# Mingrui-Yu/A-Simple-Stereo-SLAM-System-with-Deep-Loop-Closing

Hardware: AMD Instinct MI355X
Metric: stereo frames/sec (ORB+match+LCD+BA-build) @1241x376 (higher is better)
Workload: dtype u8/int32 (ORB, Hamming), f32 via f16x3 / bf16x6 split products on the matrix cores with f32 accumulate (CALC conv1 / conv2, DB scan), f64 (triangulation, BA)

## Files before the change

### a-simple-stereo-slam-system-with-deep-loop-closing_amd/api.py

```python
import ctypes as C
import os
import re

import numpy as np

_HERE = os.path.dirname(os.path.abspath(__file__))
LIB_PATH = os.path.join(_HERE, "libmyslam_hip.so")

OK, ERR_INVALID, ERR_HIP, ERR_CAPACITY, ERR_UNSUPPORTED = 0, -1, -2, -3, -4
LCD_DIM = 1064

KP_DTYPE = np.dtype([("x", "<f4"), ("y", "<f4"), ("size", "<f4"), ("angle", "<f4"),
                     ("response", "<f4"), ("octave", "<i4"), ("class_id", "<i4")])
assert KP_DTYPE.itemsize == 28


class MyslamError(RuntimeError):
    def __init__(self, where, code):
        names = {-1: "INVALID", -2: "HIP", -3: "CAPACITY", -4: "UNSUPPORTED"}
        super().__init__(f"{where} failed: {code} ({names.get(code, '?')})")
        self.code = code


HEADER_PATH = os.path.join(_HERE, "..", "include", "myslam_hip.h")
CALC_LAYER_DTYPE = np.dtype([("type", "<i4"), ("num_output", "<i4"), ("kernel", "<i4"), ("stride", "<i4"), ("pad", "<i4"),
                             ("local_size", "<i4"), ("alpha", "<f4"), ("beta", "<f4"), ("k", "<f4")])
assert CALC_LAYER_DTYPE.itemsize == 36
CALC_CONV, CALC_RELU, CALC_POOL_MAX, CALC_LRN = 1, 2, 3, 4
CAND_DTYPE = np.dtype([("best_id", "<u8"), ("max_score", "<f4"), ("cnt", "<i4")])
assert CAND_DTYPE.itemsize == 16
OWNED_DTYPE = np.dtype([("pre_best_id", "<u8"), ("pre_max_score", "<f4"), ("pre_cnt", "<i4"),
                        ("suf_best_id", "<u8"), ("suf_max_score", "<f4"), ("suf_cnt", "<i4")])
assert OWNED_DTYPE.itemsize == 32

_lib = None
_SCALARS = {"int": C.c_int, "float": C.c_float, "double": C.c_double, "size_t": C.c_size_t, "uint64_t": C.c_uint64, "long": C.c_long,
            "int32_t": C.c_int32, "uint8_t": C.c_uint8, "int64_t": C.c_int64}


def header_prototypes(path=HEADER_PATH):
    txt = open(path).read()
    txt = re.sub(r"/\*.*?\*/", " ", txt, flags=re.S)
    txt = re.sub(r"//[^\n]*", " ", txt)
    out = {}
    for m in re.finditer(r"\b(int|float|size_t|const char\s*\*)\s+(myslam_\w+)\s*\(([^()]*)\)\s*;", txt):
        ret, name, params = m.group(1), m.group(2), m.group(3).strip()
        types = []
        if params and params != "void":
            for prm in params.split(","):
                prm = prm.strip()
                if "*" in prm:
                    types.append("ptr")
                else:
                    toks = [t for t in prm.split() if t != "const"]
                    types.append(toks[0])
        out[name] = ("char*" if "char" in ret else ret, types)
    return out


def lib():
    global _lib
    if _lib is None:
        if not os.path.exists(LIB_PATH):
            raise RuntimeError(f"{LIB_PATH} is missing: run __graft_entry__.build() / build.py first (no CPU fallback)")
        L = C.CDLL(LIB_PATH)
        for name, (ret, types) in header_prototypes().items():
            fn = getattr(L, name)
            fn.restype = {"int": C.c_int, "float": C.c_float, "size_t": C.c_size_t, "char*": C.c_char_p}[ret]
            fn.argtypes = [C.c_void_p if t == "ptr" else _SCALARS[t] for t in types]
        _lib = L
    return _lib


def _check(code, where):
    if code != OK:
        raise MyslamError(where, code)


def _p(a):
    return a.ctypes.data_as(C.c_void_p) if a is not None else None


def device_count():
    return lib().myslam_hip_device_count()


def version():
    return lib().myslam_hip_version().decode()


def build_id():
    return version().rsplit(" ", 1)[-1]


def shader_clock_mhz(stream=0, spin_us=200.0):
    v = C.c_float()
    _check(lib().myslam_prof_shader_clock_mhz(stream, float(spin_us), C.byref(v)), "myslam_prof_shader_clock_mhz")
    return float(v.value)


def prof_enable(on=True):
    lib().myslam_prof_enable(1 if on else 0)


def prof_reset():
    lib().myslam_prof_reset()


def prof_read():
    L = lib()
    out = {}
    for i in range(L.myslam_prof_count()):
        name = C.c_char_p(); ms = C.c_double(); n = C.c_long()
        L.myslam_prof_get(i, C.byref(name), C.byref(ms), C.byref(n))
        out[name.value.decode()] = (ms.value, n.value)
    return out


class ORBextractor:

    def __init__(self, nfeatures=2000, scaleFactor=1.2, nlevels=8, iniThFAST=20, minThFAST=7, stream=None):
        self._h = C.c_void_p()
        _check(lib().myslam_orb_create(C.byref(self._h), int(nfeatures), C.c_float(scaleFactor), int(nlevels),
                                       int(iniThFAST), int(minThFAST)), "myslam_orb_create")
        self.nfeatures, self.nlevels = nfeatures, nlevels
        if stream is not None:
            self.set_stream(stream)

    def __del__(self):
        if getattr(self, "_h", None) and self._h.value and _lib is not None:
            _lib.myslam_orb_destroy(self._h)
            self._h = C.c_void_p()

    def set_stream(self, stream_ptr):
        _check(lib().myslam_orb_set_stream(self._h, C.c_void_p(stream_ptr)), "myslam_orb_set_stream")

    def set_fast_event(self, event_ptr):
        _check(lib().myslam_orb_set_fast_event(self._h, C.c_void_p(event_ptr or None)), "myslam_orb_set_fast_event")

    def set_fast_gate(self, event_ptr):
        _check(lib().myslam_orb_set_fast_gate(self._h, C.c_void_p(event_ptr or None)), "myslam_orb_set_fast_gate")

    OPT_FAST_MODE, OPT_INTERNAL_STREAM, OPT_STOP_AFTER, OPT_COPY_INPUT, OPT_BLUR_MFMA, OPT_SIDE_BLOCKS_PER_CU = 1, 2, 3, 4, 5, 6

    def set_option(self, option, value):
        _check(lib().myslam_orb_set_option(self._h, int(option), int(value)), "myslam_orb_set_option")

    def set_gauss_taps(self, q7=None):
        q = None if q7 is None else np.ascontiguousarray(q7, np.int32)
        _check(lib().myslam_orb_set_gauss_taps(self._h, _p(q) if q is not None else None), "myslam_orb_set_gauss_taps")

    def tables(self):
        n = self.nlevels
        sc = np.zeros(n, np.float32); isc = np.zeros(n, np.float32); npl = np.zeros(n, np.int32); um = np.zeros(16, np.int32)
        _check(lib().myslam_orb_get_tables(self._h, _p(sc), _p(isc), _p(npl), _p(um)), "myslam_orb_get_tables")
        return sc, isc, npl, um

    def max_keypoints(self, rows=None, cols=None):
        if rows is not None:
            return lib().myslam_orb_max_keypoints_for(self._h, int(rows), int(cols))
        return lib().myslam_orb_max_keypoints(self._h)

    @staticmethod
    def _img(img):
        img = np.ascontiguousarray(img, np.uint8)
        assert img.ndim == 2
        return img

    def DetectAndCompute(self, image, mask=None, cap=None):
        img = self._img(image)
        cap = cap or self.max_keypoints(*img.shape)
        kps = np.zeros(cap, KP_DTYPE); desc = np.zeros((cap, 32), np.uint8); n = C.c_int()
        m = self._img(mask) if mask is not None else None
        _check(lib().myslam_orb_detect_and_compute(self._h, _p(img), img.shape[0], img.shape[1], img.strides[0],
                                                   _p(m), m.strides[0] if m is not None else 0,
                                                   _p(kps), _p(desc), cap, C.byref(n)), "myslam_orb_detect_and_compute")
        return kps[:n.value].copy(), desc[:n.value].copy()

    def Detect(self, image, mask=None, cap=None):
        img = self._img(image)
        cap = cap or self.max_keypoints(*img.shape)
        kps = np.zeros(cap, KP_DTYPE); n = C.c_int()
        m = self._img(mask) if mask is not None else None
        _check(lib().myslam_orb_detect(self._h, _p(img), img.shape[0], img.shape[1], img.strides[0],
                                       _p(m), m.strides[0] if m is not None else 0, _p(kps), cap, C.byref(n)),
               "myslam_orb_detect")
        return kps[:n.value].copy()

    def ScreenAndComputeKPsParams(self, image, keypoints):
        img = self._img(image)
        kin = np.ascontiguousarray(keypoints, KP_DTYPE).copy()
        kout = np.zeros(max(len(kin), 1), KP_DTYPE); n = C.c_int()
        _check(lib().myslam_orb_screen_and_compute_params(self._h, _p(img), img.shape[0], img.shape[1], img.strides[0],
                                                          _p(kin), len(kin), _p(kout), len(kout), C.byref(n)),
               "myslam_orb_screen_and_compute_params")
        return kout[:n.value].copy(), kin

    def CalcDescriptors(self, image, keypoints):
        img = self._img(image)
        k = np.ascontiguousarray(keypoints, KP_DTYPE)
        desc = np.zeros((len(k), 32), np.uint8)
        _check(lib().myslam_orb_calc_descriptors(self._h, _p(img), img.shape[0], img.shape[1], img.strides[0],
                                                 _p(k), len(k), _p(desc)), "myslam_orb_calc_descriptors")
        return desc

    def detect_and_compute_batch(self, d_imgs, batch, rows, cols, step, img_stride, d_kps, d_desc, d_counts, d_status, cap,
                                 d_masks=0):
        _check(lib().myslam_orb_detect_and_compute_batch(self._h, C.c_void_p(d_imgs), batch, rows, cols, step,
                                                         C.c_size_t(img_stride), C.c_void_p(d_masks or None),
                                                         C.c_void_p(d_kps), C.c_void_p(d_desc), C.c_void_p(d_counts),
                                                         C.c_void_p(d_status or None), cap),
               "myslam_orb_detect_and_compute_batch")

    def detect_batch(self, d_imgs, batch, rows, cols, step, img_stride, d_kps, d_counts, d_status, cap, d_masks=0):
        _check(lib().myslam_orb_detect_batch(self._h, C.c_void_p(d_imgs), batch, rows, cols, step, C.c_size_t(img_stride),
                                             C.c_void_p(d_masks or None), C.c_void_p(d_kps), C.c_void_p(d_counts),
                                             C.c_void_p(d_status or None), cap), "myslam_orb_detect_batch")

    def process_keyframes_batch(self, d_imgs, batch, rows, cols, step, img_stride, d_feat_xy, d_n_feat, feat_cap, d_pyr_kps, d_desc, d_counts,
                                d_status, cap):
        _check(lib().myslam_orb_process_keyframes_batch(self._h, C.c_void_p(d_imgs), int(batch), int(rows), int(cols), int(step),
                                                        C.c_size_t(img_stride), C.c_void_p(d_feat_xy), C.c_void_p(d_n_feat), int(feat_cap),
                                                        C.c_void_p(d_pyr_kps), C.c_void_p(d_desc), C.c_void_p(d_counts), C.c_void_p(d_status),
                                                        int(cap)), "myslam_orb_process_keyframes_batch")

    def debug_pyramid(self, image, level, blurred=False):
        img = self._img(image)
        w = C.c_int(); h = C.c_int()
        _check(lib().myslam_orb_debug_pyramid(self._h, _p(img), img.shape[0], img.shape[1], img.strides[0], level,
                                              1 if blurred else 0, None, 0, C.byref(w), C.byref(h)), "debug_pyramid(size)")
        out = np.zeros((h.value, w.value), np.uint8)
        _check(lib().myslam_orb_debug_pyramid(self._h, _p(img), img.shape[0], img.shape[1], img.strides[0], level,
                                              1 if blurred else 0, _p(out), out.strides[0], C.byref(w), C.byref(h)),
               "debug_pyramid")
        return out

    def debug_candidates(self, image, level, mask=None):
        img = self._img(image)
        cap = 65536
        xs = np.zeros(cap, np.int32); ys = np.zeros(cap, np.int32); sc = np.zeros(cap, np.int32); n = C.c_int()
        m = self._img(mask) if mask is not None else None
        _check(lib().myslam_orb_debug_candidates(self._h, _p(img), img.shape[0], img.shape[1], img.strides[0],
                                                 _p(m), m.strides[0] if m is not None else 0, level,
                                                 _p(xs), _p(ys), _p(sc), cap, C.byref(n)), "debug_candidates")
        return xs[:n.value].copy(), ys[:n.value].copy(), sc[:n.value].copy()

    def fast_statistics(self, level):
        out = np.zeros(4, np.uint32)
        _check(lib().myslam_orb_debug_readback(self._h, 6, 0, level, _p(out), out.nbytes, 0), "debug_readback")
        return int(out[0]), int(out[1]), int(out[2])


def hamming_match(query, train):
    q = np.ascontiguousarray(query, np.uint8).reshape(-1, 32); t = np.ascontiguousarray(train, np.uint8).reshape(-1, 32)
    idx = np.zeros(len(q), np.int32); dist = np.zeros(len(q), np.int32)
    _check(lib().myslam_hamming_match(_p(q), len(q), _p(t), len(t), _p(idx), _p(dist)), "myslam_hamming_match")
    return idx, dist


def hamming_match_batch(d_q, d_nq, d_t, d_nt, batch, cap, d_idx, d_dist, stream=0):
    _check(lib().myslam_hamming_match_batch(C.c_void_p(d_q), C.c_void_p(d_nq), C.c_void_p(d_t), C.c_void_p(d_nt), batch, cap,
                                            C.c_void_p(d_idx), C.c_void_p(d_dist), C.c_void_p(stream or None)),
           "myslam_hamming_match_batch")


def hamming_filter(dist):
    d = np.ascontiguousarray(dist, np.int32)
    keep = np.zeros(len(d), np.uint8); mn = C.c_int()
    _check(lib().myslam_hamming_filter(_p(d), len(d), _p(keep), C.byref(mn)), "myslam_hamming_filter")
    return keep.astype(bool), mn.value


def expand_pyramid_keypoints(feats, nlevels=8):
    f = np.ascontiguousarray(feats, KP_DTYPE)
    out = np.zeros(len(f) * nlevels, KP_DTYPE)
    _check(lib().myslam_expand_pyramid_keypoints(_p(f), len(f), nlevels, _p(out)), "myslam_expand_pyramid_keypoints")
    return out


def match_feature_pairs(train_idx, dist, loop_pyr_kps, cur_pyr_kps):
    ti = np.ascontiguousarray(train_idx, np.int32); d = np.ascontiguousarray(dist, np.int32)
    lk = np.ascontiguousarray(loop_pyr_kps, KP_DTYPE); ck = np.ascontiguousarray(cur_pyr_kps, KP_DTYPE)
    assert len(ti) == len(d) == len(lk)
    pairs = np.zeros((max(len(ti), 1), 2), np.int32); n = C.c_int()
    _check(lib().myslam_match_feature_pairs(_p(ti), _p(d), len(ti), _p(lk), _p(ck), len(ck), _p(pairs), C.byref(n)), "myslam_match_feature_pairs")
    return pairs[:n.value].copy()


LOOP_MATCH_OK, LOOP_MATCH_FEW_PAIRS, LOOP_MATCH_FEW_POINTS = 0, 1, 2


def loop_match_batch(d_loop_desc, d_n_loop, d_cur_desc, d_n_cur, d_loop_pyr, d_cur_pyr, batch, cap, d_cur_feat_xy, d_loop_feat_landmark, feat_cap,
                     d_landmark_pos, landmark_stride, landmark_cap, min_matches, out_cap, d_train_idx, d_dist, d_pairs, d_n_pairs, d_valid_pairs,
                     d_pts3d, d_pts2d, d_counts, d_status, stream=0):
    ptrs = [C.c_void_p(x) for x in (d_loop_desc, d_n_loop, d_cur_desc, d_n_cur, d_loop_pyr, d_cur_pyr)]
    outs = [C.c_void_p(x) for x in (d_train_idx, d_dist, d_pairs, d_n_pairs, d_valid_pairs, d_pts3d, d_pts2d, d_counts, d_status)]
    _check(lib().myslam_loop_match_batch(*ptrs, int(batch), int(cap), C.c_void_p(d_cur_feat_xy), C.c_void_p(d_loop_feat_landmark), int(feat_cap),
                                         C.c_void_p(d_landmark_pos), int(landmark_stride), int(landmark_cap), int(min_matches), int(out_cap), *outs,
                                         C.c_void_p(stream or None)), "myslam_loop_match_batch")


def triangulate_stereo(xl, yl, xr, yr, fx, fy, cx, cy, baseline):
    xl, yl, xr, yr = [np.ascontiguousarray(a, np.float32) for a in (xl, yl, xr, yr)]
    n = len(xl)
    xyz = np.zeros((n, 3)); ok = np.zeros(n, np.uint8)
    _check(lib().myslam_triangulate_stereo(_p(xl), _p(yl), _p(xr), _p(yr), n, C.c_double(fx), C.c_double(fy), C.c_double(cx),
                                           C.c_double(cy), C.c_double(baseline), _p(xyz), _p(ok)), "myslam_triangulate_stereo")
    return xyz, ok.astype(bool)


def triangulate_stereo_batch(d_kl, d_kr, d_match, d_nl, batch, cap, K, baseline, d_xyz, d_ok, stream=0):
    _check(lib().myslam_triangulate_stereo_batch(C.c_void_p(d_kl), C.c_void_p(d_kr), C.c_void_p(d_match), C.c_void_p(d_nl),
                                                 batch, cap, C.c_double(K[0]), C.c_double(K[1]), C.c_double(K[2]),
                                                 C.c_double(K[3]), C.c_double(baseline), C.c_void_p(d_xyz), C.c_void_p(d_ok),
                                                 C.c_void_p(stream or None)), "myslam_triangulate_stereo_batch")


def hamming_match_triangulate_batch(d_q, d_nq, d_t, d_nt, d_kl, d_kr, batch, cap, K, baseline, d_idx, d_dist, d_xyz, d_ok, stream=0):
    _check(lib().myslam_hamming_match_triangulate_batch(C.c_void_p(d_q), C.c_void_p(d_nq), C.c_void_p(d_t), C.c_void_p(d_nt), C.c_void_p(d_kl),
                                                        C.c_void_p(d_kr), batch, cap, C.c_double(K[0]), C.c_double(K[1]), C.c_double(K[2]),
                                                        C.c_double(K[3]), C.c_double(baseline), C.c_void_p(d_idx), C.c_void_p(d_dist),
                                                        C.c_void_p(d_xyz), C.c_void_p(d_ok), C.c_void_p(stream or None)),
           "myslam_hamming_match_triangulate_batch")


def calc_default_layers():
    n = lib().myslam_lcd_default_layers(None, 0)
    L = np.zeros(n, CALC_LAYER_DTYPE)
    assert lib().myslam_lcd_default_layers(_p(L), n) == n
    return L


def calc_parse_caffe(prototxt_path, caffemodel_path):
    nl = C.c_int(); nw = C.c_size_t()
    _check(lib().myslam_calc_parse_caffe(prototxt_path.encode(), caffemodel_path.encode(), None, 0, C.byref(nl), None, 0, C.byref(nw)),
           "myslam_calc_parse_caffe")
    L = np.zeros(nl.value, CALC_LAYER_DTYPE); w = np.zeros(nw.value, np.float32)
    _check(lib().myslam_calc_parse_caffe(prototxt_path.encode(), caffemodel_path.encode(), _p(L), len(L), C.byref(nl), _p(w), w.size, C.byref(nw)),
           "myslam_calc_parse_caffe")
    return L, w


class DeepLCD:
    OPT_GENERIC_KERNELS = 1
    OPT_CONV2_BF16X6 = 2
    OPT_SKIP_KERNELS = 3

    def __init__(self, weights=None, stream=None, layers=None, caffe=None, path=None):
        self._h = C.c_void_p()
        if caffe is not None:
            _check(lib().myslam_lcd_create_from_caffe(C.byref(self._h), caffe[0].encode(), caffe[1].encode()), "myslam_lcd_create_from_caffe")
        elif path is not None:
            _check(lib().myslam_lcd_create_from_file(C.byref(self._h), path.encode()), "myslam_lcd_create_from_file")
        else:
            w = np.ascontiguousarray(weights, np.float32).ravel()
            if layers is not None:
                L = np.ascontiguousarray(layers, CALC_LAYER_DTYPE)
                _check(lib().myslam_lcd_create_from_layers(C.byref(self._h), _p(L), len(L), _p(w), w.size), "myslam_lcd_create_from_layers")
            else:
                _check(lib().myslam_lcd_create(C.byref(self._h), _p(w), w.size), "myslam_lcd_create")
        if stream is not None:
            _check(lib().myslam_lcd_set_stream(self._h, C.c_void_p(stream)), "myslam_lcd_set_stream")

    @classmethod
    def from_caffe(cls, prototxt_path="calc_model/deploy.prototxt", caffemodel_path="calc_model/calc.caffemodel", stream=None):
        return cls(caffe=(prototxt_path, caffemodel_path), stream=stream)

    def set_option(self, option, value):
        _check(lib().myslam_lcd_set_option(self._h, int(option), int(value)), "myslam_lcd_set_option")

    def uses_fused_kernels(self):
        return lib().myslam_lcd_uses_fused_kernels(self._h) == 1

    def conv2_products(self):
        return lib().myslam_lcd_conv2_products(self._h)

    def __del__(self):
        if getattr(self, "_h", None) and self._h.value and _lib is not None:
            _lib.myslam_lcd_destroy(self._h)
            self._h = C.c_void_p()

    def calcDescrOriginalImg(self, image, blur_in_place=True):
        img = np.ascontiguousarray(image, np.uint8).copy()
        d = np.zeros(LCD_DIM, np.float32)
        _check(lib().myslam_lcd_calc_descr_original_img(self._h, _p(img), img.shape[0], img.shape[1], img.strides[0],
                                                        1 if blur_in_place else 0, _p(d)), "myslam_lcd_calc_descr_original_img")
        return d, img

    def calcDescr(self, im160x120):
        img = np.ascontiguousarray(im160x120, np.uint8)
        assert img.shape == (120, 160)
        d = np.zeros(LCD_DIM, np.float32)
        _check(lib().myslam_lcd_calc_descr(self._h, _p(img), img.strides[0], _p(d)), "myslam_lcd_calc_descr")
        return d

    @staticmethod
    def score(d1, d2):
        a = np.ascontiguousarray(d1, np.float32); b = np.ascontiguousarray(d2, np.float32)
        return float(lib().myslam_lcd_score(_p(a), _p(b)))

    def describe_batch(self, d_imgs, batch, rows, cols, step, img_stride, d_out, blur_in_place=False):
        _check(lib().myslam_lcd_describe_batch(self._h, C.c_void_p(d_imgs), batch, rows, cols, step, C.c_size_t(img_stride),
                                               1 if blur_in_place else 0, C.c_void_p(d_out)), "myslam_lcd_describe_batch")
# ... 845 lines not shown
```

### a-simple-stereo-slam-system-with-deep-loop-closing_amd/csrc/orb_engine.hip

```cpp
#include <math.h>
#include <stdlib.h>
#include <string.h>

#include <vector>

#include "common.h"
#include "orb_launch.h"
#include "orb_plan.h"
#include "resize_tab.h"

namespace myslam_hip {

static inline int cv_round(float v) { return (int)lrintf(v); }
static inline size_t align_up(size_t v, size_t a) { return (v + a - 1) / a * a; }

void gauss_q8(int kind, int q[7]) {
    if (kind == 1) { const int t[7] = {8, 28, 56, 72, 56, 28, 8}; memcpy(q, t, sizeof(t)); return; }
    double g[7], sum = 0;
    for (int i = 0; i < 7; i++) { double x = i - 3; g[i] = exp(-(x * x) / 8.0); sum += g[i]; }
    for (int i = 0; i < 7; i++) q[i] = (int)lrint(g[i] / sum * 256.0);
}

}

using namespace myslam_hip;

struct myslam_orb {
    int nfeatures, nlevels, iniTh, minTh;
    float scaleFactor;
    std::vector<float> scale, invScale;
    std::vector<int> nPerLevel;
    int umax[16];
    hipStream_t stream = nullptr;
    hipStream_t aux = nullptr;
    hipEvent_t evFork = nullptr, evJoin = nullptr;
    hipEvent_t evUserFast = nullptr;
    hipEvent_t evUserGate = nullptr;

    int rows = 0, cols = 0;
    OrbPlan full{}, det{};

    int batchCap = 0;
    Buf<uint8_t> d_pyr, d_blur, d_mask;
    Buf<uint32_t> d_cand;
    Buf<uint32_t> d_sort;
    Buf<int32_t> d_candCount, d_selCount, d_status;
    Buf<uint32_t> d_sel;
    Buf<uint16_t> d_order;
    Buf<uint32_t> d_octTab;
    Buf<uint32_t> d_stripTab;
    Buf<uint32_t> d_resizeTab;
    size_t resizeColOff[MAXL] = {0}, resizeRowOff[MAXL] = {0}; bool resizeLvOk[MAXL] = {false};
    Buf<uint32_t> d_fastStat; int fastFlip = 0;
    int optFastMode = -1;
    int optInternalStream = 1;
    int optCopyInput = 0;
    int optStopAfter = 0;
    int tapsSet = 0, taps[7] = {0};
    int optSideBlocksPerCu = 0;
    int optBlurMfma = 0;
    Buf<uint4> d_blurTab; bool blurTabValid = false; size_t blurOffI = 0, blurOffH[MAXL] = {0}, blurOffV[MAXL] = {0}; bool blurLvOk[MAXL] = {false}; int blurVconst = 0;
    int ensure_blur_tables();

    struct HostGraph {
        static constexpr int kStayEager = -1000000;
        hipGraphExec_t exec = nullptr; hipGraph_t graph = nullptr; uint64_t gen = 0; int rows = 0, cols = 0, step = 0, dcap = 0, calls = 0; bool mask = false;
        void reset(bool stayEager = false) {
            if (exec) (void)hipGraphExecDestroy(exec);
            if (graph) (void)hipGraphDestroy(graph);
            if (stayEager) { exec = nullptr; graph = nullptr; calls = kStayEager; }
            else *this = HostGraph();
        }
        bool matches(uint64_t g, int r, int c, int st, int dc, bool m) const { return gen == g && rows == r && cols == c && step == st && dcap == dc && mask == m; }
        void rekey(uint64_t g, int r, int c, int st, int dc, bool m) { reset(); gen = g; rows = r; cols = c; step = st; dcap = dc; mask = m; }
    };
    HostGraph hostGraph[2][2];
    uint64_t gen = 1;
    ZeroArgs clr{};
    ZeroArgs take_clear() { const ZeroArgs z = clr; clr = ZeroArgs{}; return z; }
    hipStream_t hostStream = nullptr;
    PinBuf<uint8_t> h_pin;
    int ensure_pin(size_t bytes);
    void drop_host_graphs();
    Buf<uint8_t> d_stageImg, d_stageMask;
    int stageCap = 0;
    Buf<uint8_t> d_stageOut; size_t stageDescOff = 0;
    int32_t* stage_counts() const { return reinterpret_cast<int32_t*>(d_stageOut.get()); }
    myslam_keypoint* stage_kps() const { return reinterpret_cast<myslam_keypoint*>(d_stageOut + 256); }
    uint8_t* stage_desc() const { return d_stageOut + stageDescOff; }
    Buf<myslam_keypoint> d_stageKps2; Buf<uint8_t> d_stageKeep;

    int make_tables();
    void level_size(int l, int r, int c, int& w, int& h) const {
        w = cv_round((float)c * invScale[l]); h = cv_round((float)r * invScale[l]);
    }
    int make_plan(int r, int c);
    int ensure(int batch, int r, int c, bool needMask);
    int ensure_stage(size_t imgBytes, size_t maskBytes, int cap);
    int ensure_fast_stat();
    Buf<myslam_keypoint> d_pkfRows; Buf<uint8_t> d_pkfKeep;
    int ensure_pkf(size_t nrows);
    int process_keyframes(const uint8_t* d_imgs, int batch, int r, int c, int step, size_t stride, const float* d_feat_xy, const int32_t* d_n_feat,
                          int feat_cap, myslam_keypoint* d_pyr_kps, uint8_t* d_desc, int32_t* d_counts, int32_t* d_stat, int cap);
    void set_in_place(const uint8_t* p, size_t stride, int pitch, int n0) {
        full.ext0 = det.ext0 = p; full.ext0Stride = det.ext0Stride = stride; full.ext0Pitch = det.ext0Pitch = pitch; full.ext0N = det.ext0N = n0;
    }
    int stage_pyramid(const uint8_t* img, int r, int c, int step, const uint8_t* mask, int ncap);
    int build_pyramids(const uint8_t* d_imgs, int batch, int step, size_t stride, const uint8_t* d_masks, int nlev);
    ResizeArgs level_resize_args(uint8_t* base, int l) const;
    BlurArgs level_blur_args(int l) const;
    int blur_levels(int batch, int nlev, hipStream_t s);
    void fill_blur_args(BlurArgs* lv, int nlev) const;
    int run_fast(const OrbPlan& P, const uint8_t* maskPyr, int batch);
    int run_batch(const uint8_t* d_imgs, int batch, int r, int c, int step, size_t stride, const uint8_t* d_masks,
                  myslam_keypoint* d_kps, uint8_t* d_desc, int32_t* d_counts, int32_t* d_stat, int cap, bool detectOnly);
    void free_all();
};

int myslam_orb::make_tables() {
    scale.assign(nlevels, 1.f); invScale.assign(nlevels, 1.f); nPerLevel.assign(nlevels, 0);
    for (int i = 1; i < nlevels; i++) scale[i] = scale[i - 1] * scaleFactor;
    for (int i = 0; i < nlevels; i++) invScale[i] = 1.0f / scale[i];
    float factor = 1.0f / scaleFactor;
    float nDesired = nfeatures * (1 - factor) / (1 - (float)pow((double)factor, (double)nlevels));
    int sum = 0;
    for (int l = 0; l < nlevels - 1; l++) { nPerLevel[l] = cv_round(nDesired); sum += nPerLevel[l]; nDesired *= factor; }
    nPerLevel[nlevels - 1] = std::max(nfeatures - sum, 0);
    int v, v0, vmax = (int)floor(HALF_PATCH * sqrtf(2.f) / 2 + 1), vmin = (int)ceil(HALF_PATCH * sqrtf(2.f) / 2);
    const double hp2 = HALF_PATCH * HALF_PATCH;
    for (v = 0; v < 16; v++) umax[v] = 0;
    for (v = 0; v <= vmax; ++v) umax[v] = (int)lrint(sqrt(hp2 - v * v));
    for (v = HALF_PATCH, v0 = 0; v >= vmin; --v) { while (umax[v0] == umax[v0 + 1]) ++v0; umax[v] = v0; ++v0; }
    const int expect[16] = {15, 15, 15, 15, 14, 14, 14, 13, 13, 12, 11, 10, 9, 8, 6, 3};
    for (v = 0; v < 16; v++) if (umax[v] != expect[v]) return MYSLAM_ERR_INVALID;
    return MYSLAM_OK;
}

static int ceil_log2(int v) { int b = 0; while ((1 << b) < v) b++; return b; }

static int level_nini(int w, int h) {
    const int bx = w - EDGE_THRESHOLD + 3 - MIN_BORDER, by = h - EDGE_THRESHOLD + 3 - MIN_BORDER;
    return bx > 0 && by > 0 ? (int)roundf((float)bx / (float)by) : 0;
}
static int node_cap(int N, int nIni, int& cap) {
    cap = (std::max(N + 4, 4 * nIni + 4) + 3) & ~3;
    return cap > 4092 ? MYSLAM_ERR_UNSUPPORTED : MYSLAM_OK;
}

int myslam_orb::make_plan(int r, int c) {
    OrbPlan P{};
    P.nlevels = nlevels; P.rows = r; P.cols = c; P.iniTh = iniTh; P.minTh = minTh;
    size_t imgOff = 0, keyOff = 0; int cellBase = 0, outBase = 0, stripBase = 0;
    for (int l = 0; l < nlevels; l++) {
        LevelGeom& g = P.lv[l];
        level_size(l, r, c, g.w, g.h);
        if (g.w < 1 || g.h < 1) return MYSLAM_ERR_UNSUPPORTED;
        g.pitch = (int)align_up(g.w, 64);
        g.maxBX = g.w - EDGE_THRESHOLD + 3; g.maxBY = g.h - EDGE_THRESHOLD + 3;
        const float width = (float)(g.maxBX - MIN_BORDER), height = (float)(g.maxBY - MIN_BORDER);
        const float W = 30;
        g.nCols = (int)(width / W); g.nRows = (int)(height / W);
        if (g.nCols < 1 || g.nRows < 1) return MYSLAM_ERR_UNSUPPORTED;
        g.wCell = (int)ceilf(width / g.nCols); g.hCell = (int)ceilf(height / g.nRows);
        if (g.wCell > MAX_CELL || g.hCell > MAX_CELL) return MYSLAM_ERR_UNSUPPORTED;
        if (g.maxBX + 3 > 4095 + MIN_BORDER || g.maxBY + 3 > 4095 + MIN_BORDER) return MYSLAM_ERR_UNSUPPORTED;
        g.cellBase = cellBase; cellBase += g.nCols * g.nRows;
        g.stripBase = stripBase; stripBase += g.nRows * ((g.nCols + 3) / 4);
        g.N = nPerLevel[l];
        g.nIni = level_nini(g.w, g.h);
        if (g.nIni < 1 || g.nIni > 64) return MYSLAM_ERR_UNSUPPORTED;
        g.hX = (float)(g.maxBX - MIN_BORDER) / g.nIni;
        const int rootW = (int)ceilf(g.hX) + 2, H = g.maxBY - MIN_BORDER;
        g.ndepth = std::min(MAX_DEPTH, ceil_log2(std::max(rootW, H)) + 2);
        g.sortDepth = 0;
        while (g.sortDepth + 1 <= g.ndepth && (g.nIni << (2 * (g.sortDepth + 1))) <= 1024) g.sortDepth++;
        g.keyCap = (int)std::min<size_t>(262143, std::max<size_t>(256, (size_t)((g.w + 1) / 2) * ((g.h + 1) / 2)));
        if (node_cap(g.N, g.nIni, g.nodeCap)) return MYSLAM_ERR_UNSUPPORTED;
        g.outBase = outBase; outBase += g.nodeCap;
        g.scale = scale[l];
        g.scaledPatch = (float)(int)(PATCH_SIZE * scale[l]);
        g.imgOff = imgOff; imgOff += align_up((size_t)g.pitch * align_up((size_t)g.h, 8), 256);
        g.keyOff = keyOff; keyOff += g.keyCap;
    }
    for (int l = 0; l < MAXL; l++) P.stripBaseOf[l] = l < P.nlevels ? P.lv[l].stripBase : INT32_MAX;
    P.ncells = cellBase; P.nstrips = stripBase; P.totalKeyCap = (int)keyOff; P.totalOut = outBase; P.pyrBytes = imgOff;
    {
        std::vector<uint32_t> tab;
        for (int l = 0; l < nlevels; l++) {
            LevelGeom& g = P.lv[l];
            g.tabX = g.maxBX - MIN_BORDER + 8; g.tabY = g.maxBY - MIN_BORDER + 8; g.tabOff = (int)tab.size();
            tab.resize(tab.size() + 2 * (size_t)(g.tabX + g.tabY), 0u);
            uint32_t* xcode = tab.data() + g.tabOff; uint32_t* ycode = xcode + g.tabX;
            uint32_t* xcell = ycode + g.tabY; uint32_t* ycell = xcell + g.tabX;
            for (int px = 0; px < g.tabX; px++) {
                int r = (int)((float)px / g.hX);
                r = std::min(std::max(r, 0), g.nIni - 1);
                int UL = (int)(g.hX * (float)r), UR = (int)(g.hX * (float)(r + 1));
                uint32_t code = (uint32_t)r << ROOT_SHIFT;
                for (int k = 1; k <= g.ndepth; k++) {
                    const int mid = UL + ((UR - UL + 1) >> 1);
                    const uint32_t d = px >= mid;
                    code |= d << (ROOT_SHIFT - 2 * k);
                    if (d) UL = mid; else UR = mid;
                }
                xcode[px] = code;
                xcell[px] = (uint32_t)(std::max(px - 3, 0) / g.wCell);
            }
            for (int py = 0; py < g.tabY; py++) {
                int UL = 0, BR = g.maxBY - MIN_BORDER;
                uint32_t code = 0;
                for (int k = 1; k <= g.ndepth; k++) {
                    const int mid = UL + ((BR - UL + 1) >> 1);
                    const uint32_t d = py >= mid;
                    code |= (d << 1) << (ROOT_SHIFT - 2 * k);
                    if (d) UL = mid; else BR = mid;
                }
                ycode[py] = code;
                ycell[py] = (uint32_t)((std::max(py - 3, 0) / g.hCell) * g.nCols);
            }
        }
        int rc = d_octTab.renew(tab.size());
        if (rc) return rc;
        if ((rc = upload_table(d_octTab, tab.data(), tab.size() * sizeof(uint32_t)))) return rc;
    }
    {
        std::vector<uint32_t> st((size_t)P.nstrips * 8, 0u);
        for (int l = 0; l < nlevels; l++) {
            const LevelGeom& g = P.lv[l];
            const int spr = (g.nCols + 3) / 4;
            for (int strip = 0; strip < g.nRows * spr; strip++) {
                uint32_t* e = st.data() + (size_t)(g.stripBase + strip) * 8;
                const int ci = strip / spr, cj0 = (strip - ci * spr) * 4;
                const int iniY = MIN_BORDER + ci * g.hCell;
                int ncell = 0, pairs = 0; uint32_t wcs = 0; int hr = 0;
                if (iniY < g.maxBY - 3) {
                    hr = std::min(iniY + g.hCell + 6, g.maxBY) - iniY;
                    const int hc = hr - 6;
                    if (hc > 0)
                        for (int c = 0; c < 4; c++) {
                            const int cj = cj0 + c, iniX = MIN_BORDER + cj * g.wCell;
                            int wc = 0;
                            if (cj < g.nCols && iniX < g.maxBX - 6) wc = std::max(0, std::min(iniX + g.wCell + 6, g.maxBX) - iniX - 6);
                            if (wc > 0) ncell = c + 1;
                            wcs |= (uint32_t)wc << (8 * c);
                            pairs += ((wc + 1) >> 1) * hc;
                        }
                }
                if (ncell == 0) wcs = 0;
                e[0] = (uint32_t)l | ((uint32_t)ci << 8) | ((uint32_t)cj0 << 16) | ((uint32_t)ncell << 24);
                e[1] = (uint32_t)iniY | ((uint32_t)hr << 16);
                e[2] = (uint32_t)(MIN_BORDER + cj0 * g.wCell) | ((uint32_t)g.wCell << 16);
                e[3] = wcs; e[4] = (uint32_t)g.pitch; e[5] = (uint32_t)pairs;
                e[6] = (uint32_t)(g.imgOff & 0xffffffffu); e[7] = (uint32_t)(g.imgOff >> 32);
            }
        }
        int rc = d_stripTab.renew(st.size());
        if (rc) return rc;
        if ((rc = upload_table(d_stripTab, st.data(), st.size() * sizeof(uint32_t)))) return rc;
        P.stripTab = d_stripTab;
    }
    full = P;
    {
        std::vector<uint32_t> rt;
        std::vector<ResizeColRec> cr; std::vector<ResizeRowRec> rr;
        for (int l = 1; l < nlevels; l++) {
            const ResizeArgs a = level_resize_args(nullptr, l);
            resizeLvOk[l] = resize_uses_strips(a);
            if (!resizeLvOk[l]) continue;
            resize_col_records(a.sw, a.dw, a.scale_x, (a.dw + 255) / 256 * 64, cr);
            resize_row_records(a.sh, a.dh, a.scale_y, rr);
            resizeColOff[l] = rt.size();
            rt.insert(rt.end(), reinterpret_cast<const uint32_t*>(cr.data()), reinterpret_cast<const uint32_t*>(cr.data() + cr.size()));
            resizeRowOff[l] = rt.size();
            rt.insert(rt.end(), reinterpret_cast<const uint32_t*>(rr.data()), reinterpret_cast<const uint32_t*>(rr.data() + rr.size()));
            rt.resize((rt.size() + 7) & ~(size_t)7, 0u);
        }
        int rc = d_resizeTab.renew(rt.size());
        if (rc) return rc;
        if (!rt.empty() && (rc = upload_table(d_resizeTab, rt.data(), rt.size() * sizeof(uint32_t)))) return rc;
    }
    det = P;
    det.nlevels = 1;
    det.ncells = P.lv[0].nCols * P.lv[0].nRows;
    det.nstrips = P.lv[0].nRows * ((P.lv[0].nCols + 3) / 4);
    det.lv[0].N = nfeatures;
    if (node_cap(nfeatures, P.lv[0].nIni, det.lv[0].nodeCap)) return MYSLAM_ERR_UNSUPPORTED;
    det.lv[0].outBase = 0;
    det.totalOut = det.lv[0].nodeCap;
    rows = r; cols = c;
    return MYSLAM_OK;
}

int myslam_orb::ensure(int batch, int r, int c, bool needMask) {
    if (r != rows || c != cols) {
        MYSLAM_HIP_CHECK(hipStreamSynchronize(stream));
        int rc = make_plan(r, c);
        if (rc) { rows = cols = 0; return rc; }
        batchCap = 0; gen++; blurTabValid = false;
    }
    const int detOut = det.totalOut;
    const size_t selPer = (size_t)std::max(full.totalOut, detOut);
    if (batch > batchCap) {
        MYSLAM_HIP_CHECK(hipStreamSynchronize(stream));
        gen++;
        d_mask.release();
        int rc = regrow(batchCap, batch, [&]() -> int {
            int rc;
            if ((rc = d_pyr.renew((size_t)batch * full.pyrBytes + 64))) return rc;
            if ((rc = d_blur.renew((size_t)batch * full.pyrBytes + 4096))) return rc;
            if ((rc = d_cand.renew((size_t)batch * full.totalKeyCap))) return rc;
            if ((rc = d_sort.renew((size_t)batch * full.totalKeyCap * 2))) return rc;
            if ((rc = d_candCount.renew((size_t)batch * MAXL))) return rc;
            if ((rc = d_selCount.renew((size_t)batch * MAXL))) return rc;
            if ((rc = d_status.renew((size_t)batch))) return rc;
            if ((rc = d_sel.renew((size_t)batch * selPer))) return rc;
            return d_order.renew((size_t)batch * selPer);
        });
        if (rc) return rc;
    }
    if (needMask && !d_mask) return d_mask.renew((size_t)batchCap * full.pyrBytes + 64);
    return MYSLAM_OK;
}

int myslam_orb::build_pyramids(const uint8_t* d_imgs, int batch, int step, size_t stride, const uint8_t* d_masks, int nlev) {
    const OrbPlan& P = full;
    for (int pass = 0; pass < (d_masks ? 2 : 1); pass++) {
        uint8_t* base = pass ? d_mask : d_pyr;
        const uint8_t* src = pass ? d_masks : d_imgs;
        const int n0 = pass ? 0 : P.ext0N;
        int l = 1;
        const int nhead = std::min(pyr_head_levels(), nlev - 1);
        if (nhead >= 1 && batch > n0 && resize_is_little(level_resize_args(base, 1), batch)) {
            ScopedProf sp(P_RESIZE, stream);
            ResizeArgs grp[3];
            for (int j = 0; j < nhead; j++) grp[j] = level_resize_args(base, 1 + j);
            grp[0].src = src; grp[0].spitch = step; grp[0].sstride = stride;
            launch_pyr_head(grp, nhead, P.rows, P.cols, base + P.lv[0].imgOff, P.lv[0].pitch, P.pyrBytes, n0, batch, take_clear(), stream);
            l = 1 + nhead;
        } else if (batch > n0) {
            launch_ingest(src + (size_t)n0 * stride, P.rows, P.cols, step, stride, base + (size_t)n0 * P.pyrBytes + P.lv[0].imgOff, P.lv[0].pitch,
                          P.pyrBytes, batch - n0, take_clear(), stream);
        }
        for (; l < nlev;) {
            ScopedProf sp(P_RESIZE, stream);
            ResizeArgs a = level_resize_args(base, l);
            if (l == 1 && n0 > 0) { a.src0 = d_imgs; a.spitch0 = step; a.sstride0 = stride; a.n0 = n0; }
            ResizeArgs grp[4]; int ng = 0;
            const int gmax = resize_chain_max();
            if (gmax > 1 && resize_is_little(a, batch)) {
                static const double kEvals[4] = {1, 5, 21, 85};
                double evals = (double)batch * a.dw * a.dh;
                grp[ng++] = a;
                while (ng < gmax && l + ng < nlev) {
                    const ResizeArgs nx = level_resize_args(base, l + ng);
                    evals += (double)batch * nx.dw * nx.dh * kEvals[ng];
                    if (!resize_is_little(nx, batch) || evals > 6e6) break;
                    grp[ng++] = nx;
                }
            }
            if (ng > 1) { launch_resize_chain(grp, ng, batch, stream); l += ng; }
            else { launch_resize(a, batch, stream); l++; }
        }
    }
    return MYSLAM_OK;
}
ResizeArgs myslam_orb::level_resize_args(uint8_t* base, int l) const {
    const OrbPlan& P = full;
    ResizeArgs a;
    a.src = base + P.lv[l - 1].imgOff; a.sw = P.lv[l - 1].w; a.sh = P.lv[l - 1].h; a.spitch = P.lv[l - 1].pitch; a.sstride = P.pyrBytes;
    a.src0 = nullptr; a.spitch0 = 0; a.n0 = 0; a.sstride0 = 0;
    a.dst = base + P.lv[l].imgOff; a.dw = P.lv[l].w; a.dh = P.lv[l].h; a.dpitch = P.lv[l].pitch; a.dstride = P.pyrBytes;
    a.scale_x = 1. / ((double)a.dw / a.sw); a.scale_y = 1. / ((double)a.dh / a.sh);
    if (d_resizeTab && resizeLvOk[l]) { a.colTab = d_resizeTab + resizeColOff[l]; a.rowTab = d_resizeTab + resizeRowOff[l]; }
    return a;
}
int myslam_orb::ensure_blur_tables() {
    if (blurTabValid) return MYSLAM_OK;
    std::vector<uint4> tab;
    int q[7];
    if (tapsSet) memcpy(q, taps, sizeof(q)); else gauss_q8(0, q);
    int sum = 0;
    for (int t = 0; t < 7; t++) sum += q[t];
    blurVconst = sum * 128 * sum + 32768;
    blur_mfma_ident(tab, blurOffI);
    for (int l = 0; l < full.nlevels; l++) blurLvOk[l] = blur_mfma_tables(full.lv[l].w, full.lv[l].h, q, tab, blurOffH[l], blurOffV[l]);
    MYSLAM_HIP_CHECK(hipStreamSynchronize(stream));
    int rc = d_blurTab.renew(tab.size());
    if (rc) return rc;
    if ((rc = upload_table(d_blurTab, tab.data(), tab.size() * sizeof(uint4)))) return rc;
    blurTabValid = true; gen++;
    return MYSLAM_OK;
}

BlurArgs myslam_orb::level_blur_args(int l) const {
    const OrbPlan& P = full;
    BlurArgs a;
    a.src = d_pyr + P.lv[l].imgOff; a.dst = d_blur + P.lv[l].imgOff;
    a.w = P.lv[l].w; a.h = P.lv[l].h; a.spitch = a.dpitch = P.lv[l].pitch; a.sstride = a.dstride = P.pyrBytes;
    a.src0 = nullptr; a.spitch0 = 0; a.n0 = 0; a.sstride0 = 0;
    a.dtiled = 1;
    if (tapsSet) memcpy(a.q, taps, sizeof(taps)); else gauss_q8(0, a.q);
    if (optBlurMfma && blurTabValid && blurLvOk[l]) { a.tabH = d_blurTab + blurOffH[l]; a.tabV = d_blurTab + blurOffV[l]; a.ident = d_blurTab + blurOffI; a.vconst = blurVconst; }
    return a;
}
void myslam_orb::fill_blur_args(BlurArgs* lv, int nlev) const {
    const OrbPlan& P = full;
    for (int l = 0; l < nlev; l++) {
        lv[l] = level_blur_args(l);
        if (l == 0 && P.ext0N > 0) { lv[l].src0 = P.ext0; lv[l].spitch0 = P.ext0Pitch; lv[l].sstride0 = P.ext0Stride; lv[l].n0 = P.ext0N; }
    }
}
int myslam_orb::blur_levels(int batch, int nlev, hipStream_t stream) {
    BlurArgs lv[MAXL];
    fill_blur_args(lv, nlev);
    ScopedProf sp(P_BLUR, stream);
    launch_blur_levels(lv, nlev, batch, stream);
    return MYSLAM_OK;
}

int myslam_orb::run_batch(const uint8_t* d_imgs, int batch, int r, int c, int step, size_t stride, const uint8_t* d_masks,
                          myslam_keypoint* d_kps, uint8_t* d_desc, int32_t* d_counts, int32_t* d_stat, int cap, bool detectOnly) {
    if (!d_imgs || batch <= 0 || r <= 0 || c <= 0 || step < c || cap <= 0 || !d_kps || !d_counts) return MYSLAM_ERR_INVALID;
    if (!detectOnly && !d_desc) return MYSLAM_ERR_INVALID;
    int rc = ensure(batch, r, c, d_masks != nullptr);
    if (rc) return rc;
    if (optBlurMfma && !detectOnly && (rc = ensure_blur_tables())) return rc;
    const OrbPlan& P = detectOnly ? det : full;
    int32_t* stat = d_stat ? d_stat : d_status;
    if ((rc = ensure_fast_stat())) return rc;
    clr = {{reinterpret_cast<uint32_t*>(d_candCount.get()), reinterpret_cast<uint32_t*>(d_selCount.get()), reinterpret_cast<uint32_t*>(stat), d_fastStat + (size_t)fastFlip * MAXL * 4},
           {batch * MAXL, batch * MAXL, batch, MAXL * 4}};
    const int stop = optStopAfter;
    {
        int n0 = 0;
        if (!optCopyInput && stop == 0 && batch > 1 && full.nlevels >= 1 && stride >= (size_t)r * (size_t)step) {
            bool ok = blur_uses_strips(level_blur_args(0));
            if (full.nlevels > 1) ok = ok && resize_uses_strips(level_resize_args(d_pyr, 1));
            if (ok) n0 = batch - 1;
        }
        set_in_place(d_imgs, stride, step, n0);
    }
    if (stop == 1) {
        launch_ingest(d_imgs, full.rows, full.cols, step, stride, d_pyr + full.lv[0].imgOff, full.lv[0].pitch, full.pyrBytes, batch, take_clear(), stream);
        return MYSLAM_OK;
    }
    if ((rc = build_pyramids(d_imgs, batch, step, stride, d_masks, P.nlevels))) return rc;
    if (stop == 2) return MYSLAM_OK;
    hipStreamCaptureStatus capst = hipStreamCaptureStatusNone;
    if (stream && hipStreamIsCapturing(stream, &capst) != hipSuccess) { (void)hipGetLastError(); capst = hipStreamCaptureStatusNone; }
    const int aux_mode = capst == hipStreamCaptureStatusActive ? 0 : optInternalStream;
    const bool fork = aux_mode > 0 && !detectOnly && stop == 0;
    if (fork && !aux) {
        MYSLAM_HIP_CHECK(hipStreamCreateWithFlags(&aux, hipStreamNonBlocking));
        MYSLAM_HIP_CHECK(hipEventCreateWithFlags(&evFork, hipEventDisableTiming));
        MYSLAM_HIP_CHECK(hipEventCreateWithFlags(&evJoin, hipEventDisableTiming));
    }
    auto fork_blur = [&]() -> int {
        MYSLAM_HIP_CHECK(hipEventRecord(evFork, stream));
        MYSLAM_HIP_CHECK(hipStreamWaitEvent(aux, evFork, 0));
        int rc2 = blur_levels(batch, P.nlevels, aux);
        if (rc2) return rc2;
        MYSLAM_HIP_CHECK(hipEventRecord(evJoin, aux));
        return MYSLAM_OK;
    };
    if (fork && aux_mode == 2 && (rc = fork_blur())) return rc;
    if (evUserGate) MYSLAM_HIP_CHECK(hipStreamWaitEvent(stream, evUserGate, 0));
    if ((rc = run_fast(P, d_masks ? d_mask : nullptr, batch))) return rc;
    if (evUserFast) MYSLAM_HIP_CHECK(hipEventRecord(evUserFast, stream));
    if (fork && aux_mode != 2 && (rc = fork_blur())) return rc;
    bool blurred = false;
    {
        ScopedProf sp(P_OCTREE, stream);
        BlurArgs blv[MAXL];
        const bool tryBlur = !fork && !detectOnly && stop == 0 && !optBlurMfma;
        if (tryBlur) fill_blur_args(blv, P.nlevels);
        blurred = launch_octree(P, d_cand, d_candCount, d_sort, d_octTab, d_sel, d_selCount, stat, batch,
                                describe_uses_tile_order(d_order != nullptr, detectOnly ? 1 : 0, batch) ? d_order : nullptr, stream,
                                tryBlur ? blv : nullptr, tryBlur ? P.nlevels : 0);
    }
    if (stop == 3) return MYSLAM_OK;
    if (fork) MYSLAM_HIP_CHECK(hipStreamWaitEvent(stream, evJoin, 0));
    else if (!detectOnly && !blurred && (rc = blur_levels(batch, P.nlevels, stream))) return rc;
    if (stop == 4) return MYSLAM_OK;
    {
        ScopedProf sp(P_DESC, stream);
        launch_describe(P, d_pyr, d_blur, full.pyrBytes, d_sel, d_selCount, d_kps, d_desc, d_counts, stat, cap,
                        detectOnly ? 1 : 0, batch, d_order, true, optSideBlocksPerCu, stream);
    }
    MYSLAM_HIP_CHECK(hipGetLastError());
    return MYSLAM_OK;
}

int myslam_orb::run_fast(const OrbPlan& P, const uint8_t* maskPyr, int batch) {
    uint32_t* cur = d_fastStat + (size_t)fastFlip * MAXL * 4;
    const uint32_t* prev = d_fastStat + (size_t)(fastFlip ^ 1) * MAXL * 4;
    fastFlip ^= 1;
    ScopedProf sp(P_FAST, stream);
    launch_fast(P, d_pyr, full.pyrBytes, maskPyr, d_cand, d_candCount, prev, cur, optFastMode, batch, stream);
    return MYSLAM_OK;
}

int myslam_orb::ensure_pin(size_t bytes) {
    if (bytes <= h_pin.size()) return MYSLAM_OK;
    gen++;
    return h_pin.renew((bytes + (bytes >> 2) + 4095) & ~(size_t)4095);
}

void myslam_orb::drop_host_graphs() {
    for (auto& row : hostGraph)
        for (auto& g : row) g.reset();
}

int myslam_orb::ensure_fast_stat() {
    if (d_fastStat) return MYSLAM_OK;
    int rc = d_fastStat.renew(2 * MAXL * 4);
    if (rc) return rc;
    MYSLAM_HIP_CHECK(hipMemsetAsync(d_fastStat, 0, sizeof(uint32_t) * 2 * MAXL * 4, stream));
    return MYSLAM_OK;
}

int myslam_orb::ensure_pkf(size_t nrows) {
    if (nrows <= std::min(d_pkfRows.size(), d_pkfKeep.size())) return MYSLAM_OK;
    MYSLAM_HIP_CHECK(hipStreamSynchronize(stream));
    gen++; drop_host_graphs();
    int rc;
    if ((rc = d_pkfRows.renew(nrows))) return rc;
    return d_pkfKeep.renew(nrows);
}

int myslam_orb::process_keyframes(const uint8_t* d_imgs, int batch, int r, int c, int step, size_t stride, const float* d_feat_xy,
                                  const int32_t* d_n_feat, int feat_cap, myslam_keypoint* d_pyr_kps, uint8_t* d_desc, int32_t* d_counts,
                                  int32_t* d_stat, int cap) {
    if (!d_imgs || !d_feat_xy || !d_n_feat || !d_pyr_kps || !d_desc || !d_counts || !d_stat) return MYSLAM_ERR_INVALID;
    if (batch <= 0 || r <= 0 || c <= 0 || step < c || feat_cap <= 0 || cap <= 0) return MYSLAM_ERR_INVALID;
    if (batch > 65535 || (size_t)feat_cap * nlevels > ((size_t)1 << 24) || cap > (1 << 24)) return MYSLAM_ERR_CAPACITY;
    int rc = ensure(batch, r, c, false);
    if (rc) return rc;
    if (optBlurMfma && (rc = ensure_blur_tables())) return rc;
    const int rowCap = feat_cap * nlevels;
    if ((rc = ensure_pkf((size_t)batch * rowCap))) return rc;
    clr = {{reinterpret_cast<uint32_t*>(d_counts), reinterpret_cast<uint32_t*>(d_stat), nullptr, nullptr}, {batch, batch, 0, 0}};
    set_in_place(nullptr, 0, 0, 0);
    rc = build_pyramids(d_imgs, batch, step, stride, nullptr, nlevels);
    clr = ZeroArgs{};
    if (rc) return rc;
    if ((rc = blur_levels(batch, nlevels, stream))) return rc;
    {
        ScopedProf sp(P_SCREEN, stream);
        launch_process_keyframes(full, PkfArgs{d_pyr, d_blur, full.pyrBytes, d_feat_xy, d_n_feat, feat_cap, d_pkfRows, d_pkfKeep, rowCap,
                                               d_pyr_kps, d_desc, d_counts, d_stat, cap}, batch, stream);
    }
    MYSLAM_HIP_CHECK(hipGetLastError());
    return MYSLAM_OK;
}

int myslam_orb::stage_pyramid(const uint8_t* img, int r, int c, int step, const uint8_t* mask, int ncap) {
    const size_t bytes = (size_t)r * step;
    int rc = ensure(1, r, c, mask != nullptr);
    if (rc) return rc;
    if ((rc = ensure_stage(bytes, mask ? bytes : 0, ncap))) return rc;
    MYSLAM_HIP_CHECK(hipMemcpyAsync(d_stageImg, img, bytes, hipMemcpyHostToDevice, stream));
    if (mask) MYSLAM_HIP_CHECK(hipMemcpyAsync(d_stageMask, mask, bytes, hipMemcpyHostToDevice, stream));
    set_in_place(nullptr, 0, 0, 0);
    return build_pyramids(d_stageImg, 1, step, bytes, mask ? d_stageMask : nullptr, nlevels);
}

int myslam_orb::ensure_stage(size_t imgBytes, size_t maskBytes, int cap) {
    int rc;
    if (imgBytes > d_stageImg.size()) { gen++; if ((rc = d_stageImg.renew(imgBytes))) return rc; }
    if (maskBytes > d_stageMask.size()) { gen++; if ((rc = d_stageMask.renew(maskBytes))) return rc; }
    if (cap > stageCap) {
        gen++;
        stageDescOff = 256 + (((size_t)cap * sizeof(myslam_keypoint) + 255) & ~(size_t)255);
        return regrow(stageCap, cap, [&]() -> int {
            int rc;
            if ((rc = d_stageOut.renew(stageDescOff + (size_t)cap * 32))) return rc;
            if ((rc = d_stageKps2.renew((size_t)cap))) return rc;
            return d_stageKeep.renew((size_t)cap);
        });
    }
    return MYSLAM_OK;
}

void myslam_orb::free_all() {
    if (aux) { (void)hipStreamSynchronize(aux); (void)hipStreamDestroy(aux); (void)hipEventDestroy(evFork); (void)hipEventDestroy(evJoin); aux = nullptr; }
    drop_host_graphs();
    if (hostStream) { (void)hipStreamSynchronize(hostStream); (void)hipStreamDestroy(hostStream); hostStream = nullptr; }
}

extern "C" {

int myslam_orb_create(myslam_orb** out, int nfeatures, float scale_factor, int nlevels, int ini_th_fast, int min_th_fast) {
    if (!out || nfeatures < 1 || nlevels < 1 || nlevels > MAXL || !(scale_factor > 1.0f) || ini_th_fast < 0 ||
        min_th_fast < 1 || min_th_fast > ini_th_fast || ini_th_fast > 255 || scale_factor > 2.5f)
        return MYSLAM_ERR_INVALID;
    if (need_device()) return MYSLAM_ERR_HIP;
    myslam_orb* h = new myslam_orb();
    h->nfeatures = nfeatures; h->scaleFactor = scale_factor; h->nlevels = nlevels; h->iniTh = ini_th_fast; h->minTh = min_th_fast;
    int rc = h->make_tables();
    if (rc) { delete h; return rc; }
    *out = h;
    return MYSLAM_OK;
}

int myslam_orb_destroy(myslam_orb* h) {
    if (!h) return MYSLAM_ERR_INVALID;
    (void)hipStreamSynchronize(h->stream);
    h->free_all();
    delete h;
    return MYSLAM_OK;
}

int myslam_orb_set_stream(myslam_orb* h, void* s) {
    if (!h) return MYSLAM_ERR_INVALID;
    (void)hipStreamSynchronize(h->stream);
    h->stream = (hipStream_t)s; h->gen++;
    return MYSLAM_OK;
}

int myslam_orb_set_fast_event(myslam_orb* h, void* ev) {
    if (!h) return MYSLAM_ERR_INVALID;
    h->evUserFast = (hipEvent_t)ev; h->gen++;
    return MYSLAM_OK;
}

int myslam_orb_set_fast_gate(myslam_orb* h, void* ev) {
    if (!h) return MYSLAM_ERR_INVALID;
    h->evUserGate = (hipEvent_t)ev; h->gen++;
    return MYSLAM_OK;
}

int myslam_orb_set_option(myslam_orb* h, int option, int value) {
    if (!h) return MYSLAM_ERR_INVALID;
    h->gen++;
    switch (option) {
        case MYSLAM_ORB_OPT_FAST_MODE: if (value < -1 || value > 1) return MYSLAM_ERR_INVALID; h->optFastMode = value; return MYSLAM_OK;
        case MYSLAM_ORB_OPT_INTERNAL_STREAM: if (value < 0 || value > 2) return MYSLAM_ERR_INVALID; h->optInternalStream = value; return MYSLAM_OK;
        case MYSLAM_ORB_OPT_COPY_INPUT: if (value < 0 || value > 1) return MYSLAM_ERR_INVALID; h->optCopyInput = value; return MYSLAM_OK;
        case MYSLAM_ORB_OPT_STOP_AFTER: if (value < 0 || value > 4) return MYSLAM_ERR_INVALID; h->optStopAfter = value; return MYSLAM_OK;
        case MYSLAM_ORB_OPT_BLUR_MFMA: if (value < 0 || value > 1) return MYSLAM_ERR_INVALID; h->optBlurMfma = value; return MYSLAM_OK;
        case MYSLAM_ORB_OPT_SIDE_BLOCKS_PER_CU: if (value < 0 || value > 64) return MYSLAM_ERR_INVALID; h->optSideBlocksPerCu = value; return MYSLAM_OK;
    }
    return MYSLAM_ERR_INVALID;
}

int myslam_orb_set_gauss_taps(myslam_orb* h, const int32_t* q7) {
    if (!h) return MYSLAM_ERR_INVALID;
    h->blurTabValid = false;
    if (!q7) { h->tapsSet = 0; h->gen++; return MYSLAM_OK; }
    int sum = 0;
    for (int i = 0; i < 7; i++) { if (q7[i] < 0 || q7[i] > 255) return MYSLAM_ERR_INVALID; sum += q7[i]; }
    if (sum < 1 || sum > 257) return MYSLAM_ERR_INVALID;
    for (int i = 0; i < 7; i++) h->taps[i] = q7[i];
    h->tapsSet = 1; h->gen++;
    return MYSLAM_OK;
}

int myslam_orb_get_tables(const myslam_orb* h, float* scale, float* inv_scale, int* fpl, int* umax16) {
    if (!h) return MYSLAM_ERR_INVALID;
    for (int i = 0; i < h->nlevels; i++) {
        if (scale) scale[i] = h->scale[i];
        if (inv_scale) inv_scale[i] = h->invScale[i];
        if (fpl) fpl[i] = h->nPerLevel[i];
    }
    if (umax16) for (int i = 0; i < 16; i++) umax16[i] = h->umax[i];
    return MYSLAM_OK;
}

int myslam_orb_max_keypoints(const myslam_orb* h) {
    if (!h) return MYSLAM_ERR_INVALID;
    int s = 0;
    for (int l = 0; l < h->nlevels; l++) s += std::max(h->nPerLevel[l] + 3, 32);
    return std::max(s, std::max(h->nfeatures + 3, 32));
}

int myslam_orb_max_keypoints_for(const myslam_orb* h, int rows, int cols) {
    if (!h || rows < 1 || cols < 1) return MYSLAM_ERR_INVALID;
    int s = 0, first = 0;
    for (int l = 0; l < h->nlevels; l++) {
        int w, hh;
        h->level_size(l, rows, cols, w, hh);
        const int nIni = std::max(1, level_nini(w, hh));
        s += std::max(h->nPerLevel[l] + 3, 4 * nIni);
        if (l == 0) first = std::max(h->nfeatures + 3, 4 * nIni);
    }
    return std::max(std::max(s, first), 32);
}

int myslam_orb_detect_and_compute_batch(myslam_orb* h, const uint8_t* d_imgs, int batch, int rows, int cols, int step,
                                        size_t img_stride, const uint8_t* d_masks, myslam_keypoint* d_kps, uint8_t* d_desc,
                                        int32_t* d_counts, int32_t* d_status, int cap) {
    if (!h) return MYSLAM_ERR_INVALID;
    return h->run_batch(d_imgs, batch, rows, cols, step, img_stride, d_masks, d_kps, d_desc, d_counts, d_status, cap, false);
}

int myslam_orb_detect_batch(myslam_orb* h, const uint8_t* d_imgs, int batch, int rows, int cols, int step, size_t img_stride,
                            const uint8_t* d_masks, myslam_keypoint* d_kps, int32_t* d_counts, int32_t* d_status, int cap) {
    if (!h) return MYSLAM_ERR_INVALID;
    return h->run_batch(d_imgs, batch, rows, cols, step, img_stride, d_masks, d_kps, nullptr, d_counts, d_status, cap, true);
}

int myslam_orb_process_keyframes_batch(myslam_orb* h, const uint8_t* d_imgs, int batch, int rows, int cols, int step, size_t img_stride,
                                       const float* d_feat_xy, const int32_t* d_n_feat, int feat_cap, myslam_keypoint* d_pyr_kps,
                                       uint8_t* d_desc, int32_t* d_counts, int32_t* d_status, int cap) {
    if (!h) return MYSLAM_ERR_INVALID;
    return h->process_keyframes(d_imgs, batch, rows, cols, step, img_stride, d_feat_xy, d_n_feat, feat_cap, d_pyr_kps, d_desc, d_counts,
                                d_status, cap);
}

static int host_extract(myslam_orb* h, const uint8_t* img, int rows, int cols, int step, const uint8_t* mask, int mask_step,
                        myslam_keypoint* kps, uint8_t* desc, int cap, int* n, bool detectOnly) {
    if (!h || !n) return MYSLAM_ERR_INVALID;
    *n = 0;
    if (!img || rows <= 0 || cols <= 0) return MYSLAM_OK;
    if (step < cols || cap <= 0 || !kps || (!detectOnly && !desc)) return MYSLAM_ERR_INVALID;
    if (mask && mask_step < cols) return MYSLAM_ERR_INVALID;
    int rc = h->ensure(1, rows, cols, mask != nullptr);
    if (rc) return rc;
    if (mask && mask_step != step) return MYSLAM_ERR_INVALID;
    const int dcap = std::max(cap, std::max(h->full.totalOut, h->det.totalOut));
    const size_t imgBytes = (size_t)rows * step, maskBytes = mask ? imgBytes : 0;
    if ((rc = h->ensure_stage(imgBytes, maskBytes, dcap))) return rc;
    if (h->optBlurMfma && !detectOnly && (rc = h->ensure_blur_tables())) return rc;
    const size_t oOut = (imgBytes + maskBytes + 255) & ~(size_t)255, oCnt = oOut, oKps = oOut + 256, oDesc = oOut + h->stageDescOff;
    const size_t outBytes = detectOnly ? 256 + sizeof(myslam_keypoint) * (size_t)dcap : h->stageDescOff + (size_t)32 * dcap;
    if ((rc = h->ensure_pin(oOut + h->d_stageOut.size()))) return rc;
    hipStream_t caller = h->stream;
    if (!caller) {
        if (!h->hostStream) { MYSLAM_HIP_CHECK(hipStreamCreateWithFlags(&h->hostStream, hipStreamNonBlocking)); h->gen++; }
        MYSLAM_HIP_CHECK(hipStreamSynchronize(nullptr));
    }
    hipStream_t hs = caller ? caller : h->hostStream;
    struct Swap { myslam_orb* h; hipStream_t keep; ~Swap() { h->stream = keep; } } swap{h, caller};
    h->stream = hs;
    memcpy(h->h_pin, img, imgBytes);
    if (mask) memcpy(h->h_pin + imgBytes, mask, maskBytes);
    auto enqueue = [&]() -> int {
        MYSLAM_HIP_CHECK(hipMemcpyAsync(h->d_stageImg, h->h_pin, imgBytes, hipMemcpyHostToDevice, hs));
        if (mask) MYSLAM_HIP_CHECK(hipMemcpyAsync(h->d_stageMask, h->h_pin + imgBytes, maskBytes, hipMemcpyHostToDevice, hs));
        int r2 = h->run_batch(h->d_stageImg, 1, rows, cols, step, imgBytes, mask ? h->d_stageMask : nullptr,
                              h->stage_kps(), h->stage_desc(), h->stage_counts(), h->stage_counts() + 1, dcap, detectOnly);
        if (r2) return r2;
        MYSLAM_HIP_CHECK(hipMemcpyAsync(h->h_pin + oOut, h->d_stageOut, outBytes, hipMemcpyDeviceToHost, hs));
        return MYSLAM_OK;
    };
    const bool graphable = !prof_is_on() && !h->evUserGate && !h->evUserFast && h->optStopAfter == 0;
    myslam_orb::HostGraph& G = h->hostGraph[detectOnly ? 1 : 0][h->fastFlip & 1];
    if (!G.matches(h->gen, rows, cols, step, dcap, mask != nullptr)) G.rekey(h->gen, rows, cols, step, dcap, mask != nullptr);
    bool done = false;
    if (graphable && G.exec) {
        if (hipGraphLaunch(G.exec, hs) == hipSuccess) { h->fastFlip ^= 1; done = true; }
        else { (void)hipGetLastError(); G.reset(true); }
    } else if (graphable && G.calls >= 1) {
        const int flip0 = h->fastFlip;
        if (hipStreamBeginCapture(hs, hipStreamCaptureModeThreadLocal) == hipSuccess) {
            const int r2 = enqueue();
            const hipError_t e = hipStreamEndCapture(hs, &G.graph);
            if (r2 == MYSLAM_OK && e == hipSuccess && G.graph && hipGraphInstantiate(&G.exec, G.graph, nullptr, nullptr, 0) == hipSuccess &&
                hipGraphLaunch(G.exec, hs) == hipSuccess) {
                done = true;
            } else {
                (void)hipGetLastError(); G.reset(true); h->fastFlip = flip0;
            }
        } else {
            (void)hipGetLastError(); G.reset(true);
        }
    }
    if (!done && (rc = enqueue())) return rc;
    G.calls++;
    MYSLAM_HIP_CHECK(hipStreamSynchronize(hs));
    int32_t res[2];
    memcpy(res, h->h_pin + oCnt, sizeof(res));
    if (res[1] != 0) return res[1];
    if (res[0] > cap) { *n = res[0]; return MYSLAM_ERR_CAPACITY; }
    memcpy(kps, h->h_pin + oKps, sizeof(myslam_keypoint) * (size_t)res[0]);
    if (!detectOnly) memcpy(desc, h->h_pin + oDesc, (size_t)32 * res[0]);
    *n = res[0];
    return MYSLAM_OK;
}

int myslam_orb_detect_and_compute(myslam_orb* h, const uint8_t* img, int rows, int cols, int step, const uint8_t* mask,
                                  int mask_step, myslam_keypoint* kps, uint8_t* desc, int cap, int* n) {
    return host_extract(h, img, rows, cols, step, mask, mask_step, kps, desc, cap, n, false);
}

int myslam_orb_detect(myslam_orb* h, const uint8_t* img, int rows, int cols, int step, const uint8_t* mask, int mask_step,
                      myslam_keypoint* kps, int cap, int* n) {
    return host_extract(h, img, rows, cols, step, mask, mask_step, kps, nullptr, cap, n, true);
}

int myslam_orb_screen_and_compute_params(myslam_orb* h, const uint8_t* img, int rows, int cols, int step,
                                         myslam_keypoint* kps_in, int n_in, myslam_keypoint* kps_out, int cap, int* n_out) {
    if (!h || !n_out) return MYSLAM_ERR_INVALID;
    *n_out = 0;
    if (!img || rows <= 0 || cols <= 0 || n_in <= 0) return MYSLAM_OK;
    if (!kps_in || !kps_out || step < cols) return MYSLAM_ERR_INVALID;
    for (int i = 0; i < n_in; i++) if (kps_in[i].octave < 0 || kps_in[i].octave >= h->nlevels) return MYSLAM_ERR_INVALID;
    int rc = h->stage_pyramid(img, rows, cols, step, nullptr, n_in);
    if (rc) return rc;
    MYSLAM_HIP_CHECK(hipMemcpyAsync(h->stage_kps(), kps_in, sizeof(myslam_keypoint) * n_in, hipMemcpyHostToDevice, h->stream));
    {
        ScopedProf sp(P_SCREEN, h->stream);
        launch_screen(h->full, h->d_pyr, h->stage_kps(), n_in, h->d_stageKps2, h->d_stageKeep, h->stream);
    }
    std::vector<myslam_keypoint> tmp(n_in);
    std::vector<uint8_t> keep(n_in);
    MYSLAM_HIP_CHECK(hipMemcpyAsync(kps_in, h->stage_kps(), sizeof(myslam_keypoint) * n_in, hipMemcpyDeviceToHost, h->stream));
    MYSLAM_HIP_CHECK(hipMemcpyAsync(tmp.data(), h->d_stageKps2, sizeof(myslam_keypoint) * n_in, hipMemcpyDeviceToHost, h->stream));
    MYSLAM_HIP_CHECK(hipMemcpyAsync(keep.data(), h->d_stageKeep, n_in, hipMemcpyDeviceToHost, h->stream));
    MYSLAM_HIP_CHECK(hipStreamSynchronize(h->stream));
    int m = 0;
    for (int i = 0; i < n_in; i++)
        if (keep[i]) { if (m >= cap) return MYSLAM_ERR_CAPACITY; kps_out[m++] = tmp[i]; }
    *n_out = m;
    return MYSLAM_OK;
}

int myslam_orb_calc_descriptors(myslam_orb* h, const uint8_t* img, int rows, int cols, int step, const myslam_keypoint* kps,
                                int n, uint8_t* desc) {
    if (!h) return MYSLAM_ERR_INVALID;
    if (!img || rows <= 0 || cols <= 0 || n <= 0) return MYSLAM_OK;
    if (!kps || !desc || step < cols) return MYSLAM_ERR_INVALID;
    for (int i = 0; i < n; i++) if (kps[i].octave < 0 || kps[i].octave >= h->nlevels) return MYSLAM_ERR_INVALID;
    int rc = h->stage_pyramid(img, rows, cols, step, nullptr, n);
    if (rc) return rc;
    if ((rc = h->blur_levels(1, h->nlevels, h->stream))) return rc;
    MYSLAM_HIP_CHECK(hipMemcpyAsync(h->stage_kps(), kps, sizeof(myslam_keypoint) * n, hipMemcpyHostToDevice, h->stream));
    {
        ScopedProf sp(P_DESC, h->stream);
        launch_calc_desc(h->full, h->d_blur, h->stage_kps(), n, h->stage_desc(), h->stream);
    }
    MYSLAM_HIP_CHECK(hipMemcpyAsync(desc, h->stage_desc(), (size_t)32 * n, hipMemcpyDeviceToHost, h->stream));
    MYSLAM_HIP_CHECK(hipStreamSynchronize(h->stream));
    return MYSLAM_OK;
}

static int download_tiled_plane(const uint8_t* d_plane, const LevelGeom& g, uint8_t* out, int out_step, hipStream_t stream) {
    std::vector<uint8_t> tmp((size_t)g.pitch * align_up((size_t)g.h, 8));
    MYSLAM_HIP_CHECK(hipMemcpyAsync(tmp.data(), d_plane, tmp.size(), hipMemcpyDeviceToHost, stream));
    MYSLAM_HIP_CHECK(hipStreamSynchronize(stream));
    for (int y = 0; y < g.h; y++)
        for (int x = 0; x < g.w; x++) out[(size_t)y * out_step + x] = tmp[tiled_off(x, y, g.pitch)];
    return MYSLAM_OK;
}

int myslam_orb_debug_pyramid(myslam_orb* h, const uint8_t* img, int rows, int cols, int step, int level, int blurred,
                             uint8_t* out, int out_step, int* w, int* hgt) {
    if (!h || !img || level < 0 || level >= h->nlevels) return MYSLAM_ERR_INVALID;
    int rc = h->stage_pyramid(img, rows, cols, step, nullptr, 16);
    if (rc) return rc;
    if (blurred && (rc = h->blur_levels(1, h->nlevels, h->stream))) return rc;
    const LevelGeom& g = h->full.lv[level];
    if (w) *w = g.w;
    if (hgt) *hgt = g.h;
    if (out) {
        if (out_step < g.w) return MYSLAM_ERR_INVALID;
        if (blurred) return download_tiled_plane(h->d_blur + g.imgOff, g, out, out_step, h->stream);
        MYSLAM_HIP_CHECK(hipMemcpy2DAsync(out, out_step, h->d_pyr + g.imgOff, g.pitch, g.w, g.h, hipMemcpyDeviceToHost, h->stream));
    }
    MYSLAM_HIP_CHECK(hipStreamSynchronize(h->stream));
    return MYSLAM_OK;
}

int myslam_orb_debug_candidates(myslam_orb* h, const uint8_t* img, int rows, int cols, int step, const uint8_t* mask,
                                int mask_step, int level, int32_t* xs, int32_t* ys, int32_t* scores, int cap, int* n) {
    if (!h || !img || !n || level < 0 || level >= h->nlevels) return MYSLAM_ERR_INVALID;
    if (mask && mask_step != step) return MYSLAM_ERR_INVALID;
    int rc = h->stage_pyramid(img, rows, cols, step, mask, 16);
    if (rc) return rc;
    if ((rc = h->ensure_fast_stat())) return rc;
    launch_zero_u32(ZeroArgs{{reinterpret_cast<uint32_t*>(h->d_candCount.get()), h->d_fastStat + (size_t)h->fastFlip * MAXL * 4}, {MAXL, MAXL * 4}}, h->stream);
    if ((rc = h->run_fast(h->full, mask ? h->d_mask : nullptr, 1))) return rc;
    int32_t counts[MAXL];
    MYSLAM_HIP_CHECK(hipMemcpyAsync(counts, h->d_candCount, sizeof(counts), hipMemcpyDeviceToHost, h->stream));
    MYSLAM_HIP_CHECK(hipStreamSynchronize(h->stream));
    const LevelGeom& g = h->full.lv[level];
    *n = counts[level];
    if (counts[level] > g.keyCap || counts[level] > cap) return MYSLAM_ERR_CAPACITY;
    Buf<int32_t> d_tmp;
    const int m = counts[level];
    if (m > 0) {
        if ((rc = d_tmp.renew((size_t)3 * m))) return rc;
        launch_unpack_cands(h->d_cand + g.keyOff, m, d_tmp, d_tmp + m, d_tmp + 2 * m, h->stream);
        MYSLAM_HIP_CHECK(hipMemcpyAsync(xs, d_tmp, 4 * m, hipMemcpyDeviceToHost, h->stream));
        MYSLAM_HIP_CHECK(hipMemcpyAsync(ys, d_tmp + m, 4 * m, hipMemcpyDeviceToHost, h->stream));
        MYSLAM_HIP_CHECK(hipMemcpyAsync(scores, d_tmp + 2 * m, 4 * m, hipMemcpyDeviceToHost, h->stream));
        MYSLAM_HIP_CHECK(hipStreamSynchronize(h->stream));
    }
    return MYSLAM_OK;
}

int myslam_orb_debug_readback(myslam_orb* h, int what, int b, int level, void* out, size_t cap_bytes, int detect_plan) {
    if (!h || !out || h->rows == 0 || b < 0 || b >= h->batchCap || level < 0 || level >= h->nlevels) return MYSLAM_ERR_INVALID;
    MYSLAM_HIP_CHECK(hipStreamSynchronize(h->stream));
    const OrbPlan& P = detect_plan ? h->det : h->full;
    const LevelGeom& g = P.lv[level];
    switch (what) {
        case 0: case 1: {
            if (cap_bytes < (size_t)g.w * g.h) return MYSLAM_ERR_CAPACITY;
            const uint8_t* base = (what ? h->d_blur : h->d_pyr) + (size_t)b * h->full.pyrBytes + g.imgOff;
            if (what) return download_tiled_plane(base, g, static_cast<uint8_t*>(out), g.w, h->stream);
            MYSLAM_HIP_CHECK(hipMemcpy2D(out, g.w, base, g.pitch, g.w, g.h, hipMemcpyDeviceToHost));
            return MYSLAM_OK;
        }
        case 2: case 4: {
            if (cap_bytes < 4) return MYSLAM_ERR_CAPACITY;
            MYSLAM_HIP_CHECK(hipMemcpy(out, (what == 2 ? h->d_candCount : h->d_selCount) + b * MAXL + level, 4, hipMemcpyDeviceToHost));
            return MYSLAM_OK;
        }
        case 3: {
            if (cap_bytes < (size_t)g.keyCap * 4) return MYSLAM_ERR_CAPACITY;
            MYSLAM_HIP_CHECK(hipMemcpy(out, h->d_cand + (size_t)b * P.totalKeyCap + g.keyOff, (size_t)g.keyCap * 4, hipMemcpyDeviceToHost));
            return MYSLAM_OK;
        }
        case 6: {
            if (cap_bytes < 16) return MYSLAM_ERR_CAPACITY;
            if (!h->d_fastStat) return MYSLAM_ERR_INVALID;
            MYSLAM_HIP_CHECK(hipMemcpy(out, h->d_fastStat + ((size_t)(h->fastFlip ^ 1) * MAXL + level) * 4, 16, hipMemcpyDeviceToHost));
            return MYSLAM_OK;
        }
        case 5: {
            if (cap_bytes < (size_t)g.nodeCap * 4) return MYSLAM_ERR_CAPACITY;
            MYSLAM_HIP_CHECK(hipMemcpy(out, h->d_sel + (size_t)b * P.totalOut + g.outBase, (size_t)g.nodeCap * 4, hipMemcpyDeviceToHost));
            return MYSLAM_OK;
        }
    }
    return MYSLAM_ERR_INVALID;
}

}
```

### a-simple-stereo-slam-system-with-deep-loop-closing_amd/csrc/orb_kernels.hip

```cpp
#include <stdio.h>
#include <stdlib.h>

#include <type_traits>

#include "common.h"
#include "orb_launch.h"
#include "orb_plan.h"

namespace myslam_hip {

typedef unsigned short u16x2 __attribute__((ext_vector_type(2)));

#ifdef MYSLAM_BLOCK_TRACE
__device__ unsigned long long* g_bt_buf = nullptr;
__device__ unsigned int g_bt_cap = 0, g_bt_n = 0;
struct BlockTrace {
    unsigned long long t0 = 0, marks = 0, aux = 0; int kid; unsigned hw = 0; bool on = false;
    __device__ __forceinline__ void mark(int i) {
        if (on) marks |= ((__builtin_amdgcn_s_memrealtime() - t0) & 0xffffull) << (16 * i);
    }
    __device__ __forceinline__ BlockTrace(int kid_) : kid(kid_) {
        if (threadIdx.x != 0 || g_bt_buf == nullptr) return;
        const unsigned xcc = __builtin_amdgcn_s_getreg((3 << 11) | 20) & 0xf;
        if (xcc != 0) return;
        hw = __builtin_amdgcn_s_getreg((31 << 11) | 4);
        if (((hw >> 13) & 7) != 0) return;
        on = true; t0 = __builtin_amdgcn_s_memrealtime();
    }
    __device__ __forceinline__ ~BlockTrace() {
        if (!on) return;
        const unsigned long long dt = __builtin_amdgcn_s_memrealtime() - t0;
        const unsigned i = atomicAdd(&g_bt_n, 1u);
        if (i < g_bt_cap) {
            g_bt_buf[4 * i] = t0; g_bt_buf[4 * i + 2] = marks; g_bt_buf[4 * i + 3] = aux;
            g_bt_buf[4 * i + 1] = (dt & 0xffffffull) | ((unsigned long long)(kid & 0xf) << 24) | ((unsigned long long)((hw >> 8) & 0xff) << 32) |
                                  ((unsigned long long)(blockIdx.x & 0xffffff) << 40);
        }
    }
};
#define MYSLAM_BT(kid) BlockTrace bt_(kid)
#define MYSLAM_BT_MARK(i) bt_.mark(i)
#define MYSLAM_BT_AUX(v) bt_.aux = (v)
#define MYSLAM_BT_PARAM , BlockTrace* btp_
#define MYSLAM_BT_ARG , &bt_
#define MYSLAM_BT_MARKP(i) btp_->mark(i)
#else
#define MYSLAM_BT(kid) ((void)0)
#define MYSLAM_BT_MARK(i) ((void)0)
#define MYSLAM_BT_AUX(v) ((void)0)
#define MYSLAM_BT_PARAM
#define MYSLAM_BT_ARG
#define MYSLAM_BT_MARKP(i) ((void)0)
#endif

__constant__ int8_t c_pattern[1024] = {
#include "orb_pattern.inc"
};

__constant__ int c_umax[16] = {15, 15, 15, 15, 14, 14, 14, 13, 13, 12, 11, 10, 9, 8, 6, 3};

__device__ __forceinline__ void resize_coord(int d, double scale, int ssize, bool is_x, int& s, int& c0, int& c1) {
    float f = (float)__dsub_rn(__dmul_rn((double)d + 0.5, scale), 0.5);
    int si = (int)floorf(f);
    f = __fsub_rn(f, (float)si);
    if (is_x) {
        if (si < 0) { f = 0.f; si = 0; }
        if (si >= ssize - 1) { f = 0.f; si = ssize - 1; }
    }
    s = si;
    c0 = __float2int_rn(__fmul_rn(__fsub_rn(1.f, f), 2048.f));
    c1 = __float2int_rn(__fmul_rn(f, 2048.f));
}

__global__ __launch_bounds__(256) void k_resize(ResizeArgs a) {
    const int b = blockIdx.z;
    const int dy = blockIdx.y * 4 + (threadIdx.x >> 6);
    const int dx4 = (blockIdx.x * 64 + (threadIdx.x & 63)) * 4;
    if (dy >= a.dh || dx4 >= a.dw) return;
    int sy, b0, b1;
    resize_coord(dy, a.scale_y, a.sh, false, sy, b0, b1);
    const int sy0 = min(max(sy, 0), a.sh - 1), sy1 = min(max(sy + 1, 0), a.sh - 1);
    const uint8_t* S0 = a.src + (size_t)b * a.sstride + (size_t)sy0 * a.spitch;
    const uint8_t* S1 = a.src + (size_t)b * a.sstride + (size_t)sy1 * a.spitch;
    int sx[4], a0[4], a1[4];
#pragma unroll
    for (int k = 0; k < 4; k++) resize_coord(min(dx4 + k, a.dw - 1), a.scale_x, a.sw, true, sx[k], a0[k], a1[k]);
    const int xal = sx[0] & ~3;
    uint32_t w0[4], w1[4];
#pragma unroll
    for (int j = 0; j < 4; j++) {
        const int xo = xal + 4 * j;
        const bool ok = xo + 4 <= a.spitch;
        w0[j] = ok ? *reinterpret_cast<const uint32_t*>(S0 + xo) : 0u;
        w1[j] = ok ? *reinterpret_cast<const uint32_t*>(S1 + xo) : 0u;
    }
    uint32_t packed = 0;
#pragma unroll
    for (int k = 0; k < 4; k++) {
        const int o = sx[k] - xal;
        const int q = o >> 2;
        const uint32_t lo0 = (q == 0) ? w0[0] : (q == 1) ? w0[1] : (q == 2) ? w0[2] : w0[3];
        const uint32_t hi0 = (q == 0) ? w0[1] : (q == 1) ? w0[2] : (q == 2) ? w0[3] : 0u;
        const uint32_t lo1 = (q == 0) ? w1[0] : (q == 1) ? w1[1] : (q == 2) ? w1[2] : w1[3];
        const uint32_t hi1 = (q == 0) ? w1[1] : (q == 1) ? w1[2] : (q == 2) ? w1[3] : 0u;
        const uint32_t v0 = __builtin_amdgcn_alignbyte(hi0, lo0, (uint32_t)(o & 3));
        const uint32_t v1 = __builtin_amdgcn_alignbyte(hi1, lo1, (uint32_t)(o & 3));
        const int r0 = (int)(v0 & 0xff) * a0[k] + (int)((v0 >> 8) & 0xff) * a1[k];
        const int r1 = (int)(v1 & 0xff) * a0[k] + (int)((v1 >> 8) & 0xff) * a1[k];
        int v = (((b0 * (r0 >> 4)) >> 16) + ((b1 * (r1 >> 4)) >> 16) + 2) >> 2;
        v = min(max(v, 0), 255);
        packed |= (uint32_t)v << (8 * k);
    }
    *reinterpret_cast<uint32_t*>(a.dst + (size_t)b * a.dstride + (size_t)dy * a.dpitch + dx4) = packed;
}

constexpr int RC_MAX = 4;
struct ResizeChain {
    const uint8_t* src; int sw, sh, spitch; size_t sstride;
    int n;
    uint8_t* dst[RC_MAX]; int dw[RC_MAX], dh[RC_MAX], dpitch[RC_MAX]; size_t dstride;
    double scale_x[RC_MAX], scale_y[RC_MAX];
    int blk0[RC_MAX + 1];
};

template <int J>
__device__ __forceinline__ int rc_pix(const ResizeChain& c, const uint8_t* S, int x, int y) {
    if constexpr (J == 0) {
        return S[(size_t)y * c.spitch + x];
    } else {
        const int sw = J == 1 ? c.sw : c.dw[J - 2], sh = J == 1 ? c.sh : c.dh[J - 2];
        int sx, a0, a1, sy, b0, b1;
        resize_coord(x, c.scale_x[J - 1], sw, true, sx, a0, a1);
        resize_coord(y, c.scale_y[J - 1], sh, false, sy, b0, b1);
        const int sy0 = min(max(sy, 0), sh - 1), sy1 = min(max(sy + 1, 0), sh - 1);
        const int sx1 = min(sx + 1, sw - 1);
        const int r0 = rc_pix<J - 1>(c, S, sx, sy0) * a0 + rc_pix<J - 1>(c, S, sx1, sy0) * a1;
        const int r1 = rc_pix<J - 1>(c, S, sx, sy1) * a0 + rc_pix<J - 1>(c, S, sx1, sy1) * a1;
        const int v = (((b0 * (r0 >> 4)) >> 16) + ((b1 * (r1 >> 4)) >> 16) + 2) >> 2;
        return min(max(v, 0), 255);
    }
}

__host__ __device__ constexpr int rc_px(int J) { return J >= 4 ? 1 : 4; }

template <int J>
__device__ __forceinline__ void rc_store(const ResizeChain& c, const uint8_t* S, uint8_t* D, int item) {
    const int dw = c.dw[J - 1], dh = c.dh[J - 1], gpr = (dw + 3) >> 2;
    if constexpr (rc_px(J) == 4) {
        const int dy = item / gpr, dx4 = (item - dy * gpr) * 4;
        if (dy >= dh) return;
        uint32_t packed = 0;
#pragma unroll
        for (int k = 0; k < 4; k++) packed |= (uint32_t)rc_pix<J>(c, S, min(dx4 + k, dw - 1), dy) << (8 * k);
        *reinterpret_cast<uint32_t*>(D + (size_t)dy * c.dpitch[J - 1] + dx4) = packed;
    } else {
        const int dy = item / (4 * gpr), dx = item - dy * 4 * gpr;
        if (dy >= dh) return;
        D[(size_t)dy * c.dpitch[J - 1] + dx] = (uint8_t)rc_pix<J>(c, S, min(dx, dw - 1), dy);
    }
}

__device__ __forceinline__ void rc_block(const ResizeChain& c, int blk, int b) {
    const uint8_t* S = c.src + (size_t)b * c.sstride;
    if (blk < c.blk0[1]) rc_store<1>(c, S, c.dst[0] + (size_t)b * c.dstride, blk * 256 + (int)threadIdx.x);
    else if (blk < c.blk0[2]) rc_store<2>(c, S, c.dst[1] + (size_t)b * c.dstride, (blk - c.blk0[1]) * 256 + (int)threadIdx.x);
    else if (blk < c.blk0[3]) rc_store<3>(c, S, c.dst[2] + (size_t)b * c.dstride, (blk - c.blk0[2]) * 256 + (int)threadIdx.x);
    else rc_store<4>(c, S, c.dst[3] + (size_t)b * c.dstride, (blk - c.blk0[3]) * 256 + (int)threadIdx.x);
}

__global__ __launch_bounds__(256) void k_resize_chain(ResizeChain c) { rc_block(c, blockIdx.x, blockIdx.y); }

#ifndef MYSLAM_RS_BAND
#define MYSLAM_RS_BAND 64
#endif
#ifndef MYSLAM_RS_PF
#define MYSLAM_RS_PF 4
#endif
constexpr int RS_BAND = MYSLAM_RS_BAND;
constexpr int RS_PF = MYSLAM_RS_PF;

typedef uint32_t rs_u32x3 __attribute__((ext_vector_type(3)));
typedef uint32_t rs_u32x2 __attribute__((ext_vector_type(2)));

template <bool EXT>
__device__ __forceinline__ void resize_strip_walk(const ResizeArgs& a, const uint8_t* src, int spitch, uint8_t* dst, int lane, int strip, int dy0, int dy1) {
    typedef const uint32_t __attribute__((address_space(4))) * ConstU32;
    typedef const uint8_t __attribute__((address_space(1))) * GlobalU8;
    typedef std::conditional_t<EXT, rs_u32x2, rs_u32x3> Raw;
    typedef Raw __attribute__((aligned(EXT ? 1 : 4))) RawMem;
    const int dx4 = strip * 256 + 4 * lane;
    const uint4* crec = reinterpret_cast<const uint4*>(a.colTab) + 2 * (size_t)(strip * 64 + lane);
    const uint4 c0 = crec[0], c1 = crec[1];
    const uint32_t sel[4] = {0x0c010c00u, c0.y, c0.z, c0.w}, aw[4] = {c1.x, c1.y, c1.z, c1.w};
    const uint32_t xoff = EXT ? c0.x : (c0.x & ~3u), bsh = c0.x & 3u;
    const ConstU32 rt = (ConstU32)((uintptr_t)a.rowTab);
    const int r0 = (int)rt[4 * dy0];
    const int rlast = min((int)rt[4 * (dy1 - 1)] + 1, a.sh - 1);
    auto load_row = [&](int r) -> Raw {
        uintptr_t rp = (uintptr_t)src + (size_t)min(r, rlast) * (size_t)spitch;
        uint32_t xo = xoff;
        asm("" : "+s"(rp));
        asm volatile("" : "+v"(xo));
        return *reinterpret_cast<const RawMem __attribute__((address_space(1)))*>((GlobalU8)rp + xo);
    };
    auto hrow = [&](const Raw& w, uint32_t* h) {
// ... 1046 lines not shown
        int nquad = 0;
        const int hc4 = (hc + 3) >> 2, per_cell4 = ngr * hc4;
        const int nitems4 = BITMAP ? 32 * hc4 : ncell * per_cell4;
        int c, gi, cy4;
        int ec = 0, ecy = 0, egi = 0;
        if constexpr (BITMAP) {
            gi = tid & 7; c = (tid >> 3) & 3; cy4 = tid >> 5;
        } else {
            const float inv_ngr = 1.0f / (float)ngr;
            const int q = tid;
            c = (int)(((float)q + 0.5f) * (1.0f / (float)per_cell4));
            int rem = q - c * per_cell4;
            if (rem < 0) { c--; rem += per_cell4; } else if (rem >= per_cell4) { c++; rem -= per_cell4; }
            cy4 = (int)(((float)rem + 0.5f) * inv_ngr);
            gi = rem - cy4 * ngr;
            if (gi < 0) { cy4--; gi += ngr; } else if (gi >= ngr) { cy4++; gi -= ngr; }
            ec = T / per_cell4; const int erem = T - ec * per_cell4; ecy = erem / ngr; egi = erem - ecy * ngr;
        }
        const int wc_lane = BITMAP ? wc_of(c) : 0;
        const int zini = P.iniTh - zoff;
        for (int q0 = 0; q0 < nitems4; q0 += T) {
            const int q = q0 + (unsigned)tid;
            uint32_t zm[4] = {0u, 0u, 0u, 0u};
            u16x2 zacc = {0, 0};
            if (BITMAP ? (cy4 < hc4 && 4 * gi < wc_lane) : (q < nitems4 && 4 * gi < wc_of(c))) {
                uint32_t m[6][3];
#pragma unroll
                for (int j = 0; j < 6; j++) {
                    const uint32_t* rp = reinterpret_cast<const uint32_t*>(&s_score[c][(4 * cy4 + j) * SP + 4 * gi]);
                    m[j][0] = rp[0]; m[j][1] = rp[1]; m[j][2] = rp[2];
                }
                if (sampled)
                    nquad += __popcll(__ballot(m[1][1] != 0)) + __popcll(__ballot(m[2][1] != 0)) + __popcll(__ballot(m[3][1] != 0)) + __popcll(__ballot(m[4][1] != 0));
                if ((m[1][1] | m[2][1] | m[3][1] | m[4][1]) != 0) {
                    const NmsRowH Rt = nms_row_h(m[0][0], m[0][1], m[0][2]), Rb = nms_row_h(m[5][0], m[5][1], m[5][2]);
                    NmsRow R[4];
#pragma unroll
                    for (int j = 0; j < 4; j++) R[j] = nms_row(m[j + 1][0], m[j + 1][1], m[j + 1][2]);
                    zm[0] = nms_strict4(Rt, R[0], R[1], zacc);
                    zm[1] = nms_strict4(R[0], R[1], R[2], zacc);
                    zm[2] = nms_strict4(R[1], R[2], R[3], zacc);
                    zm[3] = nms_strict4(R[2], R[3], Rb, zacc);
                }
            }
            const unsigned long long b0 = __ballot(zm[0] != 0), b1 = __ballot(zm[1] != 0), b2 = __ballot(zm[2] != 0), b3 = __ballot(zm[3] != 0);
            const int total = (int)(__popcll(b0) + __popcll(b1) + __popcll(b2) + __popcll(b3));
            if (total != 0) {
                int base = 0;
                if (lane == 0) base = atomicAdd(&s_nlist, total);
                base = __builtin_amdgcn_readfirstlane(base);
                const int code = (c << 10) | (cy4 << 6) | gi;
                int pos = rank_below(b0, rank_below(b1, rank_below(b2, rank_below(b3, base))));
#pragma unroll
                for (int j = 0; j < 4; j++)
                    if (zm[j] != 0) {
                        s_recz[pos] = zm[j]; s_pairs[pos] = (uint16_t)(code | (j << 4));
                        pos++;
                    }
                if (max((int)zacc.x, (int)zacc.y) >= zini) s_ini[c] = 1;
            }
            if constexpr (BITMAP) cy4 += T / 32;
            else {
                gi += egi; cy4 += ecy; c += ec;
                if (gi >= ngr) { gi -= ngr; cy4++; }
                if (cy4 >= hc4) { cy4 -= hc4; c++; }
            }
        }
        if (lane == 0 && nquad) atomicAdd(&s_ncorner, nquad);
#if MYSLAM_FAST_PHASE == 5
        return;
#endif
    }
    __syncthreads();
    MYSLAM_BT_MARK(2);
    if constexpr (NS > 1) asm volatile("s_waitcnt vmcnt(0)" ::: "memory");
    if ((unsigned)tid == 0 && sampled) {
        atomicAdd(&ctl.cur[level * 4], (uint32_t)(dense ? s_ncorner : min(s_npair, NPAIR)));
        atomicAdd(&ctl.cur[level * 4 + 1], (uint32_t)pairs_total);
        ctl.cur[level * 4 + 2] = dense ? 1u : 0u;
    }
    const uint8_t* mimg = maskPyr ? maskPyr + (size_t)b * pyrStride + g.imgOff : nullptr;
    uint32_t* out = cand + (size_t)b * P.totalKeyCap + g.keyOff;
    if (dense) {
        const int nrec = min(s_nlist, NLIST);
        for (int i0 = 0; i0 < nrec; i0 += T) {
            if (i0 + (int)((unsigned)tid & ~63u) >= nrec) continue;
            const int i = i0 + (unsigned)tid;
            uint32_t z = 0;
            int px0 = 0, py = 0, ini = 0;
            if (i < nrec) {
                const int code = s_pairs[i], c = code >> 10;
                z = s_recz[i];
                px0 = 4 * (code & 15) + 3 + (cj0 + c) * g.wCell;
                py = ((code >> 4) & 63) + 3 + ci * g.hCell;
                ini = s_ini[c];
            }
            uint32_t kp[2];
            unsigned long long bm[2];
            bool passk[2];
#pragma unroll
            for (int k = 0; k < 2; k++) {
                const uint32_t h = k ? z >> 16 : z & 0xffffu;
                const uint32_t second = h >> 8;
                const int sc = (int)(second ? second : h) + zoff;
                const int px = px0 + 2 * k + (second ? 1 : 0);
                bool pass = h != 0 && !(ini && sc < P.iniTh);
                if (pass && mimg) pass = mimg[(size_t)py * g.pitch + px] != 0;
                kp[k] = ((uint32_t)py << 20) | ((uint32_t)px << 8) | (uint32_t)sc;
                bm[k] = __ballot(pass); passk[k] = pass;
            }
            const int total = (int)(__popcll(bm[0]) + __popcll(bm[1]));
            if (total == 0) continue;
            int gbase = 0;
            if (lane == 0) gbase = atomicAdd(&candCount[b * MAXL + level], total);
            gbase = __builtin_amdgcn_readfirstlane(gbase);
            int dst = rank_below(bm[0], rank_below(bm[1], gbase));
            if (passk[0]) {
                if (dst < g.keyCap) out[dst] = kp[0];
                dst++;
            }
            if (passk[1]) {
                if (dst < g.keyCap) out[dst] = kp[1];
            }
        }
    } else {
    const int nl = min(s_nlist, NLIST);
    for (int i0 = 0; i0 < nl; i0 += T) {
        const int i = i0 + (unsigned)tid;
        bool pass = false;
        uint32_t kp = 0;
        if (i < nl) {
            const uint32_t e = s_list[i];
            const int sc = (int)(e & 0xff) + zoff;
            kp = (e & 0xffffff00u) | (uint32_t)sc;
            pass = !(s_ini[s_listc[i]] && sc < P.iniTh);
            if (pass && mimg) pass = mimg[(size_t)(e >> 20) * g.pitch + ((e >> 8) & 0xfff)] != 0;
        }
        const unsigned long long bm = __ballot(pass);
        if (bm == 0) continue;
        int gbase = 0;
        if (lane == 0) gbase = atomicAdd(&candCount[b * MAXL + level], __popcll(bm));
        gbase = __builtin_amdgcn_readfirstlane(gbase);
        if (pass) {
            const int dst = gbase + __popcll(bm & ((1ull << lane) - 1ull));
            if (dst < g.keyCap) out[dst] = kp;
        }
    }
    }
    rec = rec_next; par ^= (NS > 1 ? 1 : 0);
  }
}

constexpr int OT_MAXB = 1024;

__device__ __forceinline__ uint64_t wave_incl_scan64(uint64_t v) {
#define MYSLAM_SCAN64_STEP(CTRL, ROWS)                                                                                   \
    {                                                                                                                    \
        const uint32_t l2 = (uint32_t)__builtin_amdgcn_update_dpp(0, (int)(uint32_t)v, CTRL, ROWS, 0xf, false);          \
        const uint32_t h2 = (uint32_t)__builtin_amdgcn_update_dpp(0, (int)(uint32_t)(v >> 32), CTRL, ROWS, 0xf, false);  \
        v += ((uint64_t)h2 << 32) | l2;                                                                                  \
    }
    MYSLAM_SCAN64_STEP(0x111, 0xf)
    MYSLAM_SCAN64_STEP(0x112, 0xf)
    MYSLAM_SCAN64_STEP(0x114, 0xf)
    MYSLAM_SCAN64_STEP(0x118, 0xf)
    MYSLAM_SCAN64_STEP(0x142, 0xa)
    MYSLAM_SCAN64_STEP(0x143, 0xc)
#undef MYSLAM_SCAN64_STEP
    return v;
}

template <int OT>
__device__ __forceinline__ uint64_t block_excl_scan64(uint64_t v, uint64_t* s_w, uint64_t& total) {
    const int lane = threadIdx.x & 63, wid = threadIdx.x >> 6;
    const uint64_t incl = wave_incl_scan64(v);
    __syncthreads();
    if (lane == 63) s_w[wid] = incl;
    __syncthreads();
    uint64_t base = 0, tot = 0;
#pragma unroll
    for (int w = 0; w < OT / 64; w++) { const uint64_t x = s_w[w]; if (w < wid) base += x; tot += x; }
    total = tot;
    return base + incl - v;
}

__device__ __forceinline__ uint32_t oct_code(int px, int py, const LevelGeom& g) {
    int r = (int)__fdiv_rn((float)px, g.hX);
    r = min(max(r, 0), g.nIni - 1);
    int ULx = (int)__fmul_rn(g.hX, (float)r), URx = (int)__fmul_rn(g.hX, (float)(r + 1));
    int ULy = 0, BRy = g.maxBY - MIN_BORDER;
    uint32_t code = (uint32_t)r << ROOT_SHIFT;
    for (int k = 1; k <= g.ndepth; k++) {
        const int midX = ULx + ((URx - ULx + 1) >> 1);
        const int midY = ULy + ((BRy - ULy + 1) >> 1);
        const uint32_t dx = px >= midX, dy = py >= midY;
        code |= (dx | (dy << 1)) << (ROOT_SHIFT - 2 * k);
        if (dx) ULx = midX; else URx = midX;
        if (dy) ULy = midY; else BRy = midY;
    }
    return code;
}

__device__ __noinline__ void partition4(uint32_t* __restrict__ S, uint32_t* __restrict__ Cd, int lo, int hi, int sh, int& b1, int& b2, int& b3) {
    int c0 = 0, c1 = 0, c2 = 0;
    for (int i = lo; i < hi; i++) {
        const int d = (int)((Cd[i] >> sh) & 3);
        c0 += (d == 0); c1 += (d == 1); c2 += (d == 2);
    }
    b1 = lo + c0; b2 = b1 + c1; b3 = b2 + c2;
    int p0 = lo, p1 = b1, p2 = b2, p3 = b3;
    auto take = [&](int d) -> int { int r; if (d == 0) r = p0++; else if (d == 1) r = p1++; else if (d == 2) r = p2++; else r = p3++; return r; };
    const int ends[4] = {b1, b2, b3, hi};
#pragma unroll
    for (int k = 0; k < 3; k++) {
        int i = (k == 0) ? p0 : (k == 1) ? p1 : p2;
        while (i < ends[k]) {
            uint32_t v = S[i], cv = Cd[i];
            int d = (int)((cv >> sh) & 3);
            while (d != k) {
                const int j = take(d);
                const uint32_t w = S[j], cw = Cd[j];
                S[j] = v; Cd[j] = cv; v = w; cv = cw;
                d = (int)((cv >> sh) & 3);
            }
            S[i] = v; Cd[i] = cv;
            i++;
            if (k == 0) p0 = i; else if (k == 1) p1 = i; else p2 = i;
        }
    }
}

struct OctLds {
    uint32_t *lo0, *lo1, *hi0, *hi1;
    uint16_t *pfx0, *pfx1;
    uint8_t *dep0, *dep1;
    uint32_t *nb1, *nb2, *nb3;
    uint32_t *ckey0, *ckey1;
    uint16_t *cpos0, *cpos1;
    uint16_t* ord;
    uint16_t *kinc, *binc;
    uint8_t* kk;
    uint8_t* mark;
    uint32_t* offs;
    __device__ __forceinline__ uint32_t* lo(int i) const { return i ? lo1 : lo0; }
    __device__ __forceinline__ uint32_t* hi(int i) const { return i ? hi1 : hi0; }
    __device__ __forceinline__ uint16_t* pfx(int i) const { return i ? pfx1 : pfx0; }
    __device__ __forceinline__ uint8_t* dep(int i) const { return i ? dep1 : dep0; }
    __device__ __forceinline__ uint32_t* ckey(int i) const { return i ? ckey1 : ckey0; }
    __device__ __forceinline__ uint16_t* cpos(int i) const { return i ? cpos1 : cpos0; }
};

__device__ __forceinline__ void child_bounds(const OctLds& L, uint32_t* __restrict__ S, uint32_t* __restrict__ Cd, int D, int lo, int hi, int d, int pfx,
                                             int& b1, int& b2, int& b3) {
    if (d < D) {
        const int sb = 2 * (D - d - 1);
        const int base = pfx << 2;
        b1 = L.offs[(base + 1) << sb]; b2 = L.offs[(base + 2) << sb]; b3 = L.offs[(base + 3) << sb];
    } else {
        partition4(S, Cd, lo, hi, ROOT_SHIFT - 2 * (d + 1), b1, b2, b3);
    }
}

__device__ __forceinline__ uint32_t half_row_max_u32(uint32_t v) {
    v = max(v, (uint32_t)__builtin_amdgcn_update_dpp(0, (int)v, 0x141, 0xf, 0xf, false));
    v = max(v, (uint32_t)__builtin_amdgcn_update_dpp(0, (int)v, 0xb1, 0xf, 0xf, false));
    v = max(v, (uint32_t)__builtin_amdgcn_update_dpp(0, (int)v, 0x4e, 0xf, 0xf, false));
    return v;
}

__device__ __forceinline__ int sel_order_bin(uint32_t pay, int ts) {
    const int tx = (int)((pay >> 8) & 0xfff) >> ts, ty = (int)(pay >> 20) >> ts;
    int z = 0;
#pragma unroll
    for (int k = 0; k < 4; k++) z |= (((tx >> k) & 1) << (2 * k)) | (((ty >> k) & 1) << (2 * k + 1));
    return ((tx >> 4) << 8) | z;
}

constexpr int OCT_WIDE_BELOW = 64;
constexpr int OCT_FL = 4;
template <int OT>
__global__ __launch_bounds__(OT) void k_octree(OrbPlan P, const uint32_t* __restrict__ cand,
                                               const int32_t* __restrict__ candCount, uint32_t* __restrict__ sortbuf,
                                               const uint32_t* __restrict__ octTab,
                                               uint32_t* __restrict__ selOut, int32_t* __restrict__ selCount,
                                               int32_t* __restrict__ status, int NCmax, uint16_t* __restrict__ order, BlurMulti BM) {
    MYSLAM_SIDE_PRIO();
    MYSLAM_BT(2);
    extern __shared__ __attribute__((aligned(16))) uint8_t smem[];
    const int t = threadIdx.x;
    if constexpr (OT == 512) {
        if ((int)blockIdx.y >= P.nlevels) {
            const int wv = __builtin_amdgcn_readfirstlane(t >> 6);
            blur7_strip_wave(BM, ((int)blockIdx.y - P.nlevels) * 8 + wv, blockIdx.x, smem + wv * (16 * B3_TS));
            return;
        }
    }
    const int level = blockIdx.y, b = blockIdx.x;
    const LevelGeom& g = P.lv[level];
    const int NC = NCmax;

    uint64_t* s_w = reinterpret_cast<uint64_t*>(smem);
    int* s_i = reinterpret_cast<int*>(smem + 128);
    uint8_t* pcur = smem + 192;
    uint32_t* s_cursor = reinterpret_cast<uint32_t*>(pcur); pcur += 4 * OT_MAXB;
    OctLds L;
    L.offs = reinterpret_cast<uint32_t*>(pcur); pcur += 4 * (OT_MAXB + 2);
    uint32_t* const s_tab = reinterpret_cast<uint32_t*>(pcur);
    L.lo0 = reinterpret_cast<uint32_t*>(pcur); pcur += 4 * NC;
    L.lo1 = reinterpret_cast<uint32_t*>(pcur); pcur += 4 * NC;
    L.hi0 = reinterpret_cast<uint32_t*>(pcur); pcur += 4 * NC;
    L.hi1 = reinterpret_cast<uint32_t*>(pcur); pcur += 4 * NC;
    L.nb1 = reinterpret_cast<uint32_t*>(pcur); pcur += 4 * NC;
    L.nb2 = reinterpret_cast<uint32_t*>(pcur); pcur += 4 * NC;
    L.nb3 = reinterpret_cast<uint32_t*>(pcur); pcur += 4 * NC;
    L.ckey0 = reinterpret_cast<uint32_t*>(pcur); pcur += 4 * NC;
    L.ckey1 = reinterpret_cast<uint32_t*>(pcur); pcur += 4 * NC;
    L.pfx0 = reinterpret_cast<uint16_t*>(pcur); pcur += 2 * NC;
    L.pfx1 = reinterpret_cast<uint16_t*>(pcur); pcur += 2 * NC;
    L.cpos0 = reinterpret_cast<uint16_t*>(pcur); pcur += 2 * NC;
    L.cpos1 = reinterpret_cast<uint16_t*>(pcur); pcur += 2 * NC;
    L.ord = reinterpret_cast<uint16_t*>(pcur); pcur += 2 * NC;
    L.kinc = reinterpret_cast<uint16_t*>(pcur); pcur += 2 * NC;
    L.binc = reinterpret_cast<uint16_t*>(pcur); pcur += 2 * NC;
    L.dep0 = pcur; pcur += NC;
    L.dep1 = pcur; pcur += NC;
    L.kk = pcur; pcur += NC;
    L.mark = pcur; pcur += NC;

    const int cnt = candCount[b * MAXL + level];
    int32_t* myCount = selCount + b * MAXL + level;
    if (cnt > g.keyCap) {
        if (t == 0) { *myCount = 0; status[b] = MYSLAM_ERR_CAPACITY; }
        return;
    }
    const int n = cnt;
    if (n == 0) { if (t == 0) *myCount = 0; return; }

    const uint32_t* keys = cand + (size_t)b * P.totalKeyCap + g.keyOff;
    uint32_t* S = sortbuf + ((size_t)b * P.totalKeyCap + g.keyOff) * 2;
    uint32_t* Cd = S + g.keyCap;
    const int D = g.sortDepth;
    const int NB = g.nIni << (2 * D);
    const int bsh = ROOT_SHIFT - 2 * D;

    const uint32_t* xcode = octTab + g.tabOff; const uint32_t* ycode = xcode + g.tabX;
    const uint32_t* xcell = ycode + g.tabY; const uint32_t* ycell = xcell + g.tabX;
    const int ntab = 2 * (g.tabX + g.tabY);
    const bool tabLds = (size_t)ntab * 4 <= (size_t)54 * NC;
    for (int i = t; i < NB; i += OT) s_cursor[i] = 0;
    if (tabLds) for (int i = t; i < ntab; i += OT) s_tab[i] = xcode[i];
    __syncthreads();
    const bool rankkey = g.nCols * g.nRows <= 1024;
    const float inv_ncols = 1.0f / (float)g.nCols;
    auto passes = [&](auto in_lds) __attribute__((always_inline)) {
        constexpr bool LDS = decltype(in_lds)::value;
        const int oyc = g.tabX, oxl = g.tabX + g.tabY, oyl = 2 * g.tabX + g.tabY;
        auto XC = [&](uint32_t i) -> uint32_t { if constexpr (LDS) return s_tab[i]; else return xcode[i]; };
        auto YC = [&](uint32_t i) -> uint32_t { if constexpr (LDS) return s_tab[oyc + i]; else return ycode[i]; };
        auto XL = [&](uint32_t i) -> uint32_t { if constexpr (LDS) return s_tab[oxl + i]; else return xcell[i]; };
        auto YL = [&](uint32_t i) -> uint32_t { if constexpr (LDS) return s_tab[oyl + i]; else return ycell[i]; };
        for (int i0 = t; i0 < n; i0 += OCT_FL * OT) {
            uint32_t pay[OCT_FL], cx[OCT_FL], cy[OCT_FL];
#pragma unroll
            for (int u = 0; u < OCT_FL; u++) pay[u] = (i0 + u * OT < n) ? keys[i0 + u * OT] : 0u;
#pragma unroll
            for (int u = 0; u < OCT_FL; u++) { cx[u] = XC((pay[u] >> 8) & 0xfff); cy[u] = YC(pay[u] >> 20); }
#pragma unroll
            for (int u = 0; u < OCT_FL; u++)
                if (i0 + u * OT < n) atomicAdd(&s_cursor[(cx[u] | cy[u]) >> bsh], 1u);
        }
        __syncthreads();
        {
            const int c = (NB + OT - 1) / OT;
            const int beg = min(NB, t * c), end = min(NB, beg + c);
            uint64_t sum = 0;
            for (int i = beg; i < end; i++) sum += s_cursor[i];
            uint64_t total;
            uint64_t run = block_excl_scan64<OT>(sum, s_w, total);
            for (int i = beg; i < end; i++) {
                const uint32_t h = s_cursor[i];
                L.offs[i] = (uint32_t)run;
                s_cursor[i] = (uint32_t)run;
                run += h;
            }
            if (t == 0) L.offs[NB] = (uint32_t)n;
        }
        __syncthreads();
        for (int i0 = t; i0 < n; i0 += OCT_FL * OT) {
            uint32_t pay[OCT_FL], cx[OCT_FL], cy[OCT_FL], qx[OCT_FL], qy[OCT_FL];
#pragma unroll
            for (int u = 0; u < OCT_FL; u++) pay[u] = (i0 + u * OT < n) ? keys[i0 + u * OT] : 0u;
#pragma unroll
            for (int u = 0; u < OCT_FL; u++) {
                const uint32_t px = (pay[u] >> 8) & 0xfff, py = pay[u] >> 20;
                cx[u] = XC(px); cy[u] = YC(py);
                qx[u] = rankkey ? XL(px) : 0u; qy[u] = rankkey ? YL(py) : 0u;
            }
#pragma unroll
            for (int u = 0; u < OCT_FL; u++) {
                if (i0 + u * OT >= n) continue;
                uint32_t low = pay[u];
                if (rankkey) {
                    const int px = (int)((pay[u] >> 8) & 0xfff), py = (int)(pay[u] >> 20);
                    const int ci = (int)(((float)qy[u] + 0.5f) * inv_ncols);
                    const uint32_t pxc = (uint32_t)(px - 3 - (int)qx[u] * g.wCell), pyc = (uint32_t)(py - 3 - ci * g.hCell);
                    low = ((pay[u] & 0xffu) << 22) | (0x3fffffu - (((qy[u] + qx[u]) << 12) | (pyc << 6) | pxc));
                }
                const uint32_t code = cx[u] | cy[u];
                const uint32_t pos = atomicAdd(&s_cursor[code >> bsh], 1u);
                S[pos] = low; Cd[pos] = code;
            }
        }
        __syncthreads();
    };
    if (tabLds) passes(std::true_type{}); else passes(std::false_type{});

    MYSLAM_BT_MARK(0);
    MYSLAM_BT_AUX((unsigned long long)level | ((unsigned long long)n << 8));
    if (t == 0) {
        int m = 0;
        for (int r = 0; r < g.nIni; r++) {
            const int lo = L.offs[r << (2 * D)], hi = L.offs[(r + 1) << (2 * D)];
            if (hi > lo) { L.lo0[m] = (uint32_t)lo; L.hi0[m] = (uint32_t)hi; L.dep0[m] = 0; L.pfx0[m] = (uint16_t)r; m++; }
        }
        s_i[0] = m; s_i[1] = 0;
    }
    __syncthreads();

    int cur = 0, ccur = 0, mode = 0;
    const int N = g.N;
    for (int round = 0; round < 96; round++) {
        const int m = s_i[0];
        const int prevSize = m;
        int newM;
        if (mode == 0) {
            const int c = (m + OT - 1) / OT;
            const int beg = min(m, t * c), end = min(m, beg + c);
            uint64_t packed = 0;
            for (int p = beg; p < end; p++) {
                const int lo = (int)L.lo(cur)[p], hi = (int)L.hi(cur)[p], d = L.dep(cur)[p];
                int k = 0;
                if (hi - lo > 1 && d < g.ndepth) {
                    int b1, b2, b3;
                    child_bounds(L, S, Cd, D, lo, hi, d, L.pfx(cur)[p], b1, b2, b3);
                    L.nb1[p] = (uint32_t)b1; L.nb2[p] = (uint32_t)b2; L.nb3[p] = (uint32_t)b3;
                    const int c0 = b1 - lo, c1 = b2 - b1, c2 = b3 - b2, c3 = hi - b3;
                    k = (c0 > 0) + (c1 > 0) + (c2 > 0) + (c3 > 0);
                    const int big = (c0 > 1) + (c1 > 1) + (c2 > 1) + (c3 > 1);
                    packed += (uint64_t)k | ((uint64_t)big << 42);
                } else {
                    packed += 1ull << 21;
                }
                L.kk[p] = (uint8_t)k;
            }
            uint64_t total;
            uint64_t run = block_excl_scan64<OT>(packed, s_w, total);
            const int Ktot = (int)(total & 0x1fffff), Ntot = (int)((total >> 21) & 0x1fffff), Btot = (int)(total >> 42);
            const int nxt = cur ^ 1, cnxt = ccur ^ 1;
            for (int p = beg; p < end; p++) {
                const int lo = (int)L.lo(cur)[p], hi = (int)L.hi(cur)[p], d = L.dep(cur)[p];
                const int pf = L.pfx(cur)[p];
                const int k = L.kk[p];
                if (k) {
                    const int bnd[5] = {lo, (int)L.nb1[p], (int)L.nb2[p], (int)L.nb3[p], hi};
                    const int rk = (int)(run & 0x1fffff);
                    int pos = Ktot - (rk + k);
                    int cidx = (int)(run >> 42);
                    int childPos[4];
#pragma unroll
                    for (int q = 3; q >= 0; q--) {
                        childPos[q] = pos;
                        if (bnd[q + 1] > bnd[q]) {
                            L.lo(nxt)[pos] = (uint32_t)bnd[q]; L.hi(nxt)[pos] = (uint32_t)bnd[q + 1];
                            L.dep(nxt)[pos] = (uint8_t)(d + 1);
                            L.pfx(nxt)[pos] = (uint16_t)((pf << 2) | q);
                            pos++;
                        }
                    }
#pragma unroll
                    for (int q = 0; q < 4; q++) {
                        const int sz = bnd[q + 1] - bnd[q];
                        if (sz > 1) {
                            L.ckey(cnxt)[cidx] = ((uint32_t)sz << 14) | (uint32_t)cidx;
                            L.cpos(cnxt)[cidx] = (uint16_t)childPos[q];
                            cidx++;
                        }
                    }
                    const int big = cidx - (int)(run >> 42);
                    run += (uint64_t)k | ((uint64_t)big << 42);
                } else {
                    const int rn = (int)((run >> 21) & 0x1fffff);
                    L.lo(nxt)[Ktot + rn] = (uint32_t)lo; L.hi(nxt)[Ktot + rn] = (uint32_t)hi;
                    L.dep(nxt)[Ktot + rn] = (uint8_t)d;
                    L.pfx(nxt)[Ktot + rn] = (uint16_t)pf;
                    run += 1ull << 21;
                }
            }
            newM = Ktot + Ntot;
            __syncthreads();
            if (t == 0) { s_i[0] = newM; s_i[1] = Btot; }
            cur = nxt; ccur = cnxt;
            __syncthreads();
            if (newM >= N || newM == prevSize) break;
            if (newM + 3 * Btot > N) mode = 1;
        } else {
            const int nc = s_i[1];
            if (nc == 0) break;
            for (int ci = t; ci < nc; ci += OT) {
                const uint32_t key = L.ckey(ccur)[ci];
                int rank = 0;
                for (int cj = 0; cj < nc; cj++) rank += (L.ckey(ccur)[cj] > key);
                L.ord[rank] = (uint16_t)ci;
            }
            for (int p = t; p < m; p += OT) L.mark[p] = 0;
            if (t == 0) s_i[2] = nc - 1;
            __syncthreads();
            const int c = (nc + OT - 1) / OT;
            const int beg = min(nc, t * c), end = min(nc, beg + c);
            uint64_t packed = 0;
            for (int j = beg; j < end; j++) {
                const int p = L.cpos(ccur)[L.ord[j]];
                const int lo = (int)L.lo(cur)[p], hi = (int)L.hi(cur)[p], d = L.dep(cur)[p];
                int k = 1, big = 1, b1 = hi, b2 = hi, b3 = hi;
                if (d < g.ndepth) {
                    child_bounds(L, S, Cd, D, lo, hi, d, L.pfx(cur)[p], b1, b2, b3);
                    const int c0 = b1 - lo, c1 = b2 - b1, c2 = b3 - b2, c3 = hi - b3;
                    k = (c0 > 0) + (c1 > 0) + (c2 > 0) + (c3 > 0);
                    big = (c0 > 1) + (c1 > 1) + (c2 > 1) + (c3 > 1);
                }
                L.nb1[j] = (uint32_t)b1; L.nb2[j] = (uint32_t)b2; L.nb3[j] = (uint32_t)b3;
                L.kk[j] = (uint8_t)(k | (big << 4));
                packed += (uint64_t)k | ((uint64_t)big << 32);
            }
            uint64_t total;
            uint64_t run = block_excl_scan64<OT>(packed, s_w, total);
            for (int j = beg; j < end; j++) {
                const int k = L.kk[j] & 15, big = L.kk[j] >> 4;
                run += (uint64_t)k | ((uint64_t)big << 32);
                const int kincl = (int)(run & 0xffffffffu);
                L.kinc[j] = (uint16_t)kincl;
                L.binc[j] = (uint16_t)(run >> 32);
                if (m + kincl - (j + 1) >= N) atomicMin(&s_i[2], j);
            }
            __syncthreads();
            const int ncmt = min(s_i[2] + 1, nc);
            const int Kc = L.kinc[ncmt - 1];
            const int nxt = cur ^ 1, cnxt = ccur ^ 1;
            for (int j = t; j < ncmt; j += OT) L.mark[L.cpos(ccur)[L.ord[j]]] = 1;
            __syncthreads();
            for (int j = t; j < ncmt; j += OT) {
                const int p = L.cpos(ccur)[L.ord[j]];
                const int lo = (int)L.lo(cur)[p], hi = (int)L.hi(cur)[p], d = L.dep(cur)[p];
                const int pf = L.pfx(cur)[p];
                const int big = L.kk[j] >> 4;
                const int bnd[5] = {lo, (int)L.nb1[j], (int)L.nb2[j], (int)L.nb3[j], hi};
                int pos = Kc - L.kinc[j];
                int childPos[4];
                if (d < g.ndepth) {
#pragma unroll
                    for (int q = 3; q >= 0; q--) {
                        childPos[q] = pos;
                        if (bnd[q + 1] > bnd[q]) {
                            L.lo(nxt)[pos] = (uint32_t)bnd[q]; L.hi(nxt)[pos] = (uint32_t)bnd[q + 1];
                            L.dep(nxt)[pos] = (uint8_t)(d + 1);
                            L.pfx(nxt)[pos] = (uint16_t)((pf << 2) | q);
                            pos++;
                        }
                    }
                    int cidx = L.binc[j] - big;
#pragma unroll
                    for (int q = 0; q < 4; q++) {
                        const int sz = bnd[q + 1] - bnd[q];
                        if (sz > 1) {
                            L.ckey(cnxt)[cidx] = ((uint32_t)sz << 14) | (uint32_t)cidx;
                            L.cpos(cnxt)[cidx] = (uint16_t)childPos[q];
                            cidx++;
                        }
                    }
                } else {
                    L.lo(nxt)[pos] = (uint32_t)lo; L.hi(nxt)[pos] = (uint32_t)hi; L.dep(nxt)[pos] = (uint8_t)d; L.pfx(nxt)[pos] = (uint16_t)pf;
                    const int cidx = L.binc[j] - 1;
                    L.ckey(cnxt)[cidx] = ((uint32_t)(hi - lo) << 14) | (uint32_t)cidx;
                    L.cpos(cnxt)[cidx] = (uint16_t)pos;
                }
            }
            {
                const int c2 = (m + OT - 1) / OT;
                const int pb = min(m, t * c2), pe = min(m, pb + c2);
                uint64_t un = 0;
                for (int p = pb; p < pe; p++) un += (L.mark[p] == 0);
                uint64_t tot2;
                uint64_t ex = block_excl_scan64<OT>(un, s_w, tot2);
                for (int p = pb; p < pe; p++) {
                    if (L.mark[p] == 0) {
                        L.lo(nxt)[Kc + (int)ex] = L.lo(cur)[p]; L.hi(nxt)[Kc + (int)ex] = L.hi(cur)[p];
                        L.dep(nxt)[Kc + (int)ex] = L.dep(cur)[p];
                        L.pfx(nxt)[Kc + (int)ex] = L.pfx(cur)[p];
                        ex++;
                    }
                }
            }
            newM = Kc + (m - ncmt);
            const int newNc = L.binc[ncmt - 1];
            __syncthreads();
            if (t == 0) { s_i[0] = newM; s_i[1] = newNc; }
            cur = nxt; ccur = cnxt;
            __syncthreads();
            if (newM >= N || newM == prevSize) break;
        }
    }

    MYSLAM_BT_MARK(1);
    const int m = s_i[0];
    uint32_t* out = selOut + (size_t)b * P.totalOut + g.outBase;
    {
        const int GLN = rankkey ? 8 : 16;
        const int sub = t & (GLN - 1);
        const int mm = min(m, g.nodeCap);
        const int ngrp = OT / GLN;
        for (int p0 = t / GLN; p0 < ((mm + ngrp - 1) / ngrp) * ngrp; p0 += ngrp) {
            const bool live = p0 < mm;
            const int lo = live ? (int)L.lo(cur)[p0] : 0, hi = live ? (int)L.hi(cur)[p0] : 0;
            if (rankkey) {
                uint32_t bk = 0;
#pragma unroll 4
                for (int i = lo + 4 * sub; i < hi; i += 32) {
                    uint4 k4;
                    __builtin_memcpy(&k4, S + i, 16);
                    const int left = hi - i;
                    bk = max(bk, k4.x);
                    bk = max(bk, left > 1 ? k4.y : 0u);
                    bk = max(bk, left > 2 ? k4.z : 0u);
                    bk = max(bk, left > 3 ? k4.w : 0u);
                }
                bk = half_row_max_u32(bk);
                if (live && sub == 0) {
                    const uint32_t rank = 0x3fffffu - (bk & 0x3fffffu), cell = rank >> 12;
                    const int ci = (int)(((float)cell + 0.5f) * inv_ncols), cj = (int)cell - ci * g.nCols;
                    const uint32_t px = (rank & 63u) + 3u + (uint32_t)(cj * g.wCell), py = ((rank >> 6) & 63u) + 3u + (uint32_t)(ci * g.hCell);
                    out[p0] = (py << 20) | (px << 8) | (bk >> 22);
                }
                continue;
            }
            uint32_t best = 0;
#pragma unroll 2
            for (int i = lo + sub; i < hi; i += 16) best = max(best, S[i] & 0xffu);
#pragma unroll
            for (int o = 1; o < 16; o <<= 1) best = max(best, (uint32_t)__shfl_xor((int)best, o, 64));
            uint64_t bo = ~0ull;
            for (int i = lo + sub; i < hi; i += 16) {
                const uint32_t pay = S[i];
                if ((pay & 0xffu) != best) continue;
                const uint32_t px = (pay >> 8) & 0xfff, py = pay >> 20;
                bo = min(bo, ((uint64_t)(ycell[py] + xcell[px]) << 24) | ((uint64_t)py << 12) | (uint64_t)px);
            }
#pragma unroll
            for (int o = 1; o < 16; o <<= 1) bo = min(bo, (uint64_t)__shfl_xor((unsigned long long)bo, o, 64));
            if (live && sub == 0) out[p0] = ((uint32_t)((bo >> 12) & 0xfff) << 20) | ((uint32_t)(bo & 0xfff) << 8) | best;
        }
    }
    if (t == 0) *myCount = min(m, g.nodeCap);
    MYSLAM_BT_MARK(2);
    if (order) {
        __threadfence_block();
        __syncthreads();
        int* s_hist = reinterpret_cast<int*>(s_cursor);
        int* s_ws = reinterpret_cast<int*>(s_w);
        const int n = min(m, g.nodeCap);
        int ts = 4;
        while ((g.w >> ts) >= 64 || (g.h >> ts) >= 16) ts++;
        uint16_t* ord = order + (size_t)b * P.totalOut + g.outBase;
        for (int i = t; i < 1024; i += OT) s_hist[i] = 0;
        __syncthreads();
        for (int i = t; i < n; i += OT) atomicAdd(&s_hist[sel_order_bin(__hip_atomic_load(&out[i], __ATOMIC_RELAXED, __HIP_MEMORY_SCOPE_AGENT), ts)], 1);
        __syncthreads();
        int base = 0, v0 = 0, v1 = 0, v2 = 0, v = 0, incl = 0;
        if (t < 256) {
            v0 = s_hist[4 * t]; v1 = s_hist[4 * t + 1]; v2 = s_hist[4 * t + 2];
            v = v0 + v1 + v2 + s_hist[4 * t + 3];
            incl = v;
#pragma unroll
            for (int o = 1; o < 64; o <<= 1) { const int nb = __shfl_up(incl, o, 64); if ((t & 63) >= o) incl += nb; }
            if ((t & 63) == 63) s_ws[t >> 6] = incl;
        }
        __syncthreads();
        if (t < 256) {
            base = incl - v;
            for (int w = 0; w < (t >> 6); w++) base += s_ws[w];
            s_hist[4 * t] = base; s_hist[4 * t + 1] = base + v0; s_hist[4 * t + 2] = base + v0 + v1; s_hist[4 * t + 3] = base + v0 + v1 + v2;
        }
        __syncthreads();
        for (int i = t; i < n; i += OT) ord[atomicAdd(&s_hist[sel_order_bin(__hip_atomic_load(&out[i], __ATOMIC_RELAXED, __HIP_MEMORY_SCOPE_AGENT), ts)], 1)] = (uint16_t)i;
    }
}

__device__ __forceinline__ float fast_atan2_deg(float y, float x) {
    const float p1 = 0.9997878412794807f * (float)(180 / 3.14159265358979323846);
    const float p3 = -0.3258083974640975f * (float)(180 / 3.14159265358979323846);
    const float p5 = 0.1555786518463281f * (float)(180 / 3.14159265358979323846);
    const float p7 = -0.04432655554792128f * (float)(180 / 3.14159265358979323846);
    const float eps = (float)2.2204460492503131e-16;
    const float ax = fabsf(x), ay = fabsf(y);
    float a, c, c2;
    if (ax >= ay) {
        c = __fdiv_rn(ay, __fadd_rn(ax, eps));
        c2 = __fmul_rn(c, c);
        a = __fmul_rn(__fadd_rn(__fmul_rn(__fadd_rn(__fmul_rn(__fadd_rn(__fmul_rn(p7, c2), p5), c2), p3), c2), p1), c);
    } else {
        c = __fdiv_rn(ax, __fadd_rn(ay, eps));
        c2 = __fmul_rn(c, c);
        a = __fsub_rn(90.f, __fmul_rn(__fadd_rn(__fmul_rn(__fadd_rn(__fmul_rn(__fadd_rn(__fmul_rn(p7, c2), p5), c2), p3), c2), p1), c));
    }
    if (x < 0) a = __fsub_rn(180.f, a);
    if (y < 0) a = __fsub_rn(360.f, a);
    return a;
}

__device__ __forceinline__ void det_sincos(float rad, float& s_out, float& c_out) {
    const double x = (double)rad;
    const double kd = rint(__dmul_rn(x, 0.6366197723675814));
    const int k = (int)kd;
    const double y = __dsub_rn(__dsub_rn(x, __dmul_rn(kd, 1.5707963267948966)), __dmul_rn(kd, 6.123233995736766e-17));
    const double y2 = __dmul_rn(y, y);
    double ps = -7.647163731819816e-13;
    ps = __dadd_rn(__dmul_rn(ps, y2), 1.6059043836821613e-10);
    ps = __dadd_rn(__dmul_rn(ps, y2), -2.505210838544172e-08);
    ps = __dadd_rn(__dmul_rn(ps, y2), 2.7557319223985893e-06);
    ps = __dadd_rn(__dmul_rn(ps, y2), -0.0001984126984126984);
    ps = __dadd_rn(__dmul_rn(ps, y2), 0.008333333333333333);
    ps = __dadd_rn(__dmul_rn(ps, y2), -0.16666666666666666);
    const double sn = __dadd_rn(y, __dmul_rn(y, __dmul_rn(y2, ps)));
    double pc = 4.779477332387385e-14;
    pc = __dadd_rn(__dmul_rn(pc, y2), -1.1470745597729725e-11);
    pc = __dadd_rn(__dmul_rn(pc, y2), 2.08767569878681e-09);
    pc = __dadd_rn(__dmul_rn(pc, y2), -2.755731922398589e-07);
    pc = __dadd_rn(__dmul_rn(pc, y2), 2.48015873015873e-05);
    pc = __dadd_rn(__dmul_rn(pc, y2), -0.001388888888888889);
    pc = __dadd_rn(__dmul_rn(pc, y2), 0.041666666666666664);
    pc = __dadd_rn(__dmul_rn(pc, y2), -0.5);
    const double cs = __dadd_rn(1.0, __dmul_rn(y2, pc));
    double s, c;
    switch (k & 3) {
        case 0: s = sn; c = cs; break;
        case 1: s = cs; c = -sn; break;
        case 2: s = -sn; c = -cs; break;
        default: s = -cs; c = sn; break;
    }
    s_out = (float)s;
    c_out = (float)c;
}

__device__ __forceinline__ float wave_ic_angle(const uint8_t* __restrict__ img, int pitch, int x, int y) {
    const int lane = threadIdx.x & 63;
    int m10 = 0, m01 = 0;
    const int r = lane >> 1;
    if (r < 31) {
        const int v = r - 15;
        const int d = c_umax[v < 0 ? -v : v];
        const uint8_t* row = img + (size_t)(y + v) * pitch + x;
        const int u0 = (lane & 1) ? 1 : -d, u1 = (lane & 1) ? d : 0;
        int sI = 0;
        for (int u = u0; u <= u1; u++) { const int I = row[u]; m10 += u * I; sI += I; }
        m01 = v * sI;
    }
    m10 = wave_reduce_sum(m10);
    m01 = wave_reduce_sum(m01);
    return fast_atan2_deg((float)m01, (float)m10);
}

template <bool TILED = false>
__device__ __forceinline__ uint32_t wave_brief(const uint8_t* __restrict__ img, int pitch, int x, int y, float angle_deg) {
    const int lane = threadIdx.x & 63;
    const float factorPI = (float)(3.14159265358979323846 / 180.f);
    const float ang = __fmul_rn(angle_deg, factorPI);
    float a, b;
    det_sincos(ang, b, a);
    const uint8_t* center = img + (size_t)y * pitch + x;
    uint32_t nib = 0;
#pragma unroll
    for (int j = 0; j < 4; j++) {
        const int8_t* pp = &c_pattern[(lane * 4 + j) * 4];
        const float x0 = (float)pp[0], y0 = (float)pp[1], x1 = (float)pp[2], y1 = (float)pp[3];
        const int r0 = __float2int_rn(__fadd_rn(__fmul_rn(x0, b), __fmul_rn(y0, a)));
        const int c0 = __float2int_rn(__fsub_rn(__fmul_rn(x0, a), __fmul_rn(y0, b)));
        const int r1 = __float2int_rn(__fadd_rn(__fmul_rn(x1, b), __fmul_rn(y1, a)));
        const int c1 = __float2int_rn(__fsub_rn(__fmul_rn(x1, a), __fmul_rn(y1, b)));
        const int t0 = TILED ? img[tiled_off(x + c0, y + r0, pitch)] : center[r0 * pitch + c0];
        const int t1 = TILED ? img[tiled_off(x + c1, y + r1, pitch)] : center[r1 * pitch + c1];
        nib |= (uint32_t)(t0 < t1) << j;
    }
    uint32_t byte = nib | (__shfl_down(nib, 1, 64) << 4);
    uint32_t w = byte | (__shfl_down(byte, 2, 64) << 8);
    w |= (__shfl_down(byte, 4, 64) << 16) | (__shfl_down(byte, 6, 64) << 24);
    return w;
}

constexpr int DB_R = 18, DB_ROWS = 2 * DB_R + 1, DB_P = 64;
constexpr int DB_N = DB_ROWS * 4;
constexpr int DB_IT = 3;


template <int CTRL, int ROW_MASK>
__device__ __forceinline__ int dpp_add_i32(int v) { return v + __builtin_amdgcn_update_dpp(0, v, CTRL, ROW_MASK, 0xf, false); }
__device__ __forceinline__ int wave_sum_lane63_i32(int v) {
    v = dpp_add_i32<0xB1, 0xf>(v); v = dpp_add_i32<0x4E, 0xf>(v); v = dpp_add_i32<0x141, 0xf>(v); v = dpp_add_i32<0x140, 0xf>(v);
    v = dpp_add_i32<0x142, 0xa>(v); v = dpp_add_i32<0x143, 0xc>(v);
    return v;
}

constexpr int KD_KPB = 64;
#ifndef MYSLAM_KD_GLDS
#define MYSLAM_KD_GLDS 2
#endif

__global__ __launch_bounds__(256) void k_sel_order(OrbPlan P, const uint32_t* __restrict__ selOut, const int32_t* __restrict__ selCount,
                                                   uint16_t* __restrict__ order, int batch) {
    constexpr int NB = 1024;
    __shared__ int s_hist[NB], s_wsum[4];
    const int level = blockIdx.x, b = blockIdx.y, t = threadIdx.x;
    const LevelGeom& g = P.lv[level];
    const int n = min(selCount[b * MAXL + level], g.nodeCap);
    int ts = 4;
    while ((g.w >> ts) >= 64 || (g.h >> ts) >= 16) ts++;
    const uint32_t* sel = selOut + (size_t)b * P.totalOut + g.outBase;
    uint16_t* out = order + (size_t)b * P.totalOut + g.outBase;
    for (int i = t; i < NB; i += 256) s_hist[i] = 0;
    __syncthreads();
    auto bin_of = [&](uint32_t pay) -> int { return sel_order_bin(pay, ts); };
    for (int i = t; i < n; i += 256) atomicAdd(&s_hist[bin_of(sel[i])], 1);
    __syncthreads();
    {
        const int v0 = s_hist[4 * t], v1 = s_hist[4 * t + 1], v2 = s_hist[4 * t + 2], v3 = s_hist[4 * t + 3];
        const int v = v0 + v1 + v2 + v3;
        int incl = v;
#pragma unroll
        for (int o = 1; o < 64; o <<= 1) { const int nb = __shfl_up(incl, o, 64); if ((t & 63) >= o) incl += nb; }
        if ((t & 63) == 63) s_wsum[t >> 6] = incl;
        __syncthreads();
        int base = incl - v;
        for (int w = 0; w < (t >> 6); w++) base += s_wsum[w];
        s_hist[4 * t] = base; s_hist[4 * t + 1] = base + v0; s_hist[4 * t + 2] = base + v0 + v1; s_hist[4 * t + 3] = base + v0 + v1 + v2;
    }
    __syncthreads();
    for (int i = t; i < n; i += 256) out[atomicAdd(&s_hist[bin_of(sel[i])], 1)] = (uint16_t)i;
}
// ... 277 lines not shown
}

__device__ __forceinline__ bool is_fast_corner(const uint8_t* __restrict__ img, int pitch, int x, int y, int th) {
    constexpr int RX[16] = {0, 1, 2, 3, 3, 3, 2, 1, 0, -1, -2, -3, -3, -3, -2, -1};
    constexpr int RY[16] = {3, 3, 2, 1, 0, -1, -2, -3, -3, -3, -2, -1, 0, 1, 2, 3};
    th = min(max(th, 0), 255);
    const uint8_t* p = img + (size_t)y * pitch + x;
    const int v = p[0];
    unsigned dm = 0, bm = 0;
#pragma unroll
    for (int k = 0; k < 16; k++) {
        const int pv = p[RX[k] + RY[k] * pitch];
        dm |= (unsigned)(pv < v - th) << k;
        bm |= (unsigned)(pv > v + th) << k;
    }
    auto run9 = [](unsigned m) {
        unsigned x = m | (m << 16);
        unsigned r = x & (x >> 1);
        r &= r >> 2;
        r &= r >> 4;
        r &= x >> 8;
        return (r & 0xffffu) != 0;
    };
    return run9(dm) || run9(bm);
}

__global__ __launch_bounds__(256) void k_screen(OrbPlan P, const uint8_t* __restrict__ pyr, myslam_keypoint* __restrict__ kin,
                                                int n, myslam_keypoint* __restrict__ kout, uint8_t* __restrict__ keep) {
    const int i = blockIdx.x * 4 + (threadIdx.x >> 6);
    const int lane = threadIdx.x & 63;
    if (i >= n) return;
    myslam_keypoint k = kin[i];
    const int level = k.octave;
    if (level < 0 || level >= P.nlevels) { if (lane == 0) keep[i] = 0; return; }
    const LevelGeom& g = P.lv[level];
    const float scale = g.scale;
    k.x = __fdiv_rn(k.x, scale); k.y = __fdiv_rn(k.y, scale);
    bool ok = (__fsub_rn(k.y, (float)EDGE_THRESHOLD) >= 0 && __fadd_rn(k.y, (float)EDGE_THRESHOLD) < (float)g.h &&
               __fsub_rn(k.x, (float)EDGE_THRESHOLD) >= 0 && __fadd_rn(k.x, (float)EDGE_THRESHOLD) < (float)g.w);
    const uint8_t* img = pyr + g.imgOff;
    int px = 0, py = 0;
    if (ok) {
        px = __float2int_rn(k.x); py = __float2int_rn(k.y);
        ok = is_fast_corner(img, g.pitch, px, py, P.minTh);
    }
    if (ok) {
        k.angle = wave_ic_angle(img, g.pitch, px, py);
        k.size = __fmul_rn((float)PATCH_SIZE, scale);
    }
    k.x = __fmul_rn(k.x, scale); k.y = __fmul_rn(k.y, scale);
    if (lane == 0) { kin[i] = k; kout[i] = k; keep[i] = ok ? 1 : 0; }
}

__global__ __launch_bounds__(256) void k_calc_desc(OrbPlan P, const uint8_t* __restrict__ blur, const myslam_keypoint* __restrict__ kps,
                                                   int n, uint8_t* __restrict__ desc) {
    const int i = blockIdx.x * 4 + (threadIdx.x >> 6);
    const int lane = threadIdx.x & 63;
    if (i >= n) return;
    const myslam_keypoint k = kps[i];
    const int level = min(max(k.octave, 0), P.nlevels - 1);
    const LevelGeom& g = P.lv[level];
    const int px = __float2int_rn(__fdiv_rn(k.x, g.scale)), py = __float2int_rn(__fdiv_rn(k.y, g.scale));
    const uint32_t w = wave_brief<true>(blur + g.imgOff, g.pitch, px, py, k.angle);
    if ((lane & 7) == 0) reinterpret_cast<uint32_t*>(desc + (size_t)i * 32)[lane >> 3] = w;
}

__device__ __forceinline__ int pkf_count(const PkfArgs& a, int b) { return min(max(a.nFeat[b], 0), a.featCap); }

__global__ __launch_bounds__(256) void k_pkf_screen(OrbPlan P, PkfArgs a) {
    const int b = blockIdx.y, r = blockIdx.x * 4 + (threadIdx.x >> 6);
    const int lane = threadIdx.x & 63;
    const int n = pkf_count(a, b);
    if (r >= n * P.nlevels) return;
    const int i = r / P.nlevels, level = r - i * P.nlevels;
    const LevelGeom& g = P.lv[level];
    const float scale = g.scale;
    const float* xy = a.featXy + ((size_t)b * a.featCap + i) * 2;
    myslam_keypoint k;
    k.x = __fdiv_rn(xy[0], scale); k.y = __fdiv_rn(xy[1], scale);
    bool ok = (__fsub_rn(k.y, (float)EDGE_THRESHOLD) >= 0 && __fadd_rn(k.y, (float)EDGE_THRESHOLD) < (float)g.h &&
               __fsub_rn(k.x, (float)EDGE_THRESHOLD) >= 0 && __fadd_rn(k.x, (float)EDGE_THRESHOLD) < (float)g.w);
    const uint8_t* img = a.pyr + (size_t)b * a.pyrStride + g.imgOff;
    int px = 0, py = 0;
    if (ok) {
        px = __float2int_rn(k.x); py = __float2int_rn(k.y);
        ok = is_fast_corner(img, g.pitch, px, py, P.minTh);
    }
    const size_t row = (size_t)b * a.rowCap + r;
    if (ok) {
        k.angle = wave_ic_angle(img, g.pitch, px, py);
        k.size = __fmul_rn((float)PATCH_SIZE, scale);
        k.x = __fmul_rn(k.x, scale); k.y = __fmul_rn(k.y, scale);
        k.response = -1.f; k.octave = level; k.class_id = i;
        if (lane == 0) a.rows[row] = k;
    }
    if (lane == 0) a.keep[row] = ok ? 1 : 0;
}

__global__ __launch_bounds__(256) void k_pkf_compact(OrbPlan P, PkfArgs a) {
    __shared__ int s_w[4];
    const int b = blockIdx.x, t = threadIdx.x, lane = t & 63, wv = t >> 6;
    const int total = pkf_count(a, b) * P.nlevels;
    const uint8_t* keep = a.keep + (size_t)b * a.rowCap;
    const myslam_keypoint* rows = a.rows + (size_t)b * a.rowCap;
    int mine = 0;
    for (int r = t; r < total; r += 256) mine += keep[r];
    mine = wave_reduce_sum(mine);
    if (lane == 0) s_w[wv] = mine;
    __syncthreads();
    const int kept = s_w[0] + s_w[1] + s_w[2] + s_w[3];
    if (kept > a.cap) {
        if (t == 0) { a.counts[b] = 0; a.status[b] = MYSLAM_ERR_CAPACITY; }
        return;
    }
    myslam_keypoint* out = a.outKps + (size_t)b * a.cap;
    int done = 0;
    for (int base = 0; base < total; base += 256) {
        const int r = base + t;
        const bool f = r < total && keep[r] != 0;
        const unsigned long long m = __ballot(f);
        __syncthreads();
        if (lane == 0) s_w[wv] = __popcll(m);
        __syncthreads();
        int before = 0, sum = 0;
#pragma unroll
        for (int k = 0; k < 4; k++) { const int c = s_w[k]; if (k < wv) before += c; sum += c; }
        if (f) out[done + before + __popcll(m & ((1ull << lane) - 1ull))] = rows[r];
        done += sum;
    }
    if (t == 0) { a.counts[b] = kept; a.status[b] = MYSLAM_OK; }
}

__global__ __launch_bounds__(256) void k_pkf_describe(OrbPlan P, PkfArgs a) {
    const int b = blockIdx.y, slot = blockIdx.x * 4 + (threadIdx.x >> 6);
    const int lane = threadIdx.x & 63;
    if (slot >= min(a.counts[b], a.cap)) return;
    const myslam_keypoint k = a.outKps[(size_t)b * a.cap + slot];
    const int level = min(max(k.octave, 0), P.nlevels - 1);
    const LevelGeom& g = P.lv[level];
    const int px = __float2int_rn(__fdiv_rn(k.x, g.scale)), py = __float2int_rn(__fdiv_rn(k.y, g.scale));
    const uint32_t w = wave_brief<true>(a.blur + (size_t)b * a.pyrStride + g.imgOff, g.pitch, px, py, k.angle);
    if ((lane & 7) == 0) reinterpret_cast<uint32_t*>(a.outDesc + ((size_t)b * a.cap + slot) * 32)[lane >> 3] = w;
}

__global__ void k_unpack_cands(const uint32_t* __restrict__ cand, int n, int32_t* xs, int32_t* ys, int32_t* sc) {
    const int i = blockIdx.x * blockDim.x + threadIdx.x;
    if (i >= n) return;
    const uint32_t p = cand[i];
    xs[i] = (p >> 8) & 0xfff; ys[i] = p >> 20; sc[i] = p & 0xff;
}

__device__ __forceinline__ void zero_part(const ZeroArgs& z, int tid, int T) {
#pragma unroll
    for (int k = 0; k < 4; k++)
        for (int i = tid; i < z.n[k]; i += T) z.p[k][i] = 0u;
}
__device__ __forceinline__ void ingest_part(const uint8_t* __restrict__ src, int rows, int cols, int step, size_t sstride,
                                            uint8_t* __restrict__ dst, int dpitch, size_t dstride, int tpr, int rpb, int bx, int by, int b) {
    const int y = by * rpb + (int)threadIdx.x / tpr;
    const int x16 = (bx * 256 + (int)threadIdx.x % tpr) * 16;
    if ((int)threadIdx.x >= tpr * rpb || y >= rows || x16 >= cols) return;
    const uint8_t* s = src + (size_t)b * sstride + (size_t)y * step + x16;
    const uint32_t sh = (uint32_t)(reinterpret_cast<uintptr_t>(s) & 3);
    const uint32_t* sa = reinterpret_cast<const uint32_t*>(s - sh);
    const int nvalid = cols - x16;
    uint32_t d[5];
#pragma unroll
    for (int j = 0; j < 5; j++) d[j] = (4 * j < (int)sh + nvalid) ? sa[j] : 0u;
    uint4 o;
    o.x = __builtin_amdgcn_alignbyte(d[1], d[0], sh); o.y = __builtin_amdgcn_alignbyte(d[2], d[1], sh);
    o.z = __builtin_amdgcn_alignbyte(d[3], d[2], sh); o.w = __builtin_amdgcn_alignbyte(d[4], d[3], sh);
    uint8_t* q = dst + (size_t)b * dstride + (size_t)y * dpitch + x16;
    if (x16 + 16 <= dpitch) *reinterpret_cast<uint4*>(q) = o;
    else { uint32_t w[4] = {o.x, o.y, o.z, o.w}; for (int j = 0; j < 4 && x16 + 4 * j < dpitch; j++) reinterpret_cast<uint32_t*>(q)[j] = w[j]; }
}
__global__ __launch_bounds__(256) void k_ingest(const uint8_t* __restrict__ src, int rows, int cols, int step, size_t sstride,
                                                uint8_t* __restrict__ dst, int dpitch, size_t dstride, int tpr, int rpb, ZeroArgs z) {
    zero_part(z, (int)((blockIdx.z * gridDim.y + blockIdx.y) * gridDim.x + blockIdx.x) * 256 + (int)threadIdx.x, (int)(gridDim.x * gridDim.y * gridDim.z) * 256);
    ingest_part(src, rows, cols, step, sstride, dst, dpitch, dstride, tpr, rpb, blockIdx.x, blockIdx.y, blockIdx.z);
}

struct IngestPart { const uint8_t* src; int rows, cols, step; size_t sstride; uint8_t* dst; int dpitch; size_t dstride; int tpr, rpb, gx, b0; };
__global__ __launch_bounds__(256) void k_pyr_head(ResizeChain c, IngestPart g, ZeroArgs z) {
    const int blk = blockIdx.x, b = blockIdx.y;
    zero_part(z, (int)(blockIdx.y * gridDim.x + blockIdx.x) * 256 + (int)threadIdx.x, (int)(gridDim.x * gridDim.y) * 256);
    if (blk < c.blk0[RC_MAX]) { rc_block(c, blk, b); return; }
    if (b < g.b0) return;
    const int ib = blk - c.blk0[RC_MAX];
    ingest_part(g.src, g.rows, g.cols, g.step, g.sstride, g.dst, g.dpitch, g.dstride, g.tpr, g.rpb, ib % g.gx, ib / g.gx, b);
}

__global__ __launch_bounds__(256) void k_zero_u32(ZeroArgs a) {
    const int i = blockIdx.x * 256 + threadIdx.x;
#pragma unroll
    for (int k = 0; k < 4; k++)
        if (a.p[k] && i < a.n[k]) a.p[k][i] = 0u;
}
void launch_zero_u32(const ZeroArgs& z, hipStream_t s) {
    const int n = max(max(z.n[0], z.n[1]), max(z.n[2], z.n[3]));
    if (n > 0) hipLaunchKernelGGL(k_zero_u32, dim3((n + 255) / 256), dim3(256), 0, s, z);
}

void launch_ingest(const uint8_t* src, int rows, int cols, int step, size_t sstride, uint8_t* dst, int dpitch, size_t dstride, int batch,
                   const ZeroArgs& z, hipStream_t s) {
    const int t = (cols + 15) / 16;
    const int tpr = t < 256 ? t : 256, rpb = t < 256 ? 256 / t : 1;
    dim3 grid((t + 255) / 256, (rows + rpb - 1) / rpb, batch);
    hipLaunchKernelGGL(k_ingest, grid, dim3(256), 0, s, src, rows, cols, step, sstride, dst, dpitch, dstride, tpr, rpb, z);
}

bool resize_uses_strips(const ResizeArgs& a) { return a.scale_y >= 1.0 && a.scale_y <= 1.25 && a.scale_x <= 1.6; }

bool resize_is_little(const ResizeArgs& a, int batch) { return a.n0 == 0 && (size_t)batch * a.dw * a.dh < (size_t)1500000; }

#ifndef MYSLAM_RESIZE_CHAIN_MAX
#define MYSLAM_RESIZE_CHAIN_MAX 3
#endif
int resize_chain_max() { return MYSLAM_RESIZE_CHAIN_MAX < RC_MAX ? MYSLAM_RESIZE_CHAIN_MAX : RC_MAX; }

static ResizeChain make_chain(const ResizeArgs* lv, int n) {
    ResizeChain c;
    c.src = lv[0].src; c.sw = lv[0].sw; c.sh = lv[0].sh; c.spitch = lv[0].spitch; c.sstride = lv[0].sstride;
    c.n = n; c.dstride = lv[0].dstride; c.blk0[0] = 0;
    for (int j = 0; j < RC_MAX; j++) {
        const ResizeArgs& a = lv[j < n ? j : n - 1];
        c.dst[j] = a.dst; c.dw[j] = a.dw; c.dh[j] = a.dh; c.dpitch[j] = a.dpitch; c.scale_x[j] = a.scale_x; c.scale_y[j] = a.scale_y;
        c.blk0[j + 1] = c.blk0[j] + (j < n ? (((a.dw + 3) / 4) * (4 / rc_px(j + 1)) * a.dh + 255) / 256 : 0);
    }
    return c;
}
void launch_resize_chain(const ResizeArgs* lv, int n, int batch, hipStream_t s) {
    const ResizeChain c = make_chain(lv, n);
    hipLaunchKernelGGL(k_resize_chain, dim3(c.blk0[RC_MAX], batch), dim3(256), 0, s, c);
}
void launch_pyr_head(const ResizeArgs* lv, int n, int rows, int cols, uint8_t* dst0, int dpitch0, size_t dstride0, int b0, int batch,
                     const ZeroArgs& z, hipStream_t s) {
    const ResizeChain c = make_chain(lv, n);
    const int t = (cols + 15) / 16;
    IngestPart g{lv[0].src, rows, cols, lv[0].spitch, lv[0].sstride, dst0, dpitch0, dstride0, t < 256 ? t : 256, t < 256 ? 256 / t : 1, (t + 255) / 256, b0};
    const int iblocks = g.gx * ((rows + g.rpb - 1) / g.rpb);
    hipLaunchKernelGGL(k_pyr_head, dim3(c.blk0[RC_MAX] + iblocks, batch), dim3(256), 0, s, c, g, z);
}
#ifndef MYSLAM_PYR_HEAD_LEVELS
#define MYSLAM_PYR_HEAD_LEVELS 2
#endif
int pyr_head_levels() { return MYSLAM_PYR_HEAD_LEVELS < 3 ? MYSLAM_PYR_HEAD_LEVELS : 3; }

void launch_resize(const ResizeArgs& a, int batch, hipStream_t s) {
    const bool little = resize_is_little(a, batch);
    if (resize_uses_strips(a) && !little) {
        if (!a.colTab || !a.rowTab) { fprintf(stderr, "myslam_hip: launch_resize: the plan holds no resize tables for this level\n"); abort(); }
        const int nstrips = (a.dw + 255) / 256, band = RS_BAND, nbands = (a.dh + band - 1) / band;
        hipLaunchKernelGGL(k_resize_strip, dim3((nstrips * nbands + 3) / 4, 1, batch), dim3(256), 0, s, a, nstrips, nbands, band);
        return;
    }
    dim3 grid((a.dw + 255) / 256, (a.dh + 3) / 4, batch);
    hipLaunchKernelGGL(k_resize, grid, dim3(256), 0, s, a);
}

bool blur_uses_strips(const BlurArgs& a) {
    return a.w >= 8 && a.h >= 8 && (a.spitch & 3) == 0 && ((reinterpret_cast<uintptr_t>(a.src) | a.sstride) & 3) == 0;
}

enum class BlurForm { Mfma, Strip, Tile };
static BlurForm blur_form(const BlurArgs& a) {
    if (a.tabH && a.tabV && a.ident && a.dtiled && (a.dpitch & 15) == 0 && ((reinterpret_cast<uintptr_t>(a.dst) | a.dstride) & 15) == 0) return BlurForm::Mfma;
    return blur_uses_strips(a) ? BlurForm::Strip : BlurForm::Tile;
}
static void blur_multi_add(BlurMulti& M, const BlurArgs& a) {
    const int nstrips = (a.w + 255) / 256, nbands = (a.h + B3_R - 1) / B3_R;
    M.a[M.n] = a; M.nstrips[M.n] = nstrips; M.wave0[M.n + 1] = M.wave0[M.n] + nstrips * nbands; M.n++;
}

void launch_blur_levels(const BlurArgs* lv, int n, int batch, hipStream_t s) {
    BlurMulti M; M.n = 0; M.wave0[0] = 0;
    BlurMfmaMulti X; X.n = 0; X.wave0[0] = 0;
    for (int i = 0; i < n; i++) {
        const BlurArgs& a = lv[i];
        switch (blur_form(a)) {
            case BlurForm::Mfma:
                X.a[X.n] = a; X.tabHOff[X.n] = 0; X.tabVOff[X.n] = 0; X.wave0[X.n + 1] = X.wave0[X.n] + (a.w + 31) / 32; X.n++;
                break;
            case BlurForm::Strip: blur_multi_add(M, a); break;
            case BlurForm::Tile:
                hipLaunchKernelGGL(k_blur7_dot, dim3((a.w + B2_W - 1) / B2_W, (a.h + B2_H - 1) / B2_H, batch), dim3(256), 0, s, a);
                break;
        }
    }
    if (M.n) hipLaunchKernelGGL(k_blur7_strip, dim3((M.wave0[M.n] + 3) / 4, 1, batch), dim3(256), 0, s, M);
    if (X.n) hipLaunchKernelGGL(k_blur7_mfma, dim3((X.wave0[X.n] + 3) / 4, 1, batch), dim3(256), 0, s, X);
}

#ifndef MYSLAM_BLUR_WITH_OCTREE
#define MYSLAM_BLUR_WITH_OCTREE 1
#endif
static bool blur_multi_for_octree(const BlurArgs* lv, int n, int batch, BlurMulti& M) {
    if (!MYSLAM_BLUR_WITH_OCTREE || batch >= OCT_WIDE_BELOW || batch >= 16) return false;
    M.n = 0; M.wave0[0] = 0;
    for (int i = 0; i < n; i++) {
        if (blur_form(lv[i]) != BlurForm::Strip) return false;
        blur_multi_add(M, lv[i]);
    }
    return M.n > 0;
}

void launch_fast(const OrbPlan& P, const uint8_t* pyr, size_t pyrStride, const uint8_t* maskPyr, uint32_t* cand,
                 int32_t* candCount, const uint32_t* statPrev, uint32_t* statCur, int forceMode, int batch, hipStream_t s) {
    int cw = 0, ch = 0;
    for (int l = 0; l < P.nlevels; l++) { cw = max(cw, P.lv[l].wCell); ch = max(ch, P.lv[l].hCell); }
    const FastCtl ctl{statPrev, statCur, forceMode};
    const dim3 grid((unsigned)P.nstrips * (unsigned)batch);
    constexpr int pad = FastLds<32, 4, 40>::PAD;
#if MYSLAM_FAST_NS > 1
    if (cw <= 32 && ch <= 40 && (size_t)P.nstrips * batch >= (size_t)MYSLAM_FAST_NS * 256 * 6 * 4) {
        const dim3 gridms((unsigned)(((size_t)P.nstrips * batch + MYSLAM_FAST_NS - 1) / MYSLAM_FAST_NS));
        constexpr int padms = FastLds<32, 4, 40, MYSLAM_FAST_NS>::PAD + FastLds<32, 4, 40, MYSLAM_FAST_NS>::TROWS * FastLds<32, 4, 40, MYSLAM_FAST_NS>::TP + 16;
        hipLaunchKernelGGL((k_fast_strip<32, 4, 40, MYSLAM_FAST_NS>), gridms, dim3(256), padms, s, P, pyr, pyrStride, maskPyr, cand, candCount, ctl, batch);
        return;
    }
#endif
    if (cw <= 32 && ch <= 40) hipLaunchKernelGGL((k_fast_strip<32, 4, 40>), grid, dim3(256), pad, s, P, pyr, pyrStride, maskPyr, cand, candCount, ctl, batch);
    else if (max(cw, ch) <= 40) hipLaunchKernelGGL((k_fast_strip<40, 4>), grid, dim3(256), 0, s, P, pyr, pyrStride, maskPyr, cand, candCount, ctl, batch);
    else hipLaunchKernelGGL((k_fast_strip<MAX_CELL, 4>), grid, dim3(256), 0, s, P, pyr, pyrStride, maskPyr, cand, candCount, ctl, batch);
}

size_t octree_lds_bytes(int nodeCap) { return 192 + 4 * (size_t)OT_MAXB + 4 * (size_t)(OT_MAXB + 2) + (size_t)nodeCap * 54 + 16; }

bool launch_octree(const OrbPlan& P, const uint32_t* cand, const int32_t* candCount, uint32_t* sortbuf, const uint32_t* octTab, uint32_t* selOut,
                   int32_t* selCount, int32_t* status, int batch, uint16_t* order, hipStream_t s, const BlurArgs* blurLv, int nBlur) {
    BlurMulti BMh;
    const BlurMulti* blurWith = (blurLv && nBlur > 0 && blur_multi_for_octree(blurLv, nBlur, batch, BMh)) ? &BMh : nullptr;
    int ncmax = 0;
    for (int l = 0; l < P.nlevels; l++) ncmax = max(ncmax, P.lv[l].nodeCap);
    const size_t lds = std::max(octree_lds_bytes(ncmax), (size_t)8 * 16 * B3_TS);
    (void)hipFuncSetAttribute(reinterpret_cast<const void*>(k_octree<256>), hipFuncAttributeMaxDynamicSharedMemorySize, 160 * 1024);
    (void)hipFuncSetAttribute(reinterpret_cast<const void*>(k_octree<512>), hipFuncAttributeMaxDynamicSharedMemorySize, 160 * 1024);
    if (batch >= OCT_WIDE_BELOW)
        hipLaunchKernelGGL(k_octree<256>, dim3(batch, P.nlevels), dim3(256), lds, s, P, cand, candCount, sortbuf, octTab, selOut, selCount, status, ncmax, order, BlurMulti{});
    else
    {
        BlurMulti M = blurWith ? *blurWith : BlurMulti{};
        if (!blurWith) M.n = 0;
        const int brows = blurWith ? (M.wave0[M.n] + 7) / 8 : 0;
        hipLaunchKernelGGL(k_octree<512>, dim3(batch, P.nlevels + brows), dim3(512), lds, s, P, cand, candCount, sortbuf, octTab, selOut, selCount, status, ncmax, order, M);
    }
    return blurWith != nullptr;
}

bool describe_uses_tile_order(bool have_order, int detectOnly, int batch) { return have_order && !detectOnly && batch >= 8; }

void launch_describe(const OrbPlan& P, const uint8_t* pyr, const uint8_t* blur, size_t pyrStride, const uint32_t* selOut,
                     const int32_t* selCount, myslam_keypoint* kps, uint8_t* desc, int32_t* counts, int32_t* status,
                     int cap, int detectOnly, int batch, uint16_t* order, bool order_ready, int blocks_per_cu, hipStream_t s) {
    const int slots = min(cap, P.totalOut);
    const int nchunk = (slots + KD_KPB - 1) / KD_KPB;
    const bool tiled = describe_uses_tile_order(order != nullptr, detectOnly, batch);
    if (tiled && !order_ready) hipLaunchKernelGGL(k_sel_order, dim3(P.nlevels, batch), dim3(256), 0, s, P, selOut, selCount, order, batch);
    const int total = nchunk * batch;
    const int grid = blocks_per_cu > 0 ? min(total, 256 * blocks_per_cu) : total;
    hipLaunchKernelGGL(k_describe2, dim3(grid), dim3(256), 0, s, P, pyr, blur, pyrStride, selOut, selCount,
                       kps, desc, counts, status, cap, nchunk, batch, detectOnly, tiled ? order : nullptr);
}

void launch_screen(const OrbPlan& P, const uint8_t* pyr, myslam_keypoint* kin, int n, myslam_keypoint* kout, uint8_t* keep,
                   hipStream_t s) {
    hipLaunchKernelGGL(k_screen, dim3((n + 3) / 4), dim3(256), 0, s, P, pyr, kin, n, kout, keep);
}

void launch_calc_desc(const OrbPlan& P, const uint8_t* blur, const myslam_keypoint* kps, int n, uint8_t* desc, hipStream_t s) {
    hipLaunchKernelGGL(k_calc_desc, dim3((n + 3) / 4), dim3(256), 0, s, P, blur, kps, n, desc);
}

void launch_process_keyframes(const OrbPlan& P, const PkfArgs& a, int batch, hipStream_t s) {
    hipLaunchKernelGGL(k_pkf_screen, dim3((a.rowCap + 3) / 4, batch), dim3(256), 0, s, P, a);
    hipLaunchKernelGGL(k_pkf_compact, dim3(batch), dim3(256), 0, s, P, a);
    hipLaunchKernelGGL(k_pkf_describe, dim3((min(a.cap, a.rowCap) + 3) / 4, batch), dim3(256), 0, s, P, a);
}

void launch_unpack_cands(const uint32_t* cand, int n, int32_t* xs, int32_t* ys, int32_t* sc, hipStream_t s) {
    if (n <= 0) return;
    hipLaunchKernelGGL(k_unpack_cands, dim3((n + 255) / 256), dim3(256), 0, s, cand, n, xs, ys, sc);
}

}

#ifdef MYSLAM_BLOCK_TRACE
extern "C" int myslam_debug_block_trace(void* d_buf, unsigned cap_records, unsigned* n) {
    using namespace myslam_hip;
    unsigned long long* p = (unsigned long long*)d_buf;
    const unsigned zero = 0;
    if (n) MYSLAM_HIP_CHECK(hipMemcpyFromSymbol(n, HIP_SYMBOL(g_bt_n), sizeof(unsigned)));
    if (d_buf) MYSLAM_HIP_CHECK(hipMemcpyToSymbol(HIP_SYMBOL(g_bt_n), &zero, sizeof(unsigned)));
    MYSLAM_HIP_CHECK(hipMemcpyToSymbol(HIP_SYMBOL(g_bt_cap), &cap_records, sizeof(unsigned)));
    MYSLAM_HIP_CHECK(hipMemcpyToSymbol(HIP_SYMBOL(g_bt_buf), &p, sizeof(p)));
    return MYSLAM_OK;
}
#endif
```

### a-simple-stereo-slam-system-with-deep-loop-closing_amd/csrc/orb_launch.h

```cpp
#pragma once
#include <vector>

#include "common.h"
#include "orb_plan.h"

namespace myslam_hip {

struct ZeroArgs { uint32_t* p[4]; int n[4]; };

void gauss_q8(int kind, int q[7]);

void launch_zero_u32(const ZeroArgs& z, hipStream_t s);
void launch_ingest(const uint8_t* src, int rows, int cols, int step, size_t sstride, uint8_t* dst, int dpitch, size_t dstride, int batch,
                   const ZeroArgs& z, hipStream_t s);

bool resize_uses_strips(const ResizeArgs& a);
bool resize_is_little(const ResizeArgs& a, int batch);
int resize_chain_max();
int pyr_head_levels();
void launch_resize(const ResizeArgs& a, int batch, hipStream_t s);
void launch_resize_chain(const ResizeArgs* lv, int n, int batch, hipStream_t s);
void launch_pyr_head(const ResizeArgs* lv, int n, int rows, int cols, uint8_t* dst0, int dpitch0, size_t dstride0, int b0, int batch,
                     const ZeroArgs& z, hipStream_t s);

bool blur_uses_strips(const BlurArgs& a);
void launch_blur_levels(const BlurArgs* lv, int n, int batch, hipStream_t s);
bool blur_mfma_tables(int w, int h, const int q[7], std::vector<uint4>& tab, size_t& offH, size_t& offV);
void blur_mfma_ident(std::vector<uint4>& tab, size_t& offI);

void launch_fast(const OrbPlan& P, const uint8_t* pyr, size_t pyrStride, const uint8_t* maskPyr, uint32_t* cand,
                 int32_t* candCount, const uint32_t* statPrev, uint32_t* statCur, int forceMode, int batch, hipStream_t s);
size_t octree_lds_bytes(int nodeCap);
bool launch_octree(const OrbPlan& P, const uint32_t* cand, const int32_t* candCount, uint32_t* sortbuf, const uint32_t* octTab, uint32_t* selOut,
                   int32_t* selCount, int32_t* status, int batch, uint16_t* order, hipStream_t s, const BlurArgs* blurLv, int nBlur);
bool describe_uses_tile_order(bool have_order, int detectOnly, int batch);
void launch_describe(const OrbPlan& P, const uint8_t* pyr, const uint8_t* blur, size_t pyrStride, const uint32_t* selOut,
                     const int32_t* selCount, myslam_keypoint* kps, uint8_t* desc, int32_t* counts, int32_t* status,
                     int cap, int detectOnly, int batch, uint16_t* order, bool order_ready, int blocks_per_cu, hipStream_t s);
void launch_screen(const OrbPlan& P, const uint8_t* pyr, myslam_keypoint* kin, int n, myslam_keypoint* kout, uint8_t* keep,
                   hipStream_t s);
void launch_calc_desc(const OrbPlan& P, const uint8_t* blur, const myslam_keypoint* kps, int n, uint8_t* desc, hipStream_t s);

struct PkfArgs {
    const uint8_t* pyr; const uint8_t* blur; size_t pyrStride;
    const float* featXy; const int32_t* nFeat; int featCap;
    myslam_keypoint* rows; uint8_t* keep; int rowCap;
    myslam_keypoint* outKps; uint8_t* outDesc; int32_t* counts; int32_t* status; int cap;
};
void launch_process_keyframes(const OrbPlan& P, const PkfArgs& a, int batch, hipStream_t s);
void launch_unpack_cands(const uint32_t* cand, int n, int32_t* xs, int32_t* ys, int32_t* sc, hipStream_t s);

}
```

### include/myslam_hip.h

```cpp
#ifndef MYSLAM_HIP_H
#define MYSLAM_HIP_H

#include <stddef.h>
#include <stdint.h>

#ifdef __cplusplus
extern "C" {
#endif

#define MYSLAM_OK 0
#define MYSLAM_ERR_INVALID (-1)
#define MYSLAM_ERR_HIP (-2)
#define MYSLAM_ERR_CAPACITY (-3)
#define MYSLAM_ERR_UNSUPPORTED (-4)

typedef struct myslam_keypoint {
    float x, y, size, angle, response;
    int32_t octave, class_id;
} myslam_keypoint;

#define MYSLAM_DESC_BYTES 32
#define MYSLAM_LCD_DIM 1064

int myslam_hip_device_count(void);
const char* myslam_hip_version(void);
int myslam_prof_shader_clock_mhz(void* hip_stream, float spin_us, float* mhz);
int myslam_prof_enable(int on);
int myslam_prof_reset(void);
int myslam_prof_count(void);
int myslam_prof_get(int i, const char** name, double* total_ms, long* launches);
int myslam_debug_peek(const void* d_ptr, void* out, size_t n);

typedef struct myslam_orb myslam_orb;

int myslam_orb_create(myslam_orb** out, int nfeatures, float scale_factor, int nlevels,
                      int ini_th_fast, int min_th_fast);
int myslam_orb_destroy(myslam_orb* h);
int myslam_orb_set_stream(myslam_orb* h, void* hip_stream);
int myslam_orb_set_fast_event(myslam_orb* h, void* hip_event);
int myslam_orb_set_fast_gate(myslam_orb* h, void* hip_event);
#define MYSLAM_ORB_OPT_FAST_MODE 1
#define MYSLAM_ORB_OPT_INTERNAL_STREAM 2
#define MYSLAM_ORB_OPT_STOP_AFTER 3
#define MYSLAM_ORB_OPT_COPY_INPUT 4
#define MYSLAM_ORB_OPT_BLUR_MFMA 5
#define MYSLAM_ORB_OPT_SIDE_BLOCKS_PER_CU 6
int myslam_orb_set_option(myslam_orb* h, int option, int value);
int myslam_orb_set_gauss_taps(myslam_orb* h, const int32_t* q7);
int myslam_orb_get_tables(const myslam_orb* h, float* scale, float* inv_scale, int* features_per_level, int* umax16);
int myslam_orb_max_keypoints(const myslam_orb* h);
int myslam_orb_max_keypoints_for(const myslam_orb* h, int rows, int cols);

int myslam_orb_detect_and_compute(myslam_orb* h, const uint8_t* img, int rows, int cols, int step,
                                  const uint8_t* mask, int mask_step,
                                  myslam_keypoint* kps, uint8_t* desc, int cap, int* n);
int myslam_orb_detect(myslam_orb* h, const uint8_t* img, int rows, int cols, int step,
                      const uint8_t* mask, int mask_step, myslam_keypoint* kps, int cap, int* n);
int myslam_orb_screen_and_compute_params(myslam_orb* h, const uint8_t* img, int rows, int cols, int step,
                                         myslam_keypoint* kps_in, int n_in,
                                         myslam_keypoint* kps_out, int cap, int* n_out);
int myslam_orb_calc_descriptors(myslam_orb* h, const uint8_t* img, int rows, int cols, int step,
                                const myslam_keypoint* kps, int n, uint8_t* desc);

int myslam_orb_detect_and_compute_batch(myslam_orb* h, const uint8_t* d_imgs, int batch, int rows, int cols,
                                        int step, size_t img_stride, const uint8_t* d_masks,
                                        myslam_keypoint* d_kps, uint8_t* d_desc, int32_t* d_counts,
                                        int32_t* d_status, int cap);
int myslam_orb_detect_batch(myslam_orb* h, const uint8_t* d_imgs, int batch, int rows, int cols,
                            int step, size_t img_stride, const uint8_t* d_masks,
                            myslam_keypoint* d_kps, int32_t* d_counts, int32_t* d_status, int cap);

int myslam_orb_process_keyframes_batch(myslam_orb* h,
        const uint8_t* d_imgs, int batch, int rows, int cols, int step, size_t img_stride,
        const float* d_feat_xy,
        const int32_t* d_n_feat,
        int feat_cap,
        myslam_keypoint* d_pyr_kps,
        uint8_t* d_desc,
        int32_t* d_counts, int32_t* d_status , int cap);

int myslam_orb_debug_pyramid(myslam_orb* h, const uint8_t* img, int rows, int cols, int step,
                             int level, int blurred, uint8_t* out, int out_step, int* w, int* hgt);
int myslam_orb_debug_candidates(myslam_orb* h, const uint8_t* img, int rows, int cols, int step,
                                const uint8_t* mask, int mask_step, int level,
                                int32_t* xs, int32_t* ys, int32_t* scores, int cap, int* n);

int myslam_orb_debug_readback(myslam_orb* h, int what, int b, int level, void* out, size_t cap_bytes, int detect_plan);

int myslam_hamming_match(const uint8_t* query, int nq, const uint8_t* train, int nt,
                         int32_t* train_idx, int32_t* dist);
int myslam_hamming_match_batch(const uint8_t* d_q, const int32_t* d_nq, const uint8_t* d_t, const int32_t* d_nt,
                               int batch, int cap, int32_t* d_train_idx, int32_t* d_dist, void* hip_stream);
int myslam_hamming_filter(const int32_t* dist, int n, uint8_t* keep, int* min_dist);

int myslam_expand_pyramid_keypoints(const myslam_keypoint* feats, int n, int nlevels, myslam_keypoint* out);
int myslam_match_feature_pairs(const int32_t* train_idx, const int32_t* dist, int n_query, const myslam_keypoint* loop_pyr_kps,
                               const myslam_keypoint* cur_pyr_kps, int n_train, int32_t* pairs, int* n_pairs);

#define MYSLAM_LOOP_MATCH_OK 0
#define MYSLAM_LOOP_MATCH_FEW_PAIRS 1
#define MYSLAM_LOOP_MATCH_FEW_POINTS 2
int myslam_loop_match_batch(
    const uint8_t* d_loop_desc, const int32_t* d_n_loop,
    const uint8_t* d_cur_desc,  const int32_t* d_n_cur,
    const myslam_keypoint* d_loop_pyr, const myslam_keypoint* d_cur_pyr,
    int batch, int cap,
    const float*   d_cur_feat_xy,
    const int32_t* d_loop_feat_landmark,
    int feat_cap,
    const double*  d_landmark_pos, size_t landmark_stride, int landmark_cap,
    int min_matches, int out_cap,
    int32_t* d_train_idx, int32_t* d_dist,
    int32_t* d_pairs, int32_t* d_n_pairs,
    int32_t* d_valid_pairs,
    float* d_pts3d, float* d_pts2d, int32_t* d_counts,
    int32_t* d_status, void* hip_stream);

typedef struct myslam_loop_store myslam_loop_store;
int myslam_loop_store_create(myslam_loop_store** out, int kf_capacity, int cap, int feat_cap);
int myslam_loop_store_destroy(myslam_loop_store* h);
int myslam_loop_store_set_stream(myslam_loop_store* h, void* hip_stream);
int myslam_loop_store_size(const myslam_loop_store* h);
int myslam_loop_store_capacity(const myslam_loop_store* h);
int myslam_loop_store_put_batch(myslam_loop_store* h, const uint64_t* ids , int batch,
        const myslam_keypoint* d_pyr_kps, const uint8_t* d_desc, const int32_t* d_counts,
        const int32_t* d_kf_status,
        const int32_t* d_feat_landmark,
        const int32_t* d_n_feat);
int myslam_loop_store_set_landmarks_batch(myslam_loop_store* h, const uint64_t* ids , int n,
        const int32_t* d_feat_landmark, const int32_t* d_n_feat);
#define MYSLAM_LOOP_DETECT_CANDIDATE 0
#define MYSLAM_LOOP_DETECT_NO_LOOP   1
int myslam_loop_detect_batch(myslam_loop_store* h,
        const uint64_t* d_best_id, const float* d_max_score, const int32_t* d_cnt, int nq,
        float thr_high, int max_suspected,
        uint8_t* d_loop_desc, int32_t* d_n_loop, myslam_keypoint* d_loop_pyr, int32_t* d_loop_feat_landmark,
        int32_t* d_loop_slot, int32_t* d_status);

int myslam_triangulate_stereo(const float* xl, const float* yl, const float* xr, const float* yr, int n,
                              double fx, double fy, double cx, double cy, double baseline,
                              double* xyz, uint8_t* ok);
int myslam_triangulate_stereo_batch(const myslam_keypoint* d_kps_l, const myslam_keypoint* d_kps_r,
                                    const int32_t* d_match, const int32_t* d_nl, int batch, int cap,
                                    double fx, double fy, double cx, double cy, double baseline,
                                    double* d_xyz, uint8_t* d_ok, void* hip_stream);

int myslam_hamming_match_triangulate_batch(const uint8_t* d_q, const int32_t* d_nq, const uint8_t* d_t, const int32_t* d_nt,
                                           const myslam_keypoint* d_kps_l, const myslam_keypoint* d_kps_r, int batch, int cap,
                                           double fx, double fy, double cx, double cy, double baseline,
                                           int32_t* d_train_idx, int32_t* d_dist, double* d_xyz, uint8_t* d_ok, void* hip_stream);

#define MYSLAM_CALC_CONV 1
#define MYSLAM_CALC_RELU 2
#define MYSLAM_CALC_POOL_MAX 3
#define MYSLAM_CALC_LRN 4
typedef struct myslam_calc_layer {
    int32_t type;
    int32_t num_output, kernel, stride, pad;
    int32_t local_size;
    float alpha, beta, k;
} myslam_calc_layer;
typedef struct myslam_lcd myslam_lcd;
int myslam_lcd_default_layers(myslam_calc_layer* layers, int cap);
int myslam_lcd_create(myslam_lcd** out, const float* weights, size_t nweights);
int myslam_lcd_create_from_layers(myslam_lcd** out, const myslam_calc_layer* layers, int nlayers, const float* weights, size_t nweights);
int myslam_lcd_create_from_caffe(myslam_lcd** out, const char* prototxt_path, const char* caffemodel_path);
int myslam_calc_parse_caffe(const char* prototxt_path, const char* caffemodel_path, myslam_calc_layer* layers, int cap, int* nlayers,
                            float* weights, size_t wcap, size_t* nweights);
int myslam_lcd_create_from_file(myslam_lcd** out, const char* path);
int myslam_lcd_uses_fused_kernels(const myslam_lcd* h);
int myslam_lcd_conv2_products(const myslam_lcd* h);
#define MYSLAM_LCD_OPT_GENERIC_KERNELS 1
#define MYSLAM_LCD_OPT_CONV2_BF16X6 2
#define MYSLAM_LCD_OPT_SKIP_KERNELS 3
int myslam_lcd_set_option(myslam_lcd* h, int option, int value);
int myslam_lcd_destroy(myslam_lcd* h);
int myslam_lcd_set_stream(myslam_lcd* h, void* hip_stream);
size_t myslam_lcd_nweights(void);
int myslam_lcd_calc_descr_original_img(myslam_lcd* h, uint8_t* img, int rows, int cols, int step,
                                       int blur_in_place, float* descr1064);
int myslam_lcd_calc_descr(myslam_lcd* h, const uint8_t* img160x120, int step, float* descr1064);
float myslam_lcd_score(const float* d1, const float* d2);
int myslam_lcd_describe_batch(myslam_lcd* h, uint8_t* d_imgs, int batch, int rows, int cols, int step,
                              size_t img_stride, int blur_in_place, float* d_descr );
int myslam_lcd_debug_forward(myslam_lcd* h, const float* in120x160, float* out_stage, int stage, size_t cap_floats);

typedef struct myslam_lcddb myslam_lcddb;
int myslam_lcddb_create(myslam_lcddb** out, int capacity);
int myslam_lcddb_destroy(myslam_lcddb* h);
int myslam_lcddb_set_stream(myslam_lcddb* h, void* hip_stream);
int myslam_lcddb_size(const myslam_lcddb* h);
int myslam_lcddb_capacity(const myslam_lcddb* h);
int myslam_lcddb_reserve(myslam_lcddb* h, int rows);
int myslam_lcddb_append(myslam_lcddb* h, uint64_t id, const float* descr1064);
int myslam_lcddb_append_batch(myslam_lcddb* h, const uint64_t* ids , const float* d_descr, int n);
int myslam_lcddb_append_batch_async(myslam_lcddb* h, const uint64_t* ids , const float* d_descr, int n, void* hip_stream);
int myslam_lcddb_query(myslam_lcddb* h, const float* descr1064, uint64_t cur_id, float thr_low,
                       uint64_t* best_id, float* max_score, int* cnt);
int myslam_lcddb_query_batch(myslam_lcddb* h, const float* d_q, const uint64_t* cur_ids , int nq, float thr_low,
// ... 295 lines not shown
```

Before: 82410.

## Add flat atomic-histogram octree path with redo pass for deep or large levels

```diff
diff --git a/a-simple-stereo-slam-system-with-deep-loop-closing_amd/api.py b/a-simple-stereo-slam-system-with-deep-loop-closing_amd/api.py
--- a/a-simple-stereo-slam-system-with-deep-loop-closing_amd/api.py
+++ b/a-simple-stereo-slam-system-with-deep-loop-closing_amd/api.py
@@ -142,6 +142,7 @@
         _check(lib().myslam_orb_set_fast_gate(self._h, C.c_void_p(event_ptr or None)), "myslam_orb_set_fast_gate")
 
     OPT_FAST_MODE, OPT_INTERNAL_STREAM, OPT_STOP_AFTER, OPT_COPY_INPUT, OPT_BLUR_MFMA, OPT_SIDE_BLOCKS_PER_CU = 1, 2, 3, 4, 5, 6
+    OPT_OCTREE_FLAT = 7
 
     def set_option(self, option, value):
         _check(lib().myslam_orb_set_option(self._h, int(option), int(value)), "myslam_orb_set_option")
@@ -249,6 +250,11 @@
         out = np.zeros(4, np.uint32)
         _check(lib().myslam_orb_debug_readback(self._h, 6, 0, level, _p(out), out.nbytes, 0), "debug_readback")
         return int(out[0]), int(out[1]), int(out[2])
+
+    def octree_redo_flag(self, b, level):
+        out = np.zeros(1, np.int32)
+        _check(lib().myslam_orb_debug_readback(self._h, 7, int(b), int(level), _p(out), out.nbytes, 0), "debug_readback")
+        return int(out[0])
 
 
 def hamming_match(query, train):
diff --git a/a-simple-stereo-slam-system-with-deep-loop-closing_amd/csrc/orb_engine.hip b/a-simple-stereo-slam-system-with-deep-loop-closing_amd/csrc/orb_engine.hip
--- a/a-simple-stereo-slam-system-with-deep-loop-closing_amd/csrc/orb_engine.hip
+++ b/a-simple-stereo-slam-system-with-deep-loop-closing_amd/csrc/orb_engine.hip
@@ -45,6 +45,7 @@
     Buf<uint32_t> d_cand;
     Buf<uint32_t> d_sort;
     Buf<int32_t> d_candCount, d_selCount, d_status;
+    Buf<int32_t> d_octRedo;
     Buf<uint32_t> d_sel;
     Buf<uint16_t> d_order;
     Buf<uint32_t> d_octTab;
@@ -58,6 +59,7 @@
     int optStopAfter = 0;
     int tapsSet = 0, taps[7] = {0};
     int optSideBlocksPerCu = 0;
+    int optOctreeFlat = 1;
     int optBlurMfma = 0;
     Buf<uint4> d_blurTab; bool blurTabValid = false; size_t blurOffI = 0, blurOffH[MAXL] = {0}, blurOffV[MAXL] = {0}; bool blurLvOk[MAXL] = {false}; int blurVconst = 0;
     int ensure_blur_tables();
@@ -312,6 +314,7 @@
             if ((rc = d_sort.renew((size_t)batch * full.totalKeyCap * 2))) return rc;
             if ((rc = d_candCount.renew((size_t)batch * MAXL))) return rc;
             if ((rc = d_selCount.renew((size_t)batch * MAXL))) return rc;
+            if ((rc = d_octRedo.renew((size_t)batch * MAXL))) return rc;
             if ((rc = d_status.renew((size_t)batch))) return rc;
             if ((rc = d_sel.renew((size_t)batch * selPer))) return rc;
             return d_order.renew((size_t)batch * selPer);
@@ -428,8 +431,9 @@
     const OrbPlan& P = detectOnly ? det : full;
     int32_t* stat = d_stat ? d_stat : d_status;
     if ((rc = ensure_fast_stat())) return rc;
-    clr = {{reinterpret_cast<uint32_t*>(d_candCount.get()), reinterpret_cast<uint32_t*>(d_selCount.get()), reinterpret_cast<uint32_t*>(stat), d_fastStat + (size_t)fastFlip * MAXL * 4},
-           {batch * MAXL, batch * MAXL, batch, MAXL * 4}};
+    clr = {{reinterpret_cast<uint32_t*>(d_candCount.get()), reinterpret_cast<uint32_t*>(d_selCount.get()), reinterpret_cast<uint32_t*>(stat), d_fastStat + (size_t)fastFlip * MAXL * 4,
+            reinterpret_cast<uint32_t*>(d_octRedo.get())},
+           {batch * MAXL, batch * MAXL, batch, MAXL * 4, batch * MAXL}};
     const int stop = optStopAfter;
     {
         int n0 = 0;
@@ -476,7 +480,7 @@
         if (tryBlur) fill_blur_args(blv, P.nlevels);
         blurred = launch_octree(P, d_cand, d_candCount, d_sort, d_octTab, d_sel, d_selCount, stat, batch,
                                 describe_uses_tile_order(d_order != nullptr, detectOnly ? 1 : 0, batch) ? d_order : nullptr, stream,
-                                tryBlur ? blv : nullptr, tryBlur ? P.nlevels : 0);
+                                tryBlur ? blv : nullptr, tryBlur ? P.nlevels : 0, d_octRedo, optOctreeFlat);
     }
     if (stop == 3) return MYSLAM_OK;
     if (fork) MYSLAM_HIP_CHECK(hipStreamWaitEvent(stream, evJoin, 0));
@@ -539,7 +543,7 @@
     if (optBlurMfma && (rc = ensure_blur_tables())) return rc;
     const int rowCap = feat_cap * nlevels;
     if ((rc = ensure_pkf((size_t)batch * rowCap))) return rc;
-    clr = {{reinterpret_cast<uint32_t*>(d_counts), reinterpret_cast<uint32_t*>(d_stat), nullptr, nullptr}, {batch, batch, 0, 0}};
+    clr = {{reinterpret_cast<uint32_t*>(d_counts), reinterpret_cast<uint32_t*>(d_stat), nullptr, nullptr, nullptr}, {batch, batch, 0, 0, 0}};
     set_in_place(nullptr, 0, 0, 0);
     rc = build_pyramids(d_imgs, batch, step, stride, nullptr, nlevels);
     clr = ZeroArgs{};
@@ -640,6 +644,7 @@
         case MYSLAM_ORB_OPT_STOP_AFTER: if (value < 0 || value > 4) return MYSLAM_ERR_INVALID; h->optStopAfter = value; return MYSLAM_OK;
         case MYSLAM_ORB_OPT_BLUR_MFMA: if (value < 0 || value > 1) return MYSLAM_ERR_INVALID; h->optBlurMfma = value; return MYSLAM_OK;
         case MYSLAM_ORB_OPT_SIDE_BLOCKS_PER_CU: if (value < 0 || value > 64) return MYSLAM_ERR_INVALID; h->optSideBlocksPerCu = value; return MYSLAM_OK;
+        case MYSLAM_ORB_OPT_OCTREE_FLAT: if (value < 0 || value > 2) return MYSLAM_ERR_INVALID; h->optOctreeFlat = value; return MYSLAM_OK;
     }
     return MYSLAM_ERR_INVALID;
 }
@@ -903,9 +908,9 @@
             MYSLAM_HIP_CHECK(hipMemcpy2D(out, g.w, base, g.pitch, g.w, g.h, hipMemcpyDeviceToHost));
             return MYSLAM_OK;
         }
-        case 2: case 4: {
+        case 2: case 4: case 7: {
             if (cap_bytes < 4) return MYSLAM_ERR_CAPACITY;
-            MYSLAM_HIP_CHECK(hipMemcpy(out, (what == 2 ? h->d_candCount : h->d_selCount) + b * MAXL + level, 4, hipMemcpyDeviceToHost));
+            MYSLAM_HIP_CHECK(hipMemcpy(out, (what == 2 ? h->d_candCount : what == 4 ? h->d_selCount : h->d_octRedo) + b * MAXL + level, 4, hipMemcpyDeviceToHost));
             return MYSLAM_OK;
         }
         case 3: {
diff --git a/a-simple-stereo-slam-system-with-deep-loop-closing_amd/csrc/orb_kernels.hip b/a-simple-stereo-slam-system-with-deep-loop-closing_amd/csrc/orb_kernels.hip
--- a/a-simple-stereo-slam-system-with-deep-loop-closing_amd/csrc/orb_kernels.hip
+++ b/a-simple-stereo-slam-system-with-deep-loop-closing_amd/csrc/orb_kernels.hip
@@ -44,6 +44,7 @@
 #define MYSLAM_BT_PARAM , BlockTrace* btp_
 #define MYSLAM_BT_ARG , &bt_
 #define MYSLAM_BT_MARKP(i) btp_->mark(i)
+#define MYSLAM_BT_AUXP(v) btp_->aux = (v)
 #else
 #define MYSLAM_BT(kid) ((void)0)
 #define MYSLAM_BT_MARK(i) ((void)0)
@@ -51,6 +52,7 @@
 #define MYSLAM_BT_PARAM
 #define MYSLAM_BT_ARG
 #define MYSLAM_BT_MARKP(i) ((void)0)
+#define MYSLAM_BT_AUXP(v) ((void)0)
 #endif
 
 __constant__ int8_t c_pattern[1024] = {
@@ -1403,6 +1405,11 @@
 }
 
 constexpr int OT_MAXB = 1024;
+constexpr int OCT_NODE_BYTES = 54;
+#ifndef MYSLAM_OCT_COMPACT
+#define MYSLAM_OCT_COMPACT 1
+#endif
+constexpr int OCT_NODE_BYTES_FLAT = MYSLAM_OCT_COMPACT ? 26 : OCT_NODE_BYTES;
 
 __device__ __forceinline__ uint64_t wave_incl_scan64(uint64_t v) {
 #define MYSLAM_SCAN64_STEP(CTRL, ROWS)                                                                                   \
@@ -1501,12 +1508,16 @@
     __device__ __forceinline__ uint16_t* cpos(int i) const { return i ? cpos1 : cpos0; }
 };
 
+template <bool FLAT>
 __device__ __forceinline__ void child_bounds(const OctLds& L, uint32_t* __restrict__ S, uint32_t* __restrict__ Cd, int D, int lo, int hi, int d, int pfx,
-                                             int& b1, int& b2, int& b3) {
+                                             int& b1, int& b2, int& b3, int* deep) {
     if (d < D) {
         const int sb = 2 * (D - d - 1);
         const int base = pfx << 2;
         b1 = L.offs[(base + 1) << sb]; b2 = L.offs[(base + 2) << sb]; b3 = L.offs[(base + 3) << sb];
+    } else if constexpr (FLAT) {
+        *deep = 1;
+        b1 = b2 = b3 = hi;
     } else {
         partition4(S, Cd, lo, hi, ROOT_SHIFT - 2 * (d + 1), b1, b2, b3);
     }
@@ -1528,25 +1539,20 @@
 }
 
 constexpr int OCT_WIDE_BELOW = 64;
+#ifndef MYSLAM_OCT_REDO_WORKERS
+#define MYSLAM_OCT_REDO_WORKERS (256 * 5)
+#endif
+constexpr int OCT_REDO_WORKERS = MYSLAM_OCT_REDO_WORKERS;
 constexpr int OCT_FL = 4;
-template <int OT>
-__global__ __launch_bounds__(OT) void k_octree(OrbPlan P, const uint32_t* __restrict__ cand,
-                                               const int32_t* __restrict__ candCount, uint32_t* __restrict__ sortbuf,
-                                               const uint32_t* __restrict__ octTab,
-                                               uint32_t* __restrict__ selOut, int32_t* __restrict__ selCount,
-                                               int32_t* __restrict__ status, int NCmax, uint16_t* __restrict__ order, BlurMulti BM) {
-    MYSLAM_SIDE_PRIO();
-    MYSLAM_BT(2);
-    extern __shared__ __attribute__((aligned(16))) uint8_t smem[];
+constexpr int OCT_REDO_DEEP = 1, OCT_REDO_PAYLOAD = 2;
+template <int OT, bool FLAT>
+__device__ __forceinline__ void octree_item(const OrbPlan& P, const uint32_t* __restrict__ cand,
+                                            const int32_t* __restrict__ candCount, uint32_t* __restrict__ sortbuf,
+                                            const uint32_t* __restrict__ octTab,
+                                            uint32_t* __restrict__ selOut, int32_t* __restrict__ selCount,
+                                            int32_t* __restrict__ status, int NCmax, int areaBytes, uint16_t* __restrict__ order,
+                                            int32_t* __restrict__ redo, const int b, const int level, uint8_t* smem MYSLAM_BT_PARAM) {
     const int t = threadIdx.x;
-    if constexpr (OT == 512) {
-        if ((int)blockIdx.y >= P.nlevels) {
-            const int wv = __builtin_amdgcn_readfirstlane(t >> 6);
-            blur7_strip_wave(BM, ((int)blockIdx.y - P.nlevels) * 8 + wv, blockIdx.x, smem + wv * (16 * B3_TS));
-            return;
-        }
-    }
-    const int level = blockIdx.y, b = blockIdx.x;
     const LevelGeom& g = P.lv[level];
     const int NC = NCmax;
 
@@ -1557,13 +1563,17 @@
     OctLds L;
     L.offs = reinterpret_cast<uint32_t*>(pcur); pcur += 4 * (OT_MAXB + 2);
     uint32_t* const s_tab = reinterpret_cast<uint32_t*>(pcur);
-    L.lo0 = reinterpret_cast<uint32_t*>(pcur); pcur += 4 * NC;
-    L.lo1 = reinterpret_cast<uint32_t*>(pcur); pcur += 4 * NC;
-    L.hi0 = reinterpret_cast<uint32_t*>(pcur); pcur += 4 * NC;
-    L.hi1 = reinterpret_cast<uint32_t*>(pcur); pcur += 4 * NC;
-    L.nb1 = reinterpret_cast<uint32_t*>(pcur); pcur += 4 * NC;
-    L.nb2 = reinterpret_cast<uint32_t*>(pcur); pcur += 4 * NC;
-    L.nb3 = reinterpret_cast<uint32_t*>(pcur); pcur += 4 * NC;
+    constexpr bool CMP = FLAT && MYSLAM_OCT_COMPACT;
+    L.lo0 = L.lo1 = L.hi0 = L.hi1 = L.nb1 = L.nb2 = L.nb3 = nullptr;
+    if constexpr (!CMP) {
+        L.lo0 = reinterpret_cast<uint32_t*>(pcur); pcur += 4 * NC;
+        L.lo1 = reinterpret_cast<uint32_t*>(pcur); pcur += 4 * NC;
+        L.hi0 = reinterpret_cast<uint32_t*>(pcur); pcur += 4 * NC;
+        L.hi1 = reinterpret_cast<uint32_t*>(pcur); pcur += 4 * NC;
+        L.nb1 = reinterpret_cast<uint32_t*>(pcur); pcur += 4 * NC;
+        L.nb2 = reinterpret_cast<uint32_t*>(pcur); pcur += 4 * NC;
+        L.nb3 = reinterpret_cast<uint32_t*>(pcur); pcur += 4 * NC;
+    }
     L.ckey0 = reinterpret_cast<uint32_t*>(pcur); pcur += 4 * NC;
     L.ckey1 = reinterpret_cast<uint32_t*>(pcur); pcur += 4 * NC;
     L.pfx0 = reinterpret_cast<uint16_t*>(pcur); pcur += 2 * NC;
@@ -1586,6 +1596,10 @@
     }
     const int n = cnt;
     if (n == 0) { if (t == 0) *myCount = 0; return; }
+    const bool rankkey = g.nCols * g.nRows <= 1024;
+    if constexpr (FLAT) {
+        if (!rankkey) { if (t == 0) redo[b * MAXL + level] = OCT_REDO_PAYLOAD; return; }
+    }
 
     const uint32_t* keys = cand + (size_t)b * P.totalKeyCap + g.keyOff;
     uint32_t* S = sortbuf + ((size_t)b * P.totalKeyCap + g.keyOff) * 2;
@@ -1597,11 +1611,12 @@
     const uint32_t* xcode = octTab + g.tabOff; const uint32_t* ycode = xcode + g.tabX;
     const uint32_t* xcell = ycode + g.tabY; const uint32_t* ycell = xcell + g.tabX;
     const int ntab = 2 * (g.tabX + g.tabY);
-    const bool tabLds = (size_t)ntab * 4 <= (size_t)54 * NC;
-    for (int i = t; i < NB; i += OT) s_cursor[i] = 0;
+    const bool tabLds = ntab * 4 <= areaBytes;
+    uint32_t* const s_best = s_cursor;
+    if constexpr (FLAT) { for (int i = t; i < NB; i += OT) { L.offs[i] = 0; s_best[i] = 0; } }
+    else { for (int i = t; i < NB; i += OT) s_cursor[i] = 0; }
     if (tabLds) for (int i = t; i < ntab; i += OT) s_tab[i] = xcode[i];
     __syncthreads();
-    const bool rankkey = g.nCols * g.nRows <= 1024;
     const float inv_ncols = 1.0f / (float)g.nCols;
     auto passes = [&](auto in_lds) __attribute__((always_inline)) {
         constexpr bool LDS = decltype(in_lds)::value;
@@ -1610,6 +1625,44 @@
         auto YC = [&](uint32_t i) -> uint32_t { if constexpr (LDS) return s_tab[oyc + i]; else return ycode[i]; };
         auto XL = [&](uint32_t i) -> uint32_t { if constexpr (LDS) return s_tab[oxl + i]; else return xcell[i]; };
         auto YL = [&](uint32_t i) -> uint32_t { if constexpr (LDS) return s_tab[oyl + i]; else return ycell[i]; };
+        if constexpr (FLAT) {
+            for (int i0 = t; i0 < n; i0 += OCT_FL * OT) {
+                uint32_t pay[OCT_FL], cx[OCT_FL], cy[OCT_FL], qx[OCT_FL], qy[OCT_FL];
+#pragma unroll
+                for (int u = 0; u < OCT_FL; u++) pay[u] = (i0 + u * OT < n) ? keys[i0 + u * OT] : 0u;
+#pragma unroll
+                for (int u = 0; u < OCT_FL; u++) {
+                    const uint32_t px = (pay[u] >> 8) & 0xfff, py = pay[u] >> 20;
+                    cx[u] = XC(px); cy[u] = YC(py); qx[u] = XL(px); qy[u] = YL(py);
+                }
+#pragma unroll
+                for (int u = 0; u < OCT_FL; u++) {
+                    if (i0 + u * OT >= n) continue;
+                    const int px = (int)((pay[u] >> 8) & 0xfff), py = (int)(pay[u] >> 20);
+                    const int ci = (int)(((float)qy[u] + 0.5f) * inv_ncols);
+                    const uint32_t pxc = (uint32_t)(px - 3 - (int)qx[u] * g.wCell), pyc = (uint32_t)(py - 3 - ci * g.hCell);
+                    const uint32_t key = ((pay[u] & 0xffu) << 22) | (0x3fffffu - (((qy[u] + qx[u]) << 12) | (pyc << 6) | pxc));
+                    const uint32_t bucket = (cx[u] | cy[u]) >> bsh;
+                    atomicAdd(&L.offs[bucket], 1u);
+                    atomicMax(&s_best[bucket], key);
+                }
+            }
+            __syncthreads();
+            const int c = (NB + OT - 1) / OT;
+            const int beg = min(NB, t * c), end = min(NB, beg + c);
+            uint64_t sum = 0;
+            for (int i = beg; i < end; i++) sum += L.offs[i];
+            uint64_t total;
+            uint64_t run = block_excl_scan64<OT>(sum, s_w, total);
+            for (int i = beg; i < end; i++) {
+                const uint32_t h = L.offs[i];
+                L.offs[i] = (uint32_t)run;
+                run += h;
+            }
+            if (t == 0) L.offs[NB] = (uint32_t)n;
+            __syncthreads();
+            return;
+        }
         for (int i0 = t; i0 < n; i0 += OCT_FL * OT) {
             uint32_t pay[OCT_FL], cx[OCT_FL], cy[OCT_FL];
 #pragma unroll
@@ -1666,15 +1719,25 @@
     };
     if (tabLds) passes(std::true_type{}); else passes(std::false_type{});
 
-    MYSLAM_BT_MARK(0);
-    MYSLAM_BT_AUX((unsigned long long)level | ((unsigned long long)n << 8));
+    MYSLAM_BT_MARKP(0);
+    MYSLAM_BT_AUXP((unsigned long long)level | ((unsigned long long)n << 8));
+    auto nlo = [&](int buf, int p) -> int {
+        if constexpr (CMP) return (int)L.offs[(int)L.pfx(buf)[p] << (2 * (D - (int)L.dep(buf)[p]))]; else return (int)L.lo(buf)[p];
+    };
+    auto nhi = [&](int buf, int p) -> int {
+        if constexpr (CMP) return (int)L.offs[((int)L.pfx(buf)[p] + 1) << (2 * (D - (int)L.dep(buf)[p]))]; else return (int)L.hi(buf)[p];
+    };
+    auto put_node = [&](int buf, int pos, int lo, int hi, int d, int pf) {
+        if constexpr (!CMP) { L.lo(buf)[pos] = (uint32_t)lo; L.hi(buf)[pos] = (uint32_t)hi; }
+        L.dep(buf)[pos] = (uint8_t)d; L.pfx(buf)[pos] = (uint16_t)pf;
+    };
     if (t == 0) {
         int m = 0;
         for (int r = 0; r < g.nIni; r++) {
             const int lo = L.offs[r << (2 * D)], hi = L.offs[(r + 1) << (2 * D)];
-            if (hi > lo) { L.lo0[m] = (uint32_t)lo; L.hi0[m] = (uint32_t)hi; L.dep0[m] = 0; L.pfx0[m] = (uint16_t)r; m++; }
-        }
-        s_i[0] = m; s_i[1] = 0;
+            if (hi > lo) { put_node(0, m, lo, hi, 0, r); m++; }
+        }
+        s_i[0] = m; s_i[1] = 0; s_i[3] = 0;
     }
     __syncthreads();
 
@@ -1689,12 +1752,12 @@
             const int beg = min(m, t * c), end = min(m, beg + c);
             uint64_t packed = 0;
             for (int p = beg; p < end; p++) {
-                const int lo = (int)L.lo(cur)[p], hi = (int)L.hi(cur)[p], d = L.dep(cur)[p];
+                const int lo = nlo(cur, p), hi = nhi(cur, p), d = L.dep(cur)[p];
                 int k = 0;
                 if (hi - lo > 1 && d < g.ndepth) {
                     int b1, b2, b3;
-                    child_bounds(L, S, Cd, D, lo, hi, d, L.pfx(cur)[p], b1, b2, b3);
-                    L.nb1[p] = (uint32_t)b1; L.nb2[p] = (uint32_t)b2; L.nb3[p] = (uint32_t)b3;
+                    child_bounds<FLAT>(L, S, Cd, D, lo, hi, d, L.pfx(cur)[p], b1, b2, b3, &s_i[3]);
+                    if constexpr (!CMP) { L.nb1[p] = (uint32_t)b1; L.nb2[p] = (uint32_t)b2; L.nb3[p] = (uint32_t)b3; }
                     const int c0 = b1 - lo, c1 = b2 - b1, c2 = b3 - b2, c3 = hi - b3;
                     k = (c0 > 0) + (c1 > 0) + (c2 > 0) + (c3 > 0);
                     const int big = (c0 > 1) + (c1 > 1) + (c2 > 1) + (c3 > 1);
@@ -1706,14 +1769,20 @@
             }
             uint64_t total;
             uint64_t run = block_excl_scan64<OT>(packed, s_w, total);
-            const int Ktot = (int)(total & 0x1fffff), Ntot = (int)((total >> 21) & 0x1fffff), Btot = (int)(total >> 42);
+            if constexpr (FLAT) {
+                if (s_i[3]) { if (t == 0) redo[b * MAXL + level] = OCT_REDO_DEEP; return; }
+            }
+            const int Ktot =(int)(total & 0x1fffff), Ntot = (int)((total >> 21) & 0x1fffff), Btot = (int)(total >> 42);
             const int nxt = cur ^ 1, cnxt = ccur ^ 1;
             for (int p = beg; p < end; p++) {
-                const int lo = (int)L.lo(cur)[p], hi = (int)L.hi(cur)[p], d = L.dep(cur)[p];
+                const int lo = nlo(cur, p), hi = nhi(cur, p), d = L.dep(cur)[p];
                 const int pf = L.pfx(cur)[p];
                 const int k = L.kk[p];
                 if (k) {
-                    const int bnd[5] = {lo, (int)L.nb1[p], (int)L.nb2[p], (int)L.nb3[p], hi};
+                    int b1, b2, b3;
+                    if constexpr (CMP) child_bounds<FLAT>(L, S, Cd, D, lo, hi, d, pf, b1, b2, b3, &s_i[3]);
+                    else { b1 = (int)L.nb1[p]; b2 = (int)L.nb2[p]; b3 = (int)L.nb3[p]; }
+                    const int bnd[5] = {lo, b1, b2, b3, hi};
                     const int rk = (int)(run & 0x1fffff);
                     int pos = Ktot - (rk + k);
                     int cidx = (int)(run >> 42);
@@ -1722,9 +1791,7 @@
                     for (int q = 3; q >= 0; q--) {
                         childPos[q] = pos;
                         if (bnd[q + 1] > bnd[q]) {
-                            L.lo(nxt)[pos] = (uint32_t)bnd[q]; L.hi(nxt)[pos] = (uint32_t)bnd[q + 1];
-                            L.dep(nxt)[pos] = (uint8_t)(d + 1);
-                            L.pfx(nxt)[pos] = (uint16_t)((pf << 2) | q);
+                            put_node(nxt, pos, bnd[q], bnd[q + 1], d + 1, (pf << 2) | q);
                             pos++;
                         }
                     }
@@ -1741,9 +1808,7 @@
                     run += (uint64_t)k | ((uint64_t)big << 42);
                 } else {
                     const int rn = (int)((run >> 21) & 0x1fffff);
-                    L.lo(nxt)[Ktot + rn] = (uint32_t)lo; L.hi(nxt)[Ktot + rn] = (uint32_t)hi;
-                    L.dep(nxt)[Ktot + rn] = (uint8_t)d;
-                    L.pfx(nxt)[Ktot + rn] = (uint16_t)pf;
+                    put_node(nxt, Ktot + rn, lo, hi, d, pf);
                     run += 1ull << 21;
                 }
             }
@@ -1771,20 +1836,23 @@
             uint64_t packed = 0;
             for (int j = beg; j < end; j++) {
                 const int p = L.cpos(ccur)[L.ord[j]];
-                const int lo = (int)L.lo(cur)[p], hi = (int)L.hi(cur)[p], d = L.dep(cur)[p];
+                const int lo = nlo(cur, p), hi = nhi(cur, p), d = L.dep(cur)[p];
                 int k = 1, big = 1, b1 = hi, b2 = hi, b3 = hi;
                 if (d < g.ndepth) {
-                    child_bounds(L, S, Cd, D, lo, hi, d, L.pfx(cur)[p], b1, b2, b3);
+                    child_bounds<FLAT>(L, S, Cd, D, lo, hi, d, L.pfx(cur)[p], b1, b2, b3, &s_i[3]);
                     const int c0 = b1 - lo, c1 = b2 - b1, c2 = b3 - b2, c3 = hi - b3;
                     k = (c0 > 0) + (c1 > 0) + (c2 > 0) + (c3 > 0);
                     big = (c0 > 1) + (c1 > 1) + (c2 > 1) + (c3 > 1);
                 }
-                L.nb1[j] = (uint32_t)b1; L.nb2[j] = (uint32_t)b2; L.nb3[j] = (uint32_t)b3;
+                if constexpr (!CMP) { L.nb1[j] = (uint32_t)b1; L.nb2[j] = (uint32_t)b2; L.nb3[j] = (uint32_t)b3; }
                 L.kk[j] = (uint8_t)(k | (big << 4));
                 packed += (uint64_t)k | ((uint64_t)big << 32);
             }
             uint64_t total;
             uint64_t run = block_excl_scan64<OT>(packed, s_w, total);
+            if constexpr (FLAT) {
+                if (s_i[3]) { if (t == 0) redo[b * MAXL + level] = OCT_REDO_DEEP; return; }
+            }
             for (int j = beg; j < end; j++) {
                 const int k = L.kk[j] & 15, big = L.kk[j] >> 4;
                 run += (uint64_t)k | ((uint64_t)big << 32);
@@ -1801,10 +1869,13 @@
             __syncthreads();
             for (int j = t; j < ncmt; j += OT) {
                 const int p = L.cpos(ccur)[L.ord[j]];
-                const int lo = (int)L.lo(cur)[p], hi = (int)L.hi(cur)[p], d = L.dep(cur)[p];
+                const int lo = nlo(cur, p), hi = nhi(cur, p), d = L.dep(cur)[p];
                 const int pf = L.pfx(cur)[p];
                 const int big = L.kk[j] >> 4;
-                const int bnd[5] = {lo, (int)L.nb1[j], (int)L.nb2[j], (int)L.nb3[j], hi};
+                int b1 = hi, b2 = hi, b3 = hi;
+                if constexpr (CMP) { if (d < g.ndepth) child_bounds<FLAT>(L, S, Cd, D, lo, hi, d, pf, b1, b2, b3, &s_i[3]); }
+                else { b1 = (int)L.nb1[j]; b2 = (int)L.nb2[j]; b3 = (int)L.nb3[j]; }
+                const int bnd[5] = {lo, b1, b2, b3, hi};
                 int pos = Kc - L.kinc[j];
                 int childPos[4];
                 if (d < g.ndepth) {
@@ -1812,9 +1883,7 @@
                     for (int q = 3; q >= 0; q--) {
                         childPos[q] = pos;
                         if (bnd[q + 1] > bnd[q]) {
-                            L.lo(nxt)[pos] = (uint32_t)bnd[q]; L.hi(nxt)[pos] = (uint32_t)bnd[q + 1];
-                            L.dep(nxt)[pos] = (uint8_t)(d + 1);
-                            L.pfx(nxt)[pos] = (uint16_t)((pf << 2) | q);
+                            put_node(nxt, pos, bnd[q], bnd[q + 1], d + 1, (pf << 2) | q);
                             pos++;
                         }
                     }
@@ -1829,7 +1898,7 @@
                         }
                     }
                 } else {
-                    L.lo(nxt)[pos] = (uint32_t)lo; L.hi(nxt)[pos] = (uint32_t)hi; L.dep(nxt)[pos] = (uint8_t)d; L.pfx(nxt)[pos] = (uint16_t)pf;
+                    put_node(nxt, pos, lo, hi, d, pf);
                     const int cidx = L.binc[j] - 1;
                     L.ckey(cnxt)[cidx] = ((uint32_t)(hi - lo) << 14) | (uint32_t)cidx;
                     L.cpos(cnxt)[cidx] = (uint16_t)pos;
@@ -1844,9 +1913,7 @@
                 uint64_t ex = block_excl_scan64<OT>(un, s_w, tot2);
                 for (int p = pb; p < pe; p++) {
                     if (L.mark[p] == 0) {
-                        L.lo(nxt)[Kc + (int)ex] = L.lo(cur)[p]; L.hi(nxt)[Kc + (int)ex] = L.hi(cur)[p];
-                        L.dep(nxt)[Kc + (int)ex] = L.dep(cur)[p];
-                        L.pfx(nxt)[Kc + (int)ex] = L.pfx(cur)[p];
+                        put_node(nxt, Kc + (int)ex, nlo(cur, p), nhi(cur, p), L.dep(cur)[p], L.pfx(cur)[p]);
                         ex++;
                     }
                 }
@@ -1861,7 +1928,7 @@
         }
     }
 
-    MYSLAM_BT_MARK(1);
+    MYSLAM_BT_MARKP(1);
     const int m = s_i[0];
     uint32_t* out = selOut + (size_t)b * P.totalOut + g.outBase;
     {
@@ -1871,6 +1938,19 @@
         const int ngrp = OT / GLN;
         for (int p0 = t / GLN; p0 < ((mm + ngrp - 1) / ngrp) * ngrp; p0 += ngrp) {
             const bool live = p0 < mm;
+            if constexpr (FLAT) {
+                int b0 = 0, b1 = 0;
+                if (live) { const int sh = 2 * (D - (int)L.dep(cur)[p0]), pf = L.pfx(cur)[p0]; b0 = pf << sh; b1 = (pf + 1) << sh; }
+                uint32_t bk = 0;
+                for (int i = b0 + sub; i < b1; i += 8) bk = max(bk, s_best[i]);
+                bk = half_row_max_u32(bk);
+                if (live && sub == 0) {
+                    const uint32_t rank = 0x3fffffu - (bk & 0x3fffffu), cell = rank >> 12;
+                    const int ci = (int)(((float)cell + 0.5f) * inv_ncols), cj = (int)cell - ci * g.nCols;
+                    const uint32_t px = (rank & 63u) + 3u + (uint32_t)(cj * g.wCell), py = ((rank >> 6) & 63u) + 3u + (uint32_t)(ci * g.hCell);
+                    out[p0] = (py << 20) | (px << 8) | (bk >> 22);
+                }
+            } else {
             const int lo = live ? (int)L.lo(cur)[p0] : 0, hi = live ? (int)L.hi(cur)[p0] : 0;
             if (rankkey) {
                 uint32_t bk = 0;
@@ -1908,10 +1988,11 @@
 #pragma unroll
             for (int o = 1; o < 16; o <<= 1) bo = min(bo, (uint64_t)__shfl_xor((unsigned long long)bo, o, 64));
             if (live && sub == 0) out[p0] = ((uint32_t)((bo >> 12) & 0xfff) << 20) | ((uint32_t)(bo & 0xfff) << 8) | best;
+            }
         }
     }
     if (t == 0) *myCount = min(m, g.nodeCap);
-    MYSLAM_BT_MARK(2);
+    MYSLAM_BT_MARKP(2);
     if (order) {
         __threadfence_block();
         __syncthreads();
@@ -1942,6 +2023,38 @@
         }
         __syncthreads();
         for (int i = t; i < n; i += OT) ord[atomicAdd(&s_hist[sel_order_bin(__hip_atomic_load(&out[i], __ATOMIC_RELAXED, __HIP_MEMORY_SCOPE_AGENT), ts)], 1)] = (uint16_t)i;
+    }
+}
+
+template <int OT, bool FLAT>
+__global__ __launch_bounds__(OT) void k_octree(OrbPlan P, const uint32_t* __restrict__ cand,
+                                               const int32_t* __restrict__ candCount, uint32_t* __restrict__ sortbuf,
+                                               const uint32_t* __restrict__ octTab,
+                                               uint32_t* __restrict__ selOut, int32_t* __restrict__ selCount,
+                                               int32_t* __restrict__ status, int NCmax, int areaBytes, uint16_t* __restrict__ order, BlurMulti BM,
+                                               int32_t* __restrict__ redo, int batch) {
+    MYSLAM_SIDE_PRIO();
+    extern __shared__ __attribute__((aligned(16))) uint8_t smem[];
+    if constexpr (OT == 512) {
+        if ((int)blockIdx.y >= P.nlevels) {
+            const int wv = __builtin_amdgcn_readfirstlane((int)threadIdx.x >> 6);
+            blur7_strip_wave(BM, ((int)blockIdx.y - P.nlevels) * 8 + wv, blockIdx.x, smem + wv * (16 * B3_TS));
+            return;
+        }
+    }
+    const bool walk = !FLAT && redo != nullptr;
+    const int nitems = batch * P.nlevels;
+    for (int it = walk ? (int)blockIdx.x : 0; it < nitems; it += walk ? (int)gridDim.x : nitems) {
+        int b = blockIdx.x, level = blockIdx.y;
+        if (walk) {
+            level = it / batch; b = it - level * batch;
+            if (redo[b * MAXL + level] == 0) continue;
+        }
+        {
+            MYSLAM_BT(2);
+            octree_item<OT, FLAT>(P, cand, candCount, sortbuf, octTab, selOut, selCount, status, NCmax, areaBytes, order, redo, b, level, smem MYSLAM_BT_ARG);
+        }
+        if (walk) __syncthreads();
     }
 }
 
@@ -2525,7 +2638,7 @@
 
 __device__ __forceinline__ void zero_part(const ZeroArgs& z, int tid, int T) {
 #pragma unroll
-    for (int k = 0; k < 4; k++)
+    for (int k = 0; k < 5; k++)
         for (int i = tid; i < z.n[k]; i += T) z.p[k][i] = 0u;
 }
 __device__ __forceinline__ void ingest_part(const uint8_t* __restrict__ src, int rows, int cols, int step, size_t sstride,
@@ -2566,11 +2679,11 @@
 __global__ __launch_bounds__(256) void k_zero_u32(ZeroArgs a) {
     const int i = blockIdx.x * 256 + threadIdx.x;
 #pragma unroll
-    for (int k = 0; k < 4; k++)
+    for (int k = 0; k < 5; k++)
         if (a.p[k] && i < a.n[k]) a.p[k][i] = 0u;
 }
 void launch_zero_u32(const ZeroArgs& z, hipStream_t s) {
-    const int n = max(max(z.n[0], z.n[1]), max(z.n[2], z.n[3]));
+    const int n = max(max(max(z.n[0], z.n[1]), max(z.n[2], z.n[3])), z.n[4]);
     if (n > 0) hipLaunchKernelGGL(k_zero_u32, dim3((n + 255) / 256), dim3(256), 0, s, z);
 }
 
@@ -2697,25 +2810,44 @@
     else hipLaunchKernelGGL((k_fast_strip<MAX_CELL, 4>), grid, dim3(256), 0, s, P, pyr, pyrStride, maskPyr, cand, candCount, ctl, batch);
 }
 
-size_t octree_lds_bytes(int nodeCap) { return 192 + 4 * (size_t)OT_MAXB + 4 * (size_t)(OT_MAXB + 2) + (size_t)nodeCap * 54 + 16; }
+static size_t octree_lds_for_area(size_t area) { return 192 + 4 * (size_t)OT_MAXB + 4 * (size_t)(OT_MAXB + 2) + area + 16; }
+size_t octree_lds_bytes(int nodeCap) { return octree_lds_for_area((size_t)nodeCap * OCT_NODE_BYTES); }
+size_t octree_flat_area_bytes(int nodeCap, size_t tabBytes) {
+    const size_t nodes = (size_t)nodeCap * OCT_NODE_BYTES_FLAT, legacy = (size_t)nodeCap * OCT_NODE_BYTES;
+    return tabBytes <= legacy ? std::max(nodes, (tabBytes + 15) & ~(size_t)15) : nodes;
+}
+size_t octree_flat_lds_bytes(int nodeCap, size_t tabBytes) { return octree_lds_for_area(octree_flat_area_bytes(nodeCap, tabBytes)); }
 
 bool launch_octree(const OrbPlan& P, const uint32_t* cand, const int32_t* candCount, uint32_t* sortbuf, const uint32_t* octTab, uint32_t* selOut,
-                   int32_t* selCount, int32_t* status, int batch, uint16_t* order, hipStream_t s, const BlurArgs* blurLv, int nBlur) {
+                   int32_t* selCount, int32_t* status, int batch, uint16_t* order, hipStream_t s, const BlurArgs* blurLv, int nBlur,
+                   int32_t* redo, int flatMode) {
+    const bool flat = redo != nullptr && (flatMode == 2 || (flatMode == 1 && batch >= OCT_WIDE_BELOW));
     BlurMulti BMh;
-    const BlurMulti* blurWith = (blurLv && nBlur > 0 && blur_multi_for_octree(blurLv, nBlur, batch, BMh)) ? &BMh : nullptr;
+    const BlurMulti* blurWith = (!flat && blurLv && nBlur > 0 && blur_multi_for_octree(blurLv, nBlur, batch, BMh)) ? &BMh : nullptr;
     int ncmax = 0;
     for (int l = 0; l < P.nlevels; l++) ncmax = max(ncmax, P.lv[l].nodeCap);
     const size_t lds = std::max(octree_lds_bytes(ncmax), (size_t)8 * 16 * B3_TS);
-    (void)hipFuncSetAttribute(reinterpret_cast<const void*>(k_octree<256>), hipFuncAttributeMaxDynamicSharedMemorySize, 160 * 1024);
-    (void)hipFuncSetAttribute(reinterpret_cast<const void*>(k_octree<512>), hipFuncAttributeMaxDynamicSharedMemorySize, 160 * 1024);
-    if (batch >= OCT_WIDE_BELOW)
-        hipLaunchKernelGGL(k_octree<256>, dim3(batch, P.nlevels), dim3(256), lds, s, P, cand, candCount, sortbuf, octTab, selOut, selCount, status, ncmax, order, BlurMulti{});
+    const int area = ncmax * OCT_NODE_BYTES;
+    size_t tabBytes = 0;
+    for (int l = 0; l < P.nlevels; l++)
+        if (P.lv[l].nCols * P.lv[l].nRows <= 1024) tabBytes = std::max(tabBytes, (size_t)8 * (P.lv[l].tabX + P.lv[l].tabY));
+    const int areaFlat = (int)octree_flat_area_bytes(ncmax, tabBytes);
+    const size_t ldsFlat = octree_flat_lds_bytes(ncmax, tabBytes);
+    (void)hipFuncSetAttribute(reinterpret_cast<const void*>(k_octree<256, false>), hipFuncAttributeMaxDynamicSharedMemorySize, 160 * 1024);
+    (void)hipFuncSetAttribute(reinterpret_cast<const void*>(k_octree<256, true>), hipFuncAttributeMaxDynamicSharedMemorySize, 160 * 1024);
+    (void)hipFuncSetAttribute(reinterpret_cast<const void*>(k_octree<512, false>), hipFuncAttributeMaxDynamicSharedMemorySize, 160 * 1024);
+    if (flat) {
+        hipLaunchKernelGGL((k_octree<256, true>), dim3(batch, P.nlevels), dim3(256), ldsFlat, s, P, cand, candCount, sortbuf, octTab, selOut, selCount, status, ncmax, areaFlat, order, BlurMulti{}, redo, batch);
+        const int workers = min(batch * P.nlevels, OCT_REDO_WORKERS);
+        hipLaunchKernelGGL((k_octree<256, false>), dim3(workers), dim3(256), lds, s, P, cand, candCount, sortbuf, octTab, selOut, selCount, status, ncmax, area, order, BlurMulti{}, redo, batch);
+    } else if (batch >= OCT_WIDE_BELOW)
+        hipLaunchKernelGGL((k_octree<256, false>), dim3(batch, P.nlevels), dim3(256), lds, s, P, cand, candCount, sortbuf, octTab, selOut, selCount, status, ncmax, area, order, BlurMulti{}, (int32_t*)nullptr, batch);
     else
     {
         BlurMulti M = blurWith ? *blurWith : BlurMulti{};
         if (!blurWith) M.n = 0;
         const int brows = blurWith ? (M.wave0[M.n] + 7) / 8 : 0;
-        hipLaunchKernelGGL(k_octree<512>, dim3(batch, P.nlevels + brows), dim3(512), lds, s, P, cand, candCount, sortbuf, octTab, selOut, selCount, status, ncmax, order, M);
+        hipLaunchKernelGGL((k_octree<512, false>), dim3(batch, P.nlevels + brows), dim3(512), lds, s, P, cand, candCount, sortbuf, octTab, selOut, selCount, status, ncmax, area, order, M, (int32_t*)nullptr, batch);
     }
     return blurWith != nullptr;
 }
diff --git a/a-simple-stereo-slam-system-with-deep-loop-closing_amd/csrc/orb_launch.h b/a-simple-stereo-slam-system-with-deep-loop-closing_amd/csrc/orb_launch.h
--- a/a-simple-stereo-slam-system-with-deep-loop-closing_amd/csrc/orb_launch.h
+++ b/a-simple-stereo-slam-system-with-deep-loop-closing_amd/csrc/orb_launch.h
@@ -6,7 +6,7 @@
 
 namespace myslam_hip {
 
-struct ZeroArgs { uint32_t* p[4]; int n[4]; };
+struct ZeroArgs { uint32_t* p[5]; int n[5]; };
 
 void gauss_q8(int kind, int q[7]);
 
@@ -31,8 +31,10 @@
 void launch_fast(const OrbPlan& P, const uint8_t* pyr, size_t pyrStride, const uint8_t* maskPyr, uint32_t* cand,
                  int32_t* candCount, const uint32_t* statPrev, uint32_t* statCur, int forceMode, int batch, hipStream_t s);
 size_t octree_lds_bytes(int nodeCap);
+size_t octree_flat_lds_bytes(int nodeCap, size_t tabBytes);
 bool launch_octree(const OrbPlan& P, const uint32_t* cand, const int32_t* candCount, uint32_t* sortbuf, const uint32_t* octTab, uint32_t* selOut,
-                   int32_t* selCount, int32_t* status, int batch, uint16_t* order, hipStream_t s, const BlurArgs* blurLv, int nBlur);
+                   int32_t* selCount, int32_t* status, int batch, uint16_t* order, hipStream_t s, const BlurArgs* blurLv, int nBlur,
+                   int32_t* redo, int flatMode);
 bool describe_uses_tile_order(bool have_order, int detectOnly, int batch);
 void launch_describe(const OrbPlan& P, const uint8_t* pyr, const uint8_t* blur, size_t pyrStride, const uint32_t* selOut,
                      const int32_t* selCount, myslam_keypoint* kps, uint8_t* desc, int32_t* counts, int32_t* status,
diff --git a/include/myslam_hip.h b/include/myslam_hip.h
--- a/include/myslam_hip.h
+++ b/include/myslam_hip.h
@@ -45,6 +45,7 @@
 #define MYSLAM_ORB_OPT_COPY_INPUT 4
 #define MYSLAM_ORB_OPT_BLUR_MFMA 5
 #define MYSLAM_ORB_OPT_SIDE_BLOCKS_PER_CU 6
+#define MYSLAM_ORB_OPT_OCTREE_FLAT 7
 int myslam_orb_set_option(myslam_orb* h, int option, int value);
 int myslam_orb_set_gauss_taps(myslam_orb* h, const int32_t* q7);
 int myslam_orb_get_tables(const myslam_orb* h, float* scale, float* inv_scale, int* features_per_level, int* umax16);
```

Result: no change. 82760 (median of 2 runs) (+0.4%).
